# fatchord/WaveRNN

Hardware: AMD Instinct MI355X
Metric: audio samples/sec (real-time factor @22.05 kHz), MoL WaveRNN batched generate (higher is better)
Workload: dtype f32

## Files before the change

### include/wavernn_amd.h

```cpp
#ifndef WAVERNN_AMD_H
#define WAVERNN_AMD_H

#include <stddef.h>
#include <stdint.h>

#ifdef __cplusplus
extern "C" {
#endif

#define WRNN_ABI_VERSION 9

enum {
    WRNN_OK = 0,
    WRNN_ERR_ARG = -1,
    WRNN_ERR_NO_DEVICE = -2,
    WRNN_ERR_HIP = -3,
    WRNN_ERR_WORKSPACE = -4,
    WRNN_ERR_KERNEL = -5,
    WRNN_ERR_RESIDENCY = -6
};

enum { WRNN_MODE_RAW = 0, WRNN_MODE_MOL = 1 };

enum {
    WRNN_ALGO_AUTO = 0,
    WRNN_ALGO_STREAM = 1,
    WRNN_ALGO_LOOP = 2,
    WRNN_ALGO_DUO = 6,
    WRNN_ALGO_CHAIN = 7,
    WRNN_ALGO_OCTO = 8,
    WRNN_ALGO_SPARSE = 5
};

typedef struct wrnn_weights {
    int32_t rnn_dims;
    int32_t fc_dims;
    int32_t feat_dims;
    int32_t aux_dims;
    int32_t n_classes;
    int32_t mode;
    const float *I_w, *I_b;
    const float *w_ih1, *w_hh1, *b_ih1, *b_hh1;
    const float *w_ih2, *w_hh2, *b_ih2, *b_hh2;
    const float *fc1_w, *fc1_b;
    const float *fc2_w, *fc2_b;
    const float *fc3_w, *fc3_b;
} wrnn_weights;

typedef struct wrnn_pack wrnn_pack;

typedef struct wrnn_geometry {
    int32_t B;
    int32_t T;
    int32_t stride;
    int32_t L;
    int32_t hop;
    int32_t n_frames;
} wrnn_geometry;

typedef struct wrnn_timer wrnn_timer;

typedef struct wrnn_run_info {
    const char *kernel;
    int32_t units_per_wg;
    int32_t clusters;
    int32_t depth;
    int32_t rounds;
    int32_t slab_steps;
    int32_t launches;
} wrnn_run_info;

typedef struct wrnn_options {
    int32_t struct_bytes;
    int32_t algo;
    int32_t depth;
    int32_t clusters;
    int32_t cond_valu;
    int32_t slab_steps;
    int32_t t_begin, t_end;
    int32_t tuning;
    const float *force_x;
    float *logits;
    unsigned long long *phase_clocks;
    wrnn_timer *timer;
    wrnn_run_info *info;
    void (*progress)(int32_t steps_done, int32_t T, int32_t n_segments, void *user);
    void *progress_user;
    int32_t mel_stage;
    int32_t mel_rows;
    int32_t mel_scale;
    const float *mel_taps;
    const int32_t *seg_moff;
    int32_t sparse_groups;
    int32_t noise_lib;
    uint64_t noise_seed;
    const uint64_t *noise_seg_id;
} wrnn_options;

const char *wrnn_last_error(void);
int wrnn_abi_version(void);

int wrnn_device_cus(int device);

int wrnn_pack_create(const wrnn_weights *w, int device, wrnn_pack **out);
void wrnn_pack_destroy(wrnn_pack *p);
size_t wrnn_pack_weight_bytes(const wrnn_pack *p);
int wrnn_pack_sparse_blocks(const wrnn_pack *p);
int wrnn_pack_sparse_fc_blocks(const wrnn_pack *p);

size_t wrnn_workspace_bytes(const wrnn_pack *p, const wrnn_geometry *g, const wrnn_options *opt);

int wrnn_generate(const wrnn_pack *p, const wrnn_geometry *g, const float *mels_up, const float *aux,
                  const float *noise, float *out, void *workspace, size_t workspace_bytes, const wrnn_options *opt,
                  void *stream);

int wrnn_generate_segments(const wrnn_pack *p, int32_t n_segments, int32_t T, const int32_t *seg_pos,
                           const int32_t *seg_lim, int32_t L, int32_t hop, int32_t n_frames,
                           const float *mels_up, const float *aux, const float *noise, float *out,
                           void *workspace, size_t workspace_bytes, const wrnn_options *opt, void *stream);
size_t wrnn_workspace_bytes_segments(const wrnn_pack *p, int32_t n_segments, int32_t T, int32_t n_frames,
                                     const wrnn_options *opt);

int wrnn_noise_fill(int mode, int32_t n_segments, int32_t n_classes, int32_t t_begin, int32_t t_end, uint64_t seed, const uint64_t *seg_id,
                    float *out, int device, void *stream);
int wrnn_noise_fill_host(int mode, int32_t n_segments, int32_t n_classes, int32_t t_begin, int32_t t_end, uint64_t seed, const uint64_t *seg_id,
                         float *out);

int wrnn_plan_segments(const wrnn_pack *p, int32_t n_segments, int32_t T, const wrnn_options *opt, wrnn_run_info *out);

int wrnn_status(void *workspace, void *stream);

int wrnn_debug_read_exchange(const wrnn_pack *p, void *workspace, int32_t n_segments, int32_t T, int32_t n_frames,
                             const wrnn_options *opt, int cluster, int slot, int layer, int ring, float *host_out);

typedef struct wrnn_plan_traits {
    int32_t struct_bytes;
    int32_t n_cus;
    int32_t mode, C;
    int32_t generic;
    int32_t gH, gF, gM, gA;
    int32_t sp_nbp;
    int32_t sp_max_blocks;
    int32_t sp_fc;
} wrnn_plan_traits;
int wrnn_debug_plan(const wrnn_plan_traits *traits, int32_t n_segments, int32_t T, int32_t n_frames,
                    const wrnn_options *opt, wrnn_run_info *out, size_t *workspace_bytes);

int wrnn_timer_create(int device, wrnn_timer **out);
void wrnn_timer_destroy(wrnn_timer *t);
float wrnn_timer_ms(wrnn_timer *t);
int wrnn_timer_launches(const wrnn_timer *t);

typedef struct wrnn_pre_weights {
    int32_t feat_dims;
    int32_t compute_dims;
    int32_t res_out_dims;
    int32_t res_blocks;
    int32_t pad;
    int32_t upsample_factors[3];
    const float *conv_in_w;
    const float *bn_in;
    const float *res_w;
    const float *res_bn;
    const float *conv_out_w;
    const float *conv_out_b;
    const float *up_w;
} wrnn_pre_weights;
typedef struct wrnn_pre wrnn_pre;

int wrnn_pre_create(const wrnn_pre_weights *w, int device, wrnn_pre **out);
void wrnn_pre_destroy(wrnn_pre *p);
int wrnn_pre_hop(const wrnn_pre *p);
size_t wrnn_pre_workspace_bytes(const wrnn_pre *p, int32_t n_frames);
int wrnn_pre_upsample(const wrnn_pre *p, const float *mel, int32_t n_frames, float *mels_up, float *aux,
                      void *workspace, size_t workspace_bytes, void *stream);
int wrnn_pre_upsample_rows(const wrnn_pre *p, const float *mel, int32_t n_frames, float *mel_rows, float *aux,
                           void *workspace, size_t workspace_bytes, void *stream);
const char *wrnn_pre_last_error(void);

int wrnn_post_unfold(const float *segments, int32_t T, int32_t n_utt, const int32_t *first, const int32_t *folds,
                     const int64_t *out_off, const double *lut, int32_t n_classes, const double *fade_in,
                     const double *fade_out, int32_t overlap, const double *tail, int32_t tail_len, int32_t batched,
                     double *out, void *stream);
const char *wrnn_post_last_error(void);

typedef struct wrnn_taco_weights {
    uint32_t struct_bytes;
    int32_t n_mels, prenet1, prenet2, decoder_dims, encoder_width, lstm_dims, attn_filters, attn_kernel;
    const float *prenet_fc1_w, *prenet_fc1_b, *prenet_fc2_w, *prenet_fc2_b;
    const float *attn_rnn_w_ih, *attn_rnn_w_hh, *attn_rnn_b_ih, *attn_rnn_b_hh;
    const float *attn_W_w, *attn_W_b, *attn_conv_w, *attn_L_w, *attn_L_b, *attn_v_w;
    const float *rnn_input_w, *rnn_input_b;
    const float *rnn1_w_ih, *rnn1_w_hh, *rnn1_b_ih, *rnn1_b_hh;
    const float *rnn2_w_ih, *rnn2_w_hh, *rnn2_b_ih, *rnn2_b_hh;
    const float *mel_proj_w;
} wrnn_taco_weights;

typedef struct wrnn_taco_call {
    uint32_t struct_bytes;
    int32_t n;
    int32_t r, max_r;
    int32_t max_steps;
    float stop_threshold;
    const float *seq;
    const float *seq_proj;
    float *mel_out;
    float *scores_out;
    int32_t *steps_done;
    void *workspace;
    size_t workspace_bytes;
    void *stream;
    int32_t variant;
} wrnn_taco_call;

size_t wrnn_taco_workspace_bytes(void);
int wrnn_taco_decode(int device, const wrnn_taco_weights *w, const wrnn_taco_call *c);
int wrnn_taco_status(const void *workspace, unsigned *out4, void *stream);
const char *wrnn_taco_last_error(void);

#define WRNN_TACO_BATCH_MAX 8
#define WRNN_TACO_BATCH_NMAX 256
typedef struct wrnn_taco_batch_call {
    uint32_t struct_bytes;
    int32_t n_sent;
    int32_t r, max_r;
    float stop_threshold;
    const int32_t *n;
    const int32_t *max_steps;
    const float *const *seq, *const *seq_proj;
    float *const *mel_out;
    float *const *scores_out;
    int32_t *steps_done;
    void *workspace;
    size_t workspace_bytes;
    void *stream;
} wrnn_taco_batch_call;
size_t wrnn_taco_batch_workspace_bytes(int32_t n_sent);
int wrnn_taco_decode_batch(int device, const wrnn_taco_weights *w, const wrnn_taco_batch_call *c);

typedef struct wrnn_bigru_call {
    uint32_t struct_bytes;
    int32_t T, hidden;
    const float *gi_fwd, *gi_rev;
    const float *w_hh_fwd, *w_hh_rev;
    const float *b_hh_fwd, *b_hh_rev;
    float *out;
    void *stream;
} wrnn_bigru_call;
int wrnn_bigru(int device, const wrnn_bigru_call *c);

typedef struct wrnn_cbhg_weights {
    int32_t K;
    int32_t in_channels;
    int32_t proj1_channels;
    int32_t proj2_channels;
    int32_t channels;
    int32_t num_highways;
    const float *bank_conv_w[16];
    const float *bank_bn_w[16], *bank_bn_b[16], *bank_bn_mean[16], *bank_bn_var[16];
    const float *proj1_conv_w;
    const float *proj1_bn_w, *proj1_bn_b, *proj1_bn_mean, *proj1_bn_var;
    const float *proj2_conv_w;
    const float *proj2_bn_w, *proj2_bn_b, *proj2_bn_mean, *proj2_bn_var;
    const float *pre_highway_w;
    const float *highway_w1[4], *highway_b1[4], *highway_w2[4], *highway_b2[4];
    const float *rnn_w_ih, *rnn_w_hh, *rnn_b_ih, *rnn_b_hh;
    const float *rnn_w_ih_rev, *rnn_w_hh_rev, *rnn_b_ih_rev, *rnn_b_hh_rev;
} wrnn_cbhg_weights;

typedef struct wrnn_taco_front_weights {
    uint32_t struct_bytes;
    int32_t n_symbols, embed_dims;
    int32_t prenet1, prenet2;
    int32_t encoder_proj_dims;
    int32_t n_mels, fft_bins;
    const float *embedding;
    const float *prenet_fc1_w, *prenet_fc1_b, *prenet_fc2_w, *prenet_fc2_b;
    const float *encoder_proj_w, *post_proj_w;
    wrnn_cbhg_weights encoder_cbhg;
    wrnn_cbhg_weights postnet;
} wrnn_taco_front_weights;
typedef struct wrnn_taco_front wrnn_taco_front;

int wrnn_taco_front_create(const wrnn_taco_front_weights *w, int device, wrnn_taco_front **out);
void wrnn_taco_front_destroy(wrnn_taco_front *f);
size_t wrnn_taco_front_workspace_bytes(const wrnn_taco_front *f, int32_t rows);
int wrnn_taco_encode(const wrnn_taco_front *f, const int32_t *ids, int32_t n, float *seq_out, float *seq_proj_out, float *pre_rnn_out,
                     void *workspace, size_t workspace_bytes, void *stream);
int wrnn_taco_postnet(const wrnn_taco_front *f, const float *mel, int32_t N, float *linear_out, float *pre_rnn_out,
                      void *workspace, size_t workspace_bytes, void *stream);

int wrnn_selftest(int device, int which);
float wrnn_selftest_metric(void);

#ifdef __cplusplus
}
#endif
#endif
```

### wavernn_amd/_lib.py

```python
import ctypes
import os
import subprocess

_HERE = os.path.dirname(os.path.abspath(__file__))
CSRC = os.path.join(_HERE, 'csrc')
SO_PATH = os.path.join(CSRC, 'libwavernn_amd.so')

WRNN_OK = 0
ERR_ARG = -1
ERR_NO_DEVICE = -2
ERR_RESIDENCY = -6
MODE_RAW, MODE_MOL = 0, 1
ABI_VERSION = 9
ALGO_AUTO, ALGO_STREAM, ALGO_LOOP, ALGO_SPARSE, ALGO_DUO, ALGO_CHAIN, ALGO_OCTO = 0, 1, 2, 5, 6, 7, 8
ALGOS = {'auto': ALGO_AUTO, 'stream': ALGO_STREAM, 'loop': ALGO_LOOP, 'sparse': ALGO_SPARSE, 'duo': ALGO_DUO, 'chain': ALGO_CHAIN, 'octo': ALGO_OCTO}

EXPORTS = ['wrnn_last_error', 'wrnn_abi_version', 'wrnn_device_cus', 'wrnn_pack_create', 'wrnn_pack_destroy',
           'wrnn_pack_weight_bytes', 'wrnn_pack_sparse_blocks', 'wrnn_pack_sparse_fc_blocks', 'wrnn_workspace_bytes', 'wrnn_workspace_bytes_segments', 'wrnn_generate',
           'wrnn_generate_segments', 'wrnn_noise_fill', 'wrnn_noise_fill_host', 'wrnn_plan_segments', 'wrnn_status', 'wrnn_timer_create', 'wrnn_timer_destroy', 'wrnn_timer_ms',
           'wrnn_timer_launches', 'wrnn_debug_read_exchange', 'wrnn_debug_plan', 'wrnn_selftest', 'wrnn_selftest_metric', 'wrnn_pre_create',
           'wrnn_pre_destroy', 'wrnn_pre_hop', 'wrnn_pre_workspace_bytes', 'wrnn_pre_upsample', 'wrnn_pre_upsample_rows', 'wrnn_pre_last_error',
           'wrnn_post_unfold', 'wrnn_post_last_error', 'wrnn_taco_workspace_bytes', 'wrnn_taco_decode', 'wrnn_taco_status',
           'wrnn_taco_last_error', 'wrnn_bigru', 'wrnn_taco_front_create', 'wrnn_taco_front_destroy', 'wrnn_taco_front_workspace_bytes',
           'wrnn_taco_encode', 'wrnn_taco_postnet', 'wrnn_taco_batch_workspace_bytes', 'wrnn_taco_decode_batch']


class Weights(ctypes.Structure):
    _fields_ = [(n, ctypes.c_int32) for n in ('rnn_dims', 'fc_dims', 'feat_dims', 'aux_dims', 'n_classes', 'mode')] + \
               [(n, ctypes.c_void_p) for n in ('I_w', 'I_b', 'w_ih1', 'w_hh1', 'b_ih1', 'b_hh1', 'w_ih2', 'w_hh2',
                                               'b_ih2', 'b_hh2', 'fc1_w', 'fc1_b', 'fc2_w', 'fc2_b', 'fc3_w', 'fc3_b')]


class PreWeights(ctypes.Structure):
    _fields_ = [(n, ctypes.c_int32) for n in ('feat_dims', 'compute_dims', 'res_out_dims', 'res_blocks', 'pad')] + \
               [('upsample_factors', ctypes.c_int32 * 3)] + \
               [(n, ctypes.c_void_p) for n in ('conv_in_w', 'bn_in', 'res_w', 'res_bn', 'conv_out_w', 'conv_out_b', 'up_w')]


TACO_WEIGHT_FIELDS = ('prenet_fc1_w', 'prenet_fc1_b', 'prenet_fc2_w', 'prenet_fc2_b', 'attn_rnn_w_ih', 'attn_rnn_w_hh', 'attn_rnn_b_ih',
                      'attn_rnn_b_hh', 'attn_W_w', 'attn_W_b', 'attn_conv_w', 'attn_L_w', 'attn_L_b', 'attn_v_w', 'rnn_input_w', 'rnn_input_b',
                      'rnn1_w_ih', 'rnn1_w_hh', 'rnn1_b_ih', 'rnn1_b_hh', 'rnn2_w_ih', 'rnn2_w_hh', 'rnn2_b_ih', 'rnn2_b_hh', 'mel_proj_w')


class TacoWeights(ctypes.Structure):
    _fields_ = [('struct_bytes', ctypes.c_uint32)] + \
               [(n, ctypes.c_int32) for n in ('n_mels', 'prenet1', 'prenet2', 'decoder_dims', 'encoder_width', 'lstm_dims', 'attn_filters',
                                              'attn_kernel')] + \
               [(n, ctypes.c_void_p) for n in TACO_WEIGHT_FIELDS]


class TacoCall(ctypes.Structure):
    _fields_ = [('struct_bytes', ctypes.c_uint32), ('n', ctypes.c_int32), ('r', ctypes.c_int32), ('max_r', ctypes.c_int32),
                ('max_steps', ctypes.c_int32), ('stop_threshold', ctypes.c_float), ('seq', ctypes.c_void_p), ('seq_proj', ctypes.c_void_p),
                ('mel_out', ctypes.c_void_p), ('scores_out', ctypes.c_void_p), ('steps_done', ctypes.c_void_p),
                ('workspace', ctypes.c_void_p), ('workspace_bytes', ctypes.c_size_t), ('stream', ctypes.c_void_p), ('variant', ctypes.c_int32)]


TACO_BATCH_MAX = 8
TACO_BATCH_NMAX = 256


class TacoBatchCall(ctypes.Structure):
    _fields_ = [('struct_bytes', ctypes.c_uint32), ('n_sent', ctypes.c_int32), ('r', ctypes.c_int32), ('max_r', ctypes.c_int32),
                ('stop_threshold', ctypes.c_float), ('n', ctypes.POINTER(ctypes.c_int32)), ('max_steps', ctypes.POINTER(ctypes.c_int32)),
                ('seq', ctypes.POINTER(ctypes.c_void_p)), ('seq_proj', ctypes.POINTER(ctypes.c_void_p)),
                ('mel_out', ctypes.POINTER(ctypes.c_void_p)), ('scores_out', ctypes.POINTER(ctypes.c_void_p)),
                ('steps_done', ctypes.c_void_p), ('workspace', ctypes.c_void_p), ('workspace_bytes', ctypes.c_size_t), ('stream', ctypes.c_void_p)]


class BigruCall(ctypes.Structure):
    _fields_ = [('struct_bytes', ctypes.c_uint32), ('T', ctypes.c_int32), ('hidden', ctypes.c_int32)] + \
               [(n, ctypes.c_void_p) for n in ('gi_fwd', 'gi_rev', 'w_hh_fwd', 'w_hh_rev', 'b_hh_fwd', 'b_hh_rev', 'out', 'stream')]


class CbhgWeights(ctypes.Structure):
    _fields_ = [(n, ctypes.c_int32) for n in ('K', 'in_channels', 'proj1_channels', 'proj2_channels', 'channels', 'num_highways')] + \
               [(n, ctypes.c_void_p * 16) for n in ('bank_conv_w', 'bank_bn_w', 'bank_bn_b', 'bank_bn_mean', 'bank_bn_var')] + \
               [(n, ctypes.c_void_p) for n in ('proj1_conv_w', 'proj1_bn_w', 'proj1_bn_b', 'proj1_bn_mean', 'proj1_bn_var', 'proj2_conv_w',
                                               'proj2_bn_w', 'proj2_bn_b', 'proj2_bn_mean', 'proj2_bn_var', 'pre_highway_w')] + \
               [(n, ctypes.c_void_p * 4) for n in ('highway_w1', 'highway_b1', 'highway_w2', 'highway_b2')] + \
               [(n, ctypes.c_void_p) for n in ('rnn_w_ih', 'rnn_w_hh', 'rnn_b_ih', 'rnn_b_hh', 'rnn_w_ih_rev', 'rnn_w_hh_rev', 'rnn_b_ih_rev',
                                               'rnn_b_hh_rev')]


class TacoFrontWeights(ctypes.Structure):
    _fields_ = [('struct_bytes', ctypes.c_uint32)] + \
               [(n, ctypes.c_int32) for n in ('n_symbols', 'embed_dims', 'prenet1', 'prenet2', 'encoder_proj_dims', 'n_mels', 'fft_bins')] + \
               [(n, ctypes.c_void_p) for n in ('embedding', 'prenet_fc1_w', 'prenet_fc1_b', 'prenet_fc2_w', 'prenet_fc2_b', 'encoder_proj_w',
                                               'post_proj_w')] + \
               [('encoder_cbhg', CbhgWeights), ('postnet', CbhgWeights)]


class Geometry(ctypes.Structure):
    _fields_ = [(n, ctypes.c_int32) for n in ('B', 'T', 'stride', 'L', 'hop', 'n_frames')]


class RunInfo(ctypes.Structure):
    _fields_ = [('kernel', ctypes.c_char_p)] + \
               [(n, ctypes.c_int32) for n in ('units_per_wg', 'clusters', 'depth', 'rounds', 'slab_steps', 'launches')]


class PlanTraits(ctypes.Structure):
    _fields_ = [(n, ctypes.c_int32) for n in ('struct_bytes', 'n_cus', 'mode', 'C', 'generic', 'gH', 'gF', 'gM', 'gA', 'sp_nbp', 'sp_max_blocks',
                                              'sp_fc')]

    def __init__(self, **kw):
        super().__init__(**kw)
        self.struct_bytes = ctypes.sizeof(PlanTraits)


class Options(ctypes.Structure):
    _fields_ = [(n, ctypes.c_int32) for n in ('struct_bytes', 'algo', 'depth', 'clusters', 'cond_valu', 'slab_steps', 't_begin',
                                              't_end', 'tuning')] + \
               [('force_x', ctypes.c_void_p), ('logits', ctypes.c_void_p), ('phase_clocks', ctypes.c_void_p), ('timer', ctypes.c_void_p),
                ('info', ctypes.POINTER(RunInfo)), ('progress', ctypes.c_void_p), ('progress_user', ctypes.c_void_p),
                ('mel_stage', ctypes.c_int32), ('mel_rows', ctypes.c_int32), ('mel_scale', ctypes.c_int32),
                ('mel_taps', ctypes.c_void_p), ('seg_moff', ctypes.c_void_p), ('sparse_groups', ctypes.c_int32),
                ('noise_lib', ctypes.c_int32), ('noise_seed', ctypes.c_uint64), ('noise_seg_id', ctypes.c_void_p)]

    def __init__(self, **kw):
        super().__init__(**kw)
        self.struct_bytes = ctypes.sizeof(Options)


PROGRESS_FN = ctypes.CFUNCTYPE(None, ctypes.c_int32, ctypes.c_int32, ctypes.c_int32, ctypes.c_void_p)


class WrnnError(RuntimeError):
    pass


class ResidencyError(WrnnError):
    """WRNN_ERR_RESIDENCY on the FIRST slice of a step-sliced `auto` run: the persistent grid is not co-resident right now.  The
    callers that slice (WaveRNN.generate, generate_corpus) catch it and redo the call unsliced on the stream kernel."""


def build(verbose=False):
    cmd = [os.path.join(CSRC, 'build.sh')]
    res = subprocess.run(cmd, stdout=subprocess.PIPE, stderr=subprocess.STDOUT, text=True)
    if verbose or res.returncode != 0:
        print(res.stdout)
    if res.returncode != 0:
        raise WrnnError('building libwavernn_amd.so failed')
    global _lib
    _lib = None
    return SO_PATH


_lib = None


def lib():
    global _lib
    if _lib is not None:
        return _lib
    if not os.path.exists(SO_PATH):
        raise WrnnError(f'{SO_PATH} not found: run `python -c "import __graft_entry__ as g; g.build()"` '
                        f'(or wavernn_amd/csrc/build.sh).  There is no CPU fallback.')
    import torch
    L = ctypes.CDLL(SO_PATH)
    L.wrnn_last_error.restype = ctypes.c_char_p
    L.wrnn_abi_version.restype = ctypes.c_int
    L.wrnn_device_cus.argtypes = [ctypes.c_int]
    L.wrnn_pack_create.argtypes = [ctypes.POINTER(Weights), ctypes.c_int, ctypes.POINTER(ctypes.c_void_p)]
    L.wrnn_pack_destroy.argtypes = [ctypes.c_void_p]
    L.wrnn_pack_destroy.restype = None
    L.wrnn_pack_weight_bytes.argtypes = [ctypes.c_void_p]
    L.wrnn_pack_weight_bytes.restype = ctypes.c_size_t
    L.wrnn_pack_sparse_blocks.argtypes = [ctypes.c_void_p]
    L.wrnn_pack_sparse_fc_blocks.argtypes = [ctypes.c_void_p]
    L.wrnn_workspace_bytes.argtypes = [ctypes.c_void_p, ctypes.POINTER(Geometry), ctypes.POINTER(Options)]
    L.wrnn_workspace_bytes.restype = ctypes.c_size_t
    L.wrnn_generate.argtypes = [ctypes.c_void_p, ctypes.POINTER(Geometry), ctypes.c_void_p, ctypes.c_void_p,
                                ctypes.c_void_p, ctypes.c_void_p, ctypes.c_void_p, ctypes.c_size_t, ctypes.POINTER(Options),
                                ctypes.c_void_p]
    L.wrnn_workspace_bytes_segments.argtypes = [ctypes.c_void_p, ctypes.c_int32, ctypes.c_int32, ctypes.c_int32,
                                                ctypes.POINTER(Options)]
    L.wrnn_workspace_bytes_segments.restype = ctypes.c_size_t
    L.wrnn_generate_segments.argtypes = [ctypes.c_void_p, ctypes.c_int32, ctypes.c_int32, ctypes.c_void_p, ctypes.c_void_p,
                                         ctypes.c_int32, ctypes.c_int32, ctypes.c_int32, ctypes.c_void_p, ctypes.c_void_p,
                                         ctypes.c_void_p, ctypes.c_void_p, ctypes.c_void_p, ctypes.c_size_t,
                                         ctypes.POINTER(Options), ctypes.c_void_p]
    L.wrnn_noise_fill.argtypes = [ctypes.c_int, ctypes.c_int32, ctypes.c_int32, ctypes.c_int32, ctypes.c_int32, ctypes.c_uint64, ctypes.c_void_p,
                                  ctypes.c_void_p, ctypes.c_int, ctypes.c_void_p]
    L.wrnn_noise_fill_host.argtypes = L.wrnn_noise_fill.argtypes[:8]
    L.wrnn_plan_segments.argtypes = [ctypes.c_void_p, ctypes.c_int32, ctypes.c_int32, ctypes.POINTER(Options), ctypes.POINTER(RunInfo)]
    L.wrnn_timer_create.argtypes = [ctypes.c_int, ctypes.POINTER(ctypes.c_void_p)]
    L.wrnn_timer_destroy.argtypes = [ctypes.c_void_p]
    L.wrnn_timer_destroy.restype = None
    L.wrnn_timer_ms.argtypes = [ctypes.c_void_p]
    L.wrnn_timer_ms.restype = ctypes.c_float
    L.wrnn_timer_launches.argtypes = [ctypes.c_void_p]
    L.wrnn_debug_read_exchange.argtypes = [ctypes.c_void_p, ctypes.c_void_p, ctypes.c_int32, ctypes.c_int32, ctypes.c_int32,
                                           ctypes.POINTER(Options), ctypes.c_int, ctypes.c_int, ctypes.c_int, ctypes.c_int,
                                           ctypes.c_void_p]
    L.wrnn_debug_plan.argtypes = [ctypes.POINTER(PlanTraits), ctypes.c_int32, ctypes.c_int32, ctypes.c_int32, ctypes.POINTER(Options),
                                  ctypes.POINTER(RunInfo), ctypes.POINTER(ctypes.c_size_t)]
    L.wrnn_pre_create.argtypes = [ctypes.POINTER(PreWeights), ctypes.c_int, ctypes.POINTER(ctypes.c_void_p)]
    L.wrnn_pre_destroy.argtypes = [ctypes.c_void_p]
    L.wrnn_pre_destroy.restype = None
    L.wrnn_pre_hop.argtypes = [ctypes.c_void_p]
    L.wrnn_pre_workspace_bytes.argtypes = [ctypes.c_void_p, ctypes.c_int32]
    L.wrnn_pre_workspace_bytes.restype = ctypes.c_size_t
    L.wrnn_pre_upsample.argtypes = [ctypes.c_void_p, ctypes.c_void_p, ctypes.c_int32, ctypes.c_void_p, ctypes.c_void_p,
                                    ctypes.c_void_p, ctypes.c_size_t, ctypes.c_void_p]
    L.wrnn_pre_upsample_rows.argtypes = L.wrnn_pre_upsample.argtypes
    L.wrnn_pre_last_error.restype = ctypes.c_char_p
    L.wrnn_post_unfold.argtypes = [ctypes.c_void_p, ctypes.c_int32, ctypes.c_int32, ctypes.c_void_p, ctypes.c_void_p, ctypes.c_void_p,
                                   ctypes.c_void_p, ctypes.c_int32, ctypes.c_void_p, ctypes.c_void_p, ctypes.c_int32,
                                   ctypes.c_void_p, ctypes.c_int32, ctypes.c_int32, ctypes.c_void_p, ctypes.c_void_p]
    L.wrnn_post_last_error.restype = ctypes.c_char_p
    L.wrnn_taco_workspace_bytes.restype = ctypes.c_size_t
    L.wrnn_taco_decode.argtypes = [ctypes.c_int, ctypes.POINTER(TacoWeights), ctypes.POINTER(TacoCall)]
    L.wrnn_taco_status.argtypes = [ctypes.c_void_p, ctypes.POINTER(ctypes.c_uint32 * 4), ctypes.c_void_p]
    L.wrnn_taco_last_error.restype = ctypes.c_char_p
    L.wrnn_taco_batch_workspace_bytes.argtypes = [ctypes.c_int32]
    L.wrnn_taco_batch_workspace_bytes.restype = ctypes.c_size_t
    L.wrnn_taco_decode_batch.argtypes = [ctypes.c_int, ctypes.POINTER(TacoWeights), ctypes.POINTER(TacoBatchCall)]
    L.wrnn_bigru.argtypes = [ctypes.c_int, ctypes.POINTER(BigruCall)]
    L.wrnn_taco_front_create.argtypes = [ctypes.POINTER(TacoFrontWeights), ctypes.c_int, ctypes.POINTER(ctypes.c_void_p)]
    L.wrnn_taco_front_destroy.argtypes = [ctypes.c_void_p]
    L.wrnn_taco_front_destroy.restype = None
    L.wrnn_taco_front_workspace_bytes.argtypes = [ctypes.c_void_p, ctypes.c_int32]
    L.wrnn_taco_front_workspace_bytes.restype = ctypes.c_size_t
    L.wrnn_taco_encode.argtypes = [ctypes.c_void_p, ctypes.c_void_p, ctypes.c_int32, ctypes.c_void_p, ctypes.c_void_p, ctypes.c_void_p,
                                   ctypes.c_void_p, ctypes.c_size_t, ctypes.c_void_p]
    L.wrnn_taco_postnet.argtypes = [ctypes.c_void_p, ctypes.c_void_p, ctypes.c_int32, ctypes.c_void_p, ctypes.c_void_p, ctypes.c_void_p,
                                    ctypes.c_size_t, ctypes.c_void_p]
    L.wrnn_status.argtypes = [ctypes.c_void_p, ctypes.c_void_p]
    L.wrnn_selftest.argtypes = [ctypes.c_int, ctypes.c_int]
    L.wrnn_selftest_metric.restype = ctypes.c_float
    _lib = L
    return L


def check(rc, what):
    if rc != WRNN_OK:
        raise WrnnError(f'{what} failed (rc={rc}): {lib().wrnn_last_error().decode()}')


def noise_fill_host(mode, n_segments, n_classes, t_begin, t_end, seed, seg_id=None):
    import numpy as np
    mol = mode == 'MOL'
    out = np.empty((t_end - t_begin, 11 * n_segments) if mol else (t_end - t_begin, n_segments, n_classes), np.float32)
    ids = None if seg_id is None else np.ascontiguousarray(seg_id, dtype=np.uint64)
    if ids is not None and ids.shape != (n_segments,):
        raise ValueError('seg_id: one 64-bit id per segment')
    check(lib().wrnn_noise_fill_host(MODE_MOL if mol else MODE_RAW, n_segments, n_classes, t_begin, t_end, int(seed) & (2 ** 64 - 1),
                                     None if ids is None else ids.ctypes.data, out.ctypes.data), 'wrnn_noise_fill_host')
    return out
```

### wavernn_amd/batch.py

```python
import time
from dataclasses import dataclass
from typing import List, Optional, Sequence

import numpy as np
import torch

from . import fold as _fold


@dataclass
class Plan:
    target: int
    overlap: int
    T: int
    stride: int
    lengths: List[int]
    offsets: np.ndarray
    folds: np.ndarray
    first: np.ndarray
    seg_pos: np.ndarray
    seg_lim: np.ndarray
    seg_utt: np.ndarray

    @property
    def n_segments(self):
        return int(self.seg_pos.shape[0])

    @property
    def total_len(self):
        return int(sum(self.lengths))


def plan_utterances(lengths: Sequence[int], target: int, overlap: int) -> Plan:
    lengths = [int(x) for x in lengths]
    if not lengths or min(lengths) < 1:
        raise ValueError('need at least one non-empty utterance')
    stride, T = target + overlap, target + 2 * overlap
    folds = np.array([_fold.fold_geometry(L, target, overlap)[0] for L in lengths], dtype=np.int64)
    offsets = np.concatenate([[0], np.cumsum(lengths)[:-1]]).astype(np.int64)
    first = np.concatenate([[0], np.cumsum(folds)[:-1]]).astype(np.int64)
    if offsets[-1] + lengths[-1] + T >= 2 ** 31:
        raise ValueError('concatenated conditioning exceeds int32 positions; split the corpus')
    seg_pos, seg_lim, seg_utt = [], [], []
    for u, (L, nf) in enumerate(zip(lengths, folds)):
        seg_pos.append(offsets[u] + np.arange(nf, dtype=np.int64) * stride)
        seg_lim.append(np.full(nf, offsets[u] + L, dtype=np.int64))
        seg_utt.append(np.full(nf, u, dtype=np.int64))
    return Plan(target, overlap, T, stride, lengths, offsets, folds, first,
                np.concatenate(seg_pos).astype(np.int32), np.concatenate(seg_lim).astype(np.int32),
                np.concatenate(seg_utt).astype(np.int32))


def shard_bounds(n_segments: int, world: int, active: Optional[int] = None):
    active = world if active is None else max(1, min(int(active), world))
    return [((r * n_segments) // active, ((r + 1) * n_segments) // active) if r < active else (n_segments, n_segments) for r in range(world)]


DEFAULT_STEP_US_BY_DEPTH = {1: 10.4, 2: 13.8, 3: 19.4, 4: 22.9, 5: 27.4, 6: 31.3, 7: 35.5, 8: 38.9}
_STEP_TABLE = None


def kernel_source_sha16() -> str:
    import hashlib
    import os
    from . import _lib
    h = hashlib.sha256()
    for name in ('wrnn_abi.hip', 'wrnn_cond.hip', 'wrnn_device.h', 'wrnn_duo.hip', 'wrnn_loop.hip', 'wrnn_ring.h', 'wrnn_tiles.h'):
        h.update(open(os.path.join(_lib.CSRC, name), 'rb').read())
    return h.hexdigest()[:16]


def step_table(path: Optional[str] = None):
    global _STEP_TABLE
    if _STEP_TABLE is None or path is not None:
        import json
        import os
        from . import _lib
        f = path or os.path.join(os.path.dirname(os.path.dirname(_lib.CSRC)), 'profiles', 'step_us.json')
        table, origin = dict(DEFAULT_STEP_US_BY_DEPTH), 'built-in defaults (no profiles/step_us.json)'
        try:
            j = json.load(open(f))
            if j.get('source_sha16') == kernel_source_sha16():
                table, origin = {int(k): float(v) for k, v in j['step_us_by_depth'].items()}, f'{f} (measured on these kernel sources)'
            else:
                origin = f'built-in defaults ({f} was measured on other kernel sources)'
        except (OSError, ValueError, KeyError):
            pass
        if path is not None:
            return table, origin
        _STEP_TABLE = (table, origin)
    return _STEP_TABLE


def estimate_step_us(n_segments: int, table: Optional[dict] = None) -> float:
    if n_segments <= 0:
        return 0.0
    table = table or step_table()[0]
    groups = -(-n_segments // 16)
    rounds = -(-groups // 32)
    depth = min(8, max(1, -(-(-(-groups // rounds)) // 4)))
    return rounds * table[depth]


def choose_ranks(n_segments: int, world: int, table: Optional[dict] = None) -> int:
    est = [estimate_step_us(-(-n_segments // r), table) for r in range(1, world + 1)]
    best = min(est)
    return 1 + next(i for i, e in enumerate(est) if e <= best * 1.01)


def pack_noise(mode: str, plan: Plan, per_utt, lo: int = 0, hi: Optional[int] = None, steps: Optional[int] = None):
    hi = plan.n_segments if hi is None else hi
    T = plan.T if steps is None else int(steps)
    n = hi - lo
    utts = [u for u in range(len(plan.lengths)) if plan.first[u] < hi and plan.first[u] + plan.folds[u] > lo]
    sample = per_utt[utts[0]]
    is_torch = isinstance(sample, torch.Tensor)
    cat = (lambda xs, d: torch.cat(xs, dim=d)) if is_torch else (lambda xs, d: np.concatenate(xs, axis=d))
    mix, logi, raw = [], [], []
    for u in utts:
        Bu, f0 = int(plan.folds[u]), int(plan.first[u])
        a, b = max(lo, f0) - f0, min(hi, f0 + Bu) - f0
        z = per_utt[u]
        if mode == 'MOL':
            z = z.reshape(T, 11 * Bu)
            mix.append(z[:, 10 * a:10 * b])
            logi.append(z[:, 10 * Bu + a:10 * Bu + b])
        else:
            raw.append(z.reshape(T, Bu, -1)[:, a:b])
    out = cat(mix + logi, 1) if mode == 'MOL' else cat(raw, 1)
    assert out.shape[0] == T and (out.shape[1] == 11 * n if mode == 'MOL' else out.shape[1] == n)
    return out.contiguous() if is_torch else np.ascontiguousarray(out)


def library_seg_ids(seed, folds, first_fold: int = 0) -> np.ndarray:
    hi = np.uint64((int(seed) & 0xffffffff) << 32)
    return hi | np.arange(first_fold, first_fold + int(folds), dtype=np.uint64)


def chunk_utterances(plan: Plan, lo: int, hi: int, max_segments: int):
    chunks, cur, cur_lo, cur_hi = [], [], None, None
    for u in range(len(plan.lengths)):
        a, b = max(lo, int(plan.first[u])), min(hi, int(plan.first[u] + plan.folds[u]))
        if a >= b:
            continue
        if cur and (b - cur_lo) > max_segments:
            chunks.append((cur, cur_lo, cur_hi))
            cur, cur_lo = [], None
        if cur_lo is None:
            cur_lo = a
        cur.append(u)
        cur_hi = b
    if cur:
        chunks.append((cur, cur_lo, cur_hi))
    return chunks


def generate_corpus(model, mels: Sequence, target: int, overlap: int, mu_law: bool, seeds: Optional[Sequence[int]] = None,
                    group=None, loop_fn=None, return_segments=False, noise_source='cpu', finish='all', check=True,
                    max_segments_per_launch: int = 4096, shard=None, ranks: Optional[int] = None, timings: Optional[dict] = None):
    import torch.distributed as dist
    from .rng import draw_steps
    if noise_source in ('cpu', 'library') and seeds is None:
        raise ValueError(f"noise_source={noise_source!r} needs `seeds` (one per utterance); "
                         "pass noise_source='device' to draw from the device generator instead")
    if noise_source not in ('cpu', 'device', 'library'):
        raise ValueError(f'unknown noise source {noise_source!r}')
    world = dist.get_world_size(group) if group is not None else 1
    rank = dist.get_rank(group) if group is not None else 0
    if shard is not None:
        if group is not None:
            raise ValueError('shard=(rank, world) emulates a rank without a process group')
        rank, world = int(shard[0]), int(shard[1])
        finish = 'own'
    device = next(model.parameters()).device
    mode = model.mode
    mu_law = mu_law if mode == 'RAW' else False
    hop = model.hop_length
    was_training = model.training
    model.eval()
    mels = [torch.as_tensor(m) for m in mels]
    mels = [m.unsqueeze(0) if m.dim() == 2 else m for m in mels]
    frames = [int(m.size(-1)) for m in mels]
    plan = plan_utterances([n * hop for n in frames], target, overlap)
    bounds = shard_bounds(plan.n_segments, world, ranks)
    lo, hi = bounds[rank]
    n_max = max(h - l for l, h in bounds)

    out_local = torch.zeros(n_max, plan.T, dtype=torch.float32, device=device)
    native_pre = loop_fn is None and getattr(model, 'pre_algo', 'torch') == 'native' and device.type == 'cuda'
    with torch.no_grad():
        for utts, clo, chi in (chunk_utterances(plan, lo, hi, max_segments_per_launch) if hi > lo else []):
            noise = [None] * len(mels)
            local_off, off = {}, 0
            for u in utts:
                local_off[u] = off
                off += frames[u] * hop
            n_seg, T = chi - clo, plan.T
            eng = model._loop_engine() if loop_fn is None else None

            def conditioning(rows):
                if native_pre:
                    pre = model._pre_engine()
                    n_rows = [pre.rows_of(frames[u]) for u in utts] if rows else None
                    mels_up = torch.empty(sum(n_rows) if rows else off, mels[utts[0]].size(1), dtype=torch.float32, device=device)
                    aux = torch.empty(off // hop, 4 * model.aux_dims, dtype=torch.float32, device=device)
                    r0, jobs = 0, []
                    for k, u in enumerate(utts):
                        a0 = local_off[u]
                        if rows:
                            jobs.append((mels[u], mels_up[r0:r0 + n_rows[k]], aux[a0 // hop:a0 // hop + frames[u]]))
                            r0 += n_rows[k]
                        else:
                            jobs.append((mels[u], mels_up[a0:a0 + frames[u] * hop], aux[a0 // hop:a0 // hop + frames[u]]))
                    pre.upsample_many(jobs, rows=rows, streams=int(getattr(model, 'pre_streams', 8)))
                    if rows:
                        from .engine import MelRows
                        indent, order = pre.pad * hop, {u: k for k, u in enumerate(utts)}
                        seg_off = np.array([indent * (2 * order[int(u)] + 1) for u in plan.seg_utt[clo:chi]], dtype=np.int32)
                        mels_up = MelRows(mels_up, off, pre.scales[2], pre.last_taps, seg_off)
                    return mels_up, aux
                ups, auxs = zip(*[model.conditioning(mels[u])[:2] for u in utts])
                return torch.cat(ups).contiguous(), torch.cat(auxs).contiguous()
            rows = eng is not None and native_pre and model.mel_rows_ok(eng, n_seg, T)
            mels_up, aux = conditioning(rows)
            rebase = np.array([local_off[int(u)] - int(plan.offsets[int(u)]) for u in plan.seg_utt[clo:chi]], dtype=np.int64)
            seg_pos = (plan.seg_pos[clo:chi].astype(np.int64) + rebase).astype(np.int32)
            seg_lim = (plan.seg_lim[clo:chi].astype(np.int64) + rebase).astype(np.int32)
            out_view = out_local[clo - lo:chi - lo]
            gens, pool = {}, None
            if noise_source == 'cpu':
                if len(utts) > 1 and mode == 'RAW':
                    import os
                    from concurrent.futures import ThreadPoolExecutor
                    pool = ThreadPoolExecutor(max(1, min(len(utts), (os.cpu_count() or 2) // (2 * max(1, int(os.environ.get('LOCAL_WORLD_SIZE', '1')))))))
                from .rng import burn_ctor_draws
                for u in utts:
                    gens[u] = torch.Generator(device='cpu').manual_seed(int(seeds[u]))
                    burn_ctor_draws(model.rnn_dims, model.aux_dims, 'cpu', gens[u])

            lib_ids = None
            if noise_source == 'library':
                lib_ids = np.concatenate([library_seg_ids(seeds[u], min(chi, int(plan.first[u] + plan.folds[u])) - max(clo, int(plan.first[u])),
                                                          max(clo, int(plan.first[u])) - int(plan.first[u])) for u in utts])
                assert lib_ids.shape == (n_seg,)
            lib_kw = dict(noise_seed=int(getattr(model, 'noise_key', 0)), noise_seg_id=lib_ids) if lib_ids is not None else {}

            def draw(steps_):
                if noise_source == 'library':
                    if loop_fn is None:
                        return None
                    from ._lib import noise_fill_host
                    return torch.from_numpy(noise_fill_host(mode, n_seg, model.n_classes, 0, steps_, lib_kw['noise_seed'], lib_ids)).to(device)
                if noise_source != 'cpu':
                    return draw_steps(mode, n_seg, steps_, model.n_classes, device, 'device')
                def one(u):
                    noise[u] = draw_steps(mode, int(plan.folds[u]), steps_, model.n_classes, 'cpu', 'cpu', generator=gens[u])
                if pool is None:
                    for u in utts:
                        one(u)
                else:
                    list(pool.map(one, utts))
                return pack_noise(mode, plan, noise, clo, chi, steps=steps_).to(device)

            if loop_fn is not None:
                out_view[:] = loop_fn(mels_up, aux, seg_pos, seg_lim, T, draw(T), hop)
                if pool is not None:
                    pool.shutdown()
                continue
            from ._lib import ResidencyError
            from .engine import RESUMABLE_KERNELS
            steps = T
            groups = model.loop_sparse_groups(eng, n_seg, T) if hasattr(model, 'loop_sparse_groups') else 0
            if noise_source != 'library' and eng.plan(n_seg, T, algo=model.loop_algo)['kernel'] in RESUMABLE_KERNELS:
                per_step = n_seg * (11 if mode == 'MOL' else model.n_classes) * 4
                steps = max(1, min(T, getattr(model, 'noise_chunk_bytes', 2 << 30) // per_step))
                steps = -(-T // (-(-T // steps)))
            try:
                for t0 in range(0, T, steps):
                    t1 = min(T, t0 + steps)
                    eng.run_segments(mels_up, aux, seg_pos, seg_lim, T, draw(t1 - t0), hop, algo=model.loop_algo, check=check, out=out_view,
                                     t_range=None if (t0 == 0 and t1 == T) else (t0, t1), sparse_groups=groups, **lib_kw)
            except ResidencyError as e:
                import warnings
                warnings.warn(f'wavernn_amd: {e}; redoing the chunk unsliced on the next kernel')
                if rows:
                    mels_up, aux = conditioning(False)
                for u in gens:
                    gens[u].manual_seed(int(seeds[u]))
                    burn_ctor_draws(model.rnn_dims, model.aux_dims, 'cpu', gens[u])
                eng.run_segments(mels_up, aux, seg_pos, seg_lim, T, draw(T), hop, algo=model.loop_algo, check=check, out=out_view, sparse_groups=groups, **lib_kw)
            finally:
                if pool is not None:
                    pool.shutdown()
    n_utt = len(frames)
    work, gathered = None, None
    if group is not None:
        gathered = [torch.empty_like(out_local) for _ in range(world)]
        work = dist.all_gather(gathered, out_local, group=group, async_op=True)
        if timings is not None:
            timings['gather_bytes'] = timings.get('gather_bytes', 0) + (world - 1) * out_local.numel() * out_local.element_size()
            timings['world_seen'] = dist.get_world_size(group)

    def gathered_segments():
        nonlocal work
        if group is None:
            if shard is not None:
                raise ValueError('an emulated shard has only its own block of segments')
            return out_local[:plan.n_segments]
        if work is not None:
            t_w = time.perf_counter()
            work.wait()
            work = None
            if timings is not None:
                timings['gather_wait_ms'] = timings.get('gather_wait_ms', 0.0) + (time.perf_counter() - t_w) * 1e3
        return torch.cat([gathered[r][:h - l] for r, (l, h) in enumerate(bounds)])

    if was_training:
        model.train()
    if return_segments:
        return gathered_segments().cpu().numpy().astype(np.float64), plan
    mine_u = [u for u in range(n_utt) if finish != 'own' or (lo <= plan.first[u] < hi)]
    local_u = [u for u in mine_u if lo <= plan.first[u] and plan.first[u] + plan.folds[u] <= hi]
    local_set = set(local_u)
    rest_u = [u for u in mine_u if u not in local_set]
    outs = [None] * n_utt
    native_post = loop_fn is None and getattr(model, 'post_algo', 'numpy') == 'native' and out_local.is_cuda

    def unfold(segs, first_of, us):
        if not us:
            return
        if native_post:
            from .post import unfold_on_device
            wav, sl = unfold_on_device(segs, [first_of(u) for u in us], [int(plan.folds[u]) for u in us],
                                       [(frames[u] - 1) * hop for u in us], overlap, hop, model.n_classes, mu_law, True)
            if getattr(model, 'pinned_output', True):
                host = torch.empty(wav.shape, dtype=wav.dtype, pin_memory=True)
                host.copy_(wav, non_blocking=True)
                torch.cuda.current_stream(wav.device).synchronize()
                wav = host.numpy()
            else:
                wav = wav.cpu().numpy()
            for (a, b), u in zip(sl, us):
                outs[u] = wav[a:b]
            return
        host = segs.cpu().numpy().astype(np.float64)
        for u in us:
            y = host[first_of(u):first_of(u) + int(plan.folds[u])].copy()
            if mu_law:
                y = _fold.decode_mu_law(y, model.n_classes, False)
            y = _fold.xfade_and_unfold(y, target, overlap)
            outs[u] = _fold.finish_waveform(y, (frames[u] - 1) * hop, hop)

    t_u = time.perf_counter()
    unfold(out_local, lambda u: int(plan.first[u]) - lo, local_u)
    if timings is not None:
        timings['unfold_under_gather_ms'] = timings.get('unfold_under_gather_ms', 0.0) + (time.perf_counter() - t_u) * 1e3
    if shard is not None:
        return outs
    if rest_u:
        unfold(gathered_segments(), lambda u: int(plan.first[u]), rest_u)
    elif work is not None:
        t_w = time.perf_counter()
        work.wait()
        if timings is not None:
            timings['gather_wait_ms'] = timings.get('gather_wait_ms', 0.0) + (time.perf_counter() - t_w) * 1e3
    return outs
```

### wavernn_amd/csrc/wrnn_abi.hip

```cpp
#include <hip/hip_runtime.h>
#include <stdarg.h>
#include <stdio.h>
#include <stdlib.h>
#include <string.h>
#include <math.h>
#include <string>
#include <vector>

#include "../../include/wavernn_amd.h"
#include "wrnn_device.h"

namespace wrnn {
hipError_t launch_cond(const CondArgs &a, int n_cus, bool valu, hipStream_t stream);
hipError_t launch_cond_frames(const CondArgs &a, hipStream_t stream);
hipError_t launch_cond_frames_slab(const CondArgs &a, hipStream_t stream);
hipError_t launch_cond_frag(const CondArgs &a, int n_cus, hipStream_t stream);
hipError_t launch_noise_mol(const float *in, float *out, long n, int B, int n_cus, hipStream_t stream);
hipError_t launch_noise_fill(bool mol, int B, int C, int t0, int t1, uint64_t seed, const uint64_t *seg_id, float *out, int n_cus, hipStream_t stream);
void noise_fill_host(bool mol, int B, int C, int t0, int t1, uint64_t seed, const uint64_t *seg_id, float *out);
hipError_t launch_stream(const LoopArgs &args, int mode, hipStream_t stream);
hipError_t launch_loop(const LoopArgs &args, int ncl, int mode, hipStream_t stream);
int loop_max_depth(int mode);
size_t loop_state_floats(int G);
hipError_t launch_generic(const GenArgs &args, int mode, hipStream_t stream);
bool generic_dims_ok(int H, int F, int M, int A, int C, int mode);
hipError_t launch_duo(const LoopArgs &args, int ncl, int mode, hipStream_t stream);
int duo_max_depth();
size_t duo_xbuf_bytes(int G);
size_t duo_xbuf_bytes_max();
hipError_t launch_sparse(const LoopArgs &args, int nbp, int mode, hipStream_t stream);
int sparse_clusters(int n_cus);
int sparse_max_slots();
size_t sparse_state_floats(int slots);
size_t sparse_xbuf_bytes(int slots);
hipError_t launch_put_floats(float *dst, const float *src, int n, hipStream_t stream);
hipError_t launch_chain(const LoopArgs &args, int mode, hipStream_t stream);
hipError_t launch_octo(const LoopArgs &args, int ncl, int mode, hipStream_t stream);
int octo_max_depth();
int chain_clusters(int n_cus);
int chain_max_depth();
size_t chain_state_floats(int G);
size_t chain_xbuf_bytes(int G);
int selftest_mfma(char *msg, size_t n);
int selftest_allgather(int n_cus, char *msg, size_t n, float *us_per_round);
int selftest_tanh(char *msg, size_t n);
int selftest_xor(char *msg, size_t n);
}

using namespace wrnn;

static thread_local char g_err[512] = "";
static void set_err(const char *fmt, ...)
{
    va_list ap;
    va_start(ap, fmt);
    vsnprintf(g_err, sizeof g_err, fmt, ap);
    va_end(ap);
}
#define HIPCHK(expr)                                                                          \
    do {                                                                                      \
        hipError_t e_ = (expr);                                                               \
        if (e_ != hipSuccess) {                                                               \
            set_err("%s failed: %s (%s:%d)", #expr, hipGetErrorString(e_), __FILE__, __LINE__); \
            return WRNN_ERR_HIP;                                                              \
        }                                                                                     \
    } while (0)

struct wrnn_pack {
    int device;
    wrnn_plan_traits tr;
    size_t weight_bytes;
    char *dev;
    size_t dev_bytes;
    const float *I_w0, *I_b, *I_cT;
    const float *w_ih1, *w_hh1, *b_ih1, *b_hh1, *w_ih2, *w_hh2, *b_ih2, *b_hh2;
    const float *fc1_w, *fc1_b, *fc2_w, *fc2_b, *fc3_w, *fc3_b;
    const float *w_ih1T, *w_hh1T, *w_ih2T, *w_hh2T, *fc1T, *fc2T, *fc3T, *c2_wT, *c3_wT, *c4_wT;
    const float *fc3f;
    const float *u1;
    const float *g_I_T, *g_fc1T, *g_fc2T, *g_w_ih2T;
    const float *sp_vals;
    const int *sp_cols;
    int sp_fc_max_blocks;
    const float *sp_fc_vals;
    const int *sp_fc_cols;
};

extern "C" const char *wrnn_last_error(void) { return g_err; }
extern "C" int wrnn_abi_version(void) { return WRNN_ABI_VERSION; }

extern "C" int wrnn_device_cus(int device)
{
    int n = 0;
    if (hipGetDeviceCount(&n) != hipSuccess || n <= 0 || device >= n) {
        set_err("no HIP device %d (count %d)", device, n);
        return WRNN_ERR_NO_DEVICE;
    }
    hipDeviceProp_t prop;
    if (hipGetDeviceProperties(&prop, device) != hipSuccess) return WRNN_ERR_NO_DEVICE;
    return prop.multiProcessorCount;
}

namespace {
struct Builder {
    std::vector<float> host;
    size_t add(const float *src, size_t n)
    {
        size_t off = (host.size() + 63) / 64 * 64;
        host.resize(off + n);
        if (src) memcpy(host.data() + off, src, n * sizeof(float));
        return off;
    }
    size_t add_T(const float *src, int rows, int ld, int col0, int ncols)
    {
        size_t off = add(nullptr, (size_t)ncols * rows);
        float *d = host.data() + off;
        for (int r = 0; r < rows; ++r)
            for (int k = 0; k < ncols; ++k) d[(size_t)k * rows + r] = src[(size_t)r * ld + col0 + k];
        return off;
    }
};
}

extern "C" int wrnn_pack_create(const wrnn_weights *w, int device, wrnn_pack **out)
{
    if (!w || !out) { set_err("NULL argument"); return WRNN_ERR_ARG; }
    const int C = w->n_classes;
    const bool shipped = w->rnn_dims == H && w->fc_dims == H && w->feat_dims == MEL && w->aux_dims == AUX && !(w->mode == WRNN_MODE_RAW && C > H);
    if (w->mode == WRNN_MODE_MOL) {
        if (C != 30) { set_err("MOL needs n_classes == 30"); return WRNN_ERR_ARG; }
    } else if (w->mode == WRNN_MODE_RAW) {
        if (shipped && C < 2) { set_err("RAW needs 2 <= n_classes <= 2048 (the shipped dims: up to 512 on the MFMA / stream kernels, more on the generic kernel)"); return WRNN_ERR_ARG; }
    } else { set_err("unknown mode %d", w->mode); return WRNN_ERR_ARG; }
    if (!shipped && !generic_dims_ok(w->rnn_dims, w->fc_dims, w->feat_dims, w->aux_dims, C, w->mode)) {
        set_err("unsupported dims rnn=%d fc=%d feat=%d aux=%d classes=%d: the generic kernel takes rnn, fc, classes <= 2048, feat + aux <= 1024 "
                "(MOL: 30 classes)", w->rnn_dims, w->fc_dims, w->feat_dims, w->aux_dims, C);
        return WRNN_ERR_ARG;
    }
    const float *const *ptrs = &w->I_w;
    for (int i = 0; i < 16; ++i)
        if (!ptrs[i]) { set_err("NULL weight pointer #%d", i); return WRNN_ERR_ARG; }
    const int cus = wrnn_device_cus(device);
    if (cus < 0) return cus;
    DeviceGuard dg(device);
    HIPCHK(dg.err);

    if (!shipped) {
        const int gH = w->rnn_dims, gF = w->fc_dims, gM = w->feat_dims, gA = w->aux_dims;
        Builder b;
        const size_t oI = b.add_T(w->I_w, gH, 1 + gM + gA, 0, 1 + gM + gA), oIb = b.add(w->I_b, gH);
        const size_t o1i = b.add_T(w->w_ih1, 3 * gH, gH, 0, gH), o1h = b.add_T(w->w_hh1, 3 * gH, gH, 0, gH);
        const size_t o1bi = b.add(w->b_ih1, 3 * gH), o1bh = b.add(w->b_hh1, 3 * gH);
        const size_t o2i = b.add_T(w->w_ih2, 3 * gH, gH + gA, 0, gH + gA), o2h = b.add_T(w->w_hh2, 3 * gH, gH, 0, gH);
        const size_t o2bi = b.add(w->b_ih2, 3 * gH), o2bh = b.add(w->b_hh2, 3 * gH);
        const size_t of1 = b.add_T(w->fc1_w, gF, gH + gA, 0, gH + gA), of1b = b.add(w->fc1_b, gF);
        const size_t of2 = b.add_T(w->fc2_w, gF, gF + gA, 0, gF + gA), of2b = b.add(w->fc2_b, gF);
        const size_t of3 = b.add_T(w->fc3_w, C, gF, 0, gF), of3b = b.add(w->fc3_b, C);
        b.add(nullptr, 64);
        wrnn_pack *p = new wrnn_pack();
        memset(p, 0, sizeof *p);
        p->device = device; p->tr.n_cus = cus; p->tr.C = C; p->tr.mode = w->mode; p->tr.generic = 1;
        p->tr.gH = gH; p->tr.gF = gF; p->tr.gM = gM; p->tr.gA = gA;
        p->dev_bytes = b.host.size() * sizeof(float);
        p->weight_bytes = sizeof(float) * ((size_t)gH * (1 + gM + gA) + gH + 2 * ((size_t)3 * gH * gH) + (size_t)3 * gH * (gH + gA) + (size_t)3 * gH * gH +
                                           4 * 3 * gH + (size_t)gF * (gH + gA) + (size_t)gF * (gF + gA) + 2 * gF + (size_t)C * gF + C);
        hipError_t e = hipMalloc((void **)&p->dev, p->dev_bytes);
        if (e != hipSuccess) { set_err("hipMalloc(%zu) failed: %s", p->dev_bytes, hipGetErrorString(e)); delete p; return WRNN_ERR_HIP; }
        e = hipMemcpy(p->dev, b.host.data(), p->dev_bytes, hipMemcpyHostToDevice);
        if (e != hipSuccess) { set_err("hipMemcpy failed: %s", hipGetErrorString(e)); (void)hipFree(p->dev); delete p; return WRNN_ERR_HIP; }
        const float *base = (const float *)p->dev;
        p->g_I_T = base + oI; p->I_b = base + oIb;
        p->w_ih1T = base + o1i; p->w_hh1T = base + o1h; p->b_ih1 = base + o1bi; p->b_hh1 = base + o1bh;
        p->g_w_ih2T = base + o2i; p->w_hh2T = base + o2h; p->b_ih2 = base + o2bi; p->b_hh2 = base + o2bh;
        p->g_fc1T = base + of1; p->fc1_b = base + of1b; p->g_fc2T = base + of2; p->fc2_b = base + of2b;
        p->fc3T = base + of3; p->fc3_b = base + of3b;
        p->tr.sp_max_blocks = gH;
        p->tr.struct_bytes = (int32_t)sizeof p->tr;
        *out = p;
        return WRNN_OK;
    }

    const int KI = 1 + MEL + AUX, K2 = H + AUX;
    Builder b;
    std::vector<float> col0(H);
    for (int r = 0; r < H; ++r) col0[r] = w->I_w[(size_t)r * KI];
    const size_t o_I_w0 = b.add(col0.data(), H), o_I_b = b.add(w->I_b, H);
    const size_t o_I_cT = b.add_T(w->I_w, H, KI, 1, KCOND);
    const size_t o_w_ih1 = b.add(w->w_ih1, (size_t)3 * H * H), o_w_hh1 = b.add(w->w_hh1, (size_t)3 * H * H);
    const size_t o_b_ih1 = b.add(w->b_ih1, 3 * H), o_b_hh1 = b.add(w->b_hh1, 3 * H);
    const size_t o_w_ih2 = b.add(w->w_ih2, (size_t)3 * H * K2), o_w_hh2 = b.add(w->w_hh2, (size_t)3 * H * H);
    const size_t o_b_ih2 = b.add(w->b_ih2, 3 * H), o_b_hh2 = b.add(w->b_hh2, 3 * H);
    const size_t o_fc1_w = b.add(w->fc1_w, (size_t)H * K2), o_fc1_b = b.add(w->fc1_b, H);
    const size_t o_fc2_w = b.add(w->fc2_w, (size_t)H * K2), o_fc2_b = b.add(w->fc2_b, H);
    const size_t o_fc3_w = b.add(w->fc3_w, (size_t)C * H), o_fc3_b = b.add(w->fc3_b, C);
    const size_t o_w_ih1T = b.add_T(w->w_ih1, 3 * H, H, 0, H), o_w_hh1T = b.add_T(w->w_hh1, 3 * H, H, 0, H);
    const size_t o_w_ih2T = b.add_T(w->w_ih2, 3 * H, K2, 0, H), o_w_hh2T = b.add_T(w->w_hh2, 3 * H, H, 0, H);
    const size_t o_fc1T = b.add_T(w->fc1_w, H, K2, 0, H), o_fc2T = b.add_T(w->fc2_w, H, K2, 0, H);
    const size_t o_fc3T = b.add_T(w->fc3_w, C, H, 0, H);
    const size_t o_c2_wT = b.add_T(w->w_ih2, 3 * H, K2, H, AUX);
    const size_t o_c3_wT = b.add_T(w->fc1_w, H, K2, H, AUX), o_c4_wT = b.add_T(w->fc2_w, H, K2, H, AUX);
    size_t o_fc3f = 0;
    if (w->mode == WRNN_MODE_MOL) {
        o_fc3f = b.add(nullptr, (size_t)2 * SEG * H);
        for (int q = 0; q < 2 * SEG * H / 4; ++q) {
            const int l6 = q & 63, r = (q >> 6) & 7, wv = (q >> 9) & 3, tile = q >> 11;
            const int row = 16 * tile + (l6 & 15), kq = l6 >> 4;
            for (int e = 0; e < 4; ++e)
                b.host[o_fc3f + (size_t)q * 4 + e] = row < C ? w->fc3_w[(size_t)row * H + 128 * wv + 16 * r + 4 * kq + e] : 0.f;
        }
    }
    size_t o_u1 = 0;
    {
        o_u1 = b.add(nullptr, (size_t)3 * H);
        for (int r = 0; r < 3 * H; ++r) {
            double acc = 0.0;
            for (int k = 0; k < H; ++k) acc += (double)w->w_ih1[(size_t)r * H + k] * (double)col0[k];
            b.host[o_u1 + r] = (float)acc;
        }
    }
    int sp_nbp = 0, sp_max = 0, sp_fc_max = 0;
    bool sp_fc_ok = false;
    size_t o_spv = 0, o_spc = 0, o_sfv = 0, o_sfc = 0;
    {
        const float *mats[4] = {w->w_ih1, w->w_hh1, w->w_ih2, w->w_hh2};
        const int lds_[4] = {H, H, K2, H};
        std::vector<std::vector<int>> cols((size_t)4 * 32 * 3);
        for (int m = 0; m < 4; ++m)
            for (int wg = 0; wg < 32; ++wg)
                for (int g = 0; g < 3; ++g) {
                    std::vector<int> &cv = cols[((size_t)m * 32 + wg) * 3 + g];
                    const float *base = mats[m] + ((size_t)g * H + 16 * wg) * lds_[m];
                    for (int c = 0; c < H; ++c) {
                        bool nz = false;
                        for (int r = 0; r < 16 && !nz; ++r) nz = base[(size_t)r * lds_[m] + c] != 0.0f;
                        if (nz) cv.push_back(c);
                    }
                    if ((int)cv.size() > sp_max) sp_max = (int)cv.size();
                }
        const float *fmats[2] = {w->fc1_w, w->fc2_w};
        std::vector<std::vector<int>> fcols((size_t)2 * 32);
        for (int m = 0; m < 2; ++m)
            for (int wg = 0; wg < 32; ++wg) {
                std::vector<int> &cv = fcols[(size_t)m * 32 + wg];
                const float *base = fmats[m] + (size_t)(16 * wg) * K2;
                for (int c = 0; c < H; ++c) {
                    bool nz = false;
                    for (int r = 0; r < 16 && !nz; ++r) nz = base[(size_t)r * K2 + c] != 0.0f;
                    if (nz) cv.push_back(c);
                }
                if ((int)cv.size() > sp_fc_max) sp_fc_max = (int)cv.size();
            }
        if (sp_max <= 64 && (w->mode == WRNN_MODE_MOL || C == H)) {
            sp_nbp = sp_max <= 48 ? 48 : 64;
            if (sp_fc_max <= 64) {
                if (sp_fc_max > 48) sp_nbp = 64;
                o_sfv = b.add(nullptr, (size_t)2 * 32 * sp_nbp * 16);
                o_sfc = b.add(nullptr, (size_t)2 * 32 * sp_nbp);
                for (size_t q = 0; q < (size_t)2 * 32 * sp_nbp * 16; ++q) b.host[o_sfv + q] = 0.f;
                int *fi_ = reinterpret_cast<int *>(b.host.data() + o_sfc);
                for (size_t q = 0; q < (size_t)2 * 32 * sp_nbp; ++q) fi_[q] = 0;
                for (int m = 0; m < 2; ++m)
                    for (int wg = 0; wg < 32; ++wg) {
                        const size_t br = (size_t)m * 32 + wg;
                        const std::vector<int> &cv = fcols[br];
                        const float *base = fmats[m] + (size_t)(16 * wg) * K2;
                        for (size_t k = 0; k < cv.size(); ++k) {
                            reinterpret_cast<int *>(b.host.data() + o_sfc)[br * sp_nbp + k] = cv[k];
                            for (int r = 0; r < 16; ++r) b.host[o_sfv + (br * sp_nbp + k) * 16 + r] = base[(size_t)r * K2 + cv[k]];
                        }
                    }
                sp_fc_ok = true;
            }
            o_spv = b.add(nullptr, (size_t)4 * 32 * 3 * sp_nbp * 16);
            o_spc = b.add(nullptr, (size_t)4 * 32 * 3 * sp_nbp);
            for (size_t q = 0; q < (size_t)4 * 32 * 3 * sp_nbp * 16; ++q) b.host[o_spv + q] = 0.f;
            int *ci = reinterpret_cast<int *>(b.host.data() + o_spc);
            for (size_t q = 0; q < (size_t)4 * 32 * 3 * sp_nbp; ++q) ci[q] = 0;
            for (int m = 0; m < 4; ++m)
                for (int wg = 0; wg < 32; ++wg)
                    for (int g = 0; g < 3; ++g) {
                        const size_t br = ((size_t)m * 32 + wg) * 3 + g;
                        const std::vector<int> &cv = cols[br];
                        const float *base = mats[m] + ((size_t)g * H + 16 * wg) * lds_[m];
                        for (size_t k = 0; k < cv.size(); ++k) {
                            ci[br * sp_nbp + k] = cv[k];
                            for (int r = 0; r < 16; ++r) b.host[o_spv + (br * sp_nbp + k) * 16 + r] = base[(size_t)r * lds_[m] + cv[k]];
                        }
                    }
        }
    }
    b.add(nullptr, 64);

    wrnn_pack *p = new wrnn_pack();
    p->device = device; p->tr.n_cus = cus; p->tr.C = C; p->tr.mode = w->mode;
    p->dev_bytes = b.host.size() * sizeof(float);
    p->weight_bytes = sizeof(float) * ((size_t)H * KI + H + 2 * ((size_t)3 * H * H) + (size_t)3 * H * K2 + (size_t)3 * H * H +
                                       4 * 3 * H + 2 * ((size_t)H * K2 + H) + (size_t)C * H + C);
    hipError_t e = hipMalloc((void **)&p->dev, p->dev_bytes);
    if (e != hipSuccess) { set_err("hipMalloc(%zu) failed: %s", p->dev_bytes, hipGetErrorString(e)); delete p; return WRNN_ERR_HIP; }
    e = hipMemcpy(p->dev, b.host.data(), p->dev_bytes, hipMemcpyHostToDevice);
    if (e != hipSuccess) { set_err("hipMemcpy failed: %s", hipGetErrorString(e)); (void)hipFree(p->dev); delete p; return WRNN_ERR_HIP; }
    const float *base = (const float *)p->dev;
    p->I_w0 = base + o_I_w0; p->I_b = base + o_I_b; p->I_cT = base + o_I_cT;
    p->w_ih1 = base + o_w_ih1; p->w_hh1 = base + o_w_hh1; p->b_ih1 = base + o_b_ih1; p->b_hh1 = base + o_b_hh1;
    p->w_ih2 = base + o_w_ih2; p->w_hh2 = base + o_w_hh2; p->b_ih2 = base + o_b_ih2; p->b_hh2 = base + o_b_hh2;
    p->fc1_w = base + o_fc1_w; p->fc1_b = base + o_fc1_b; p->fc2_w = base + o_fc2_w; p->fc2_b = base + o_fc2_b;
    p->fc3_w = base + o_fc3_w; p->fc3_b = base + o_fc3_b;
    p->w_ih1T = base + o_w_ih1T; p->w_hh1T = base + o_w_hh1T; p->w_ih2T = base + o_w_ih2T; p->w_hh2T = base + o_w_hh2T;
    p->fc1T = base + o_fc1T; p->fc2T = base + o_fc2T; p->fc3T = base + o_fc3T;
    p->c2_wT = base + o_c2_wT; p->c3_wT = base + o_c3_wT; p->c4_wT = base + o_c4_wT;
    p->fc3f = w->mode == WRNN_MODE_MOL ? base + o_fc3f : nullptr;
    p->u1 = base + o_u1;
    p->tr.sp_nbp = sp_nbp; p->tr.sp_max_blocks = sp_max;
    p->sp_vals = sp_nbp ? base + o_spv : nullptr;
    p->sp_cols = sp_nbp ? reinterpret_cast<const int *>(base + o_spc) : nullptr;
    p->sp_fc_max_blocks = sp_fc_max;
    p->sp_fc_vals = sp_fc_ok ? base + o_sfv : nullptr;
    p->sp_fc_cols = sp_fc_ok ? reinterpret_cast<const int *>(base + o_sfc) : nullptr;
// ... 244 lines not shown
        return p->mode != WRNN_MODE_MOL ? WRNN_ERR_ARG : WRNN_ERR_RESIDENCY;
    }
    if (algo == WRNN_ALGO_DUO && (!shape_ok || KINDS[K_DUO].clusters(p->n_cus) < 1)) {
        set_err("the two-workgroups-per-CU loop kernel needs MOL or RAW with 512 classes, and >= 64 CUs (C = %d, device has %d CUs)", p->C, p->n_cus);
        return !shape_ok ? WRNN_ERR_ARG : WRNN_ERR_RESIDENCY;
    }
    if (algo == WRNN_ALGO_LOOP && !(shape_ok && lcl >= 1)) {
        set_err("the loop kernel needs >= 64 CUs and (MOL or RAW with 512 classes); device has %d CUs, C=%d", p->n_cus, p->C);
        return WRNN_ERR_RESIDENCY;
    }
    const bool sparse_auto = p->sp_nbp && p->mode == WRNN_MODE_MOL;
    Kind kind = K_STREAM;
    int ncl = 0;
    if (algo == WRNN_ALGO_CHAIN || (algo == WRNN_ALGO_AUTO && chain_hw && groups <= CHAIN_AUTO_GROUPS && !sparse_auto)) {
        kind = K_CHAIN; ncl = ccl;
    } else if (algo == WRNN_ALGO_SPARSE || (algo == WRNN_ALGO_AUTO && sparse_auto && scl >= 1)) {
        kind = K_SPARSE; ncl = scl;
    } else if (algo != WRNN_ALGO_STREAM && shape_ok && lcl >= 1) {
        ncl = lcl;
        if (o->clusters == 1 || o->clusters == 2 || o->clusters == 4) ncl = o->clusters < ncl ? o->clusters : ncl;
        else if (groups < ncl && !(DUO_AUTO && algo != WRNN_ALGO_LOOP && ncl == MAXCL)) {
            int c2 = 1; while (c2 < groups) c2 *= 2; if (c2 < ncl) ncl = c2;
        }
        kind = K_LOOP;
        if (algo == WRNN_ALGO_DUO || (algo == WRNN_ALGO_AUTO && DUO_AUTO && ncl == MAXCL)) kind = K_DUO;
        if (algo == WRNN_ALGO_OCTO || (kind == K_DUO && algo == WRNN_ALGO_AUTO && OCTO_AUTO && p->mode == WRNN_MODE_MOL && !o->clusters)) kind = K_OCTO;
    }
    const KindDesc &k = KINDS[kind];
    pl->kind = kind;
    if (two_groups) {
        if (kind != K_SPARSE) {
            set_err("wrnn_options.sparse_groups = 2: only wrnn_sparse_kernel runs two groups per cluster (this call runs on %s)", k.name);
            return WRNN_ERR_ARG;
        }
        if (p->mode != WRNN_MODE_MOL) { set_err("wrnn_options.sparse_groups = 2: wrnn_sparse_kernel's 9-bit RAW form is built with one group per cluster only"); return WRNN_ERR_ARG; }
        if (!p->sp_fc || (o->tuning & 2048)) {
            set_err("wrnn_options.sparse_groups = 2: needs a pack whose Linear layers are block-sparse too (wrnn_pack_sparse_fc_blocks() > 0) and their gathered fc "
                    "stages: the dense fc tiles leave no registers for a second group");
            return WRNN_ERR_ARG;
        }
        if (o->phase_clocks && !(o->tuning & 64)) { set_err("wrnn_options.sparse_groups = 2: the phase-clock build of wrnn_sparse_kernel has one group per cluster only"); return WRNN_ERR_ARG; }
    }
    if (k.persistent) {
        if (two_groups) plan_split(pl, B, ncl, sparse_max_slots(), sparse_max_slots());
        else plan_split(pl, B, ncl, k.max_depth(p->mode), o->depth);
        pl->slab = o->slab_steps >= 1 ? o->slab_steps : default_slab(*pl, p->mode, p->C, o->noise_lib != 0);
        if (pl->slab > T) pl->slab = T;
        pl->tab_fps = DUO_TAB_FPS;
    } else if (partial) {
        set_err("a partial step range [%d, %d) needs a persistent loop kernel", pl->t0, pl->t1);
        return WRNN_ERR_ARG;
    }
    if (k.slabbed && ((size_t)B * pl->tab_fps + 1) * 3 * H * sizeof(float) >= 0x7FFFF000ull) {
        set_err("%d segments in one call: the per-slab aux tables exceed a 2 GB buffer resource; split the call (generate_corpus caps a launch at 4096 segments)", B);
        return WRNN_ERR_ARG;
    }
    return WRNN_OK;
}

WsLayout ws_layout(const wrnn_plan_traits *p, const Plan &pl, int B, int T, int n_frames, bool noise_lib)
{
    const size_t noise_row = (size_t)B * (p->mode == WRNN_MODE_MOL ? 11 : p->C) * sizeof(float);
    const KindDesc &k = KINDS[pl.kind];
    WsLayout l;
    memset(&l, 0, sizeof l);
    size_t o = 0;
    l.status = o; o = al(o + STATUS_WORDS * sizeof(unsigned));
    l.xcc = o;    o = al(o + XCC_WORDS * sizeof(unsigned));
    l.segs = o;   o = al(o + (size_t)3 * B * sizeof(int));
    l.melc = o;   o = al(o + (size_t)3 * LAST_SCALE * sizeof(float));
    if (pl.kind == K_GENERIC) {
        l.nlib = o; if (noise_lib) o = al(o + (size_t)T * noise_row);
        l.total = o;
        return l;
    }
    const size_t tab_rows = k.slabbed ? (size_t)B * pl.tab_fps + 1 : (size_t)n_frames + 1;
    l.c2f = o;    o = al(o + tab_rows * 3 * H * sizeof(float));
    l.c3f = o;    o = al(o + tab_rows * H * sizeof(float));
    l.c4f = o;    o = al(o + tab_rows * H * sizeof(float));
    if (k.persistent) {
        l.xbuf = o;  o = al(o + k.xbuf_bytes(pl.G));
        l.state = o; o = al(o + (size_t)pl.rounds * k.state_floats(pl.G) * sizeof(float));
        l.cIf = o;   if (!k.slabbed) o = al(o + (size_t)pl.slab * pl.ngr_max * SEG * H * sizeof(float));
        l.npre = o;  if (p->mode == WRNN_MODE_MOL) o = al(o + (size_t)pl.slab * 11 * B * sizeof(float));
    } else {
        l.cI = o;    o = al(o + (size_t)T * B * H * sizeof(float));
        l.npre = o;
    }
    l.nlib = o;   if (noise_lib) o = al(o + (size_t)(k.persistent ? pl.slab : T) * noise_row);
    l.total = o;
    return l;
}
void hop_magic(int hop, unsigned *magic, int *shift)
{
    *magic = 0u; *shift = 0;
    if (hop < 2) return;
    int s = 0;
    while ((1ll << s) < hop) ++s;
    const unsigned long long m = ((1ull << (31 + s)) + (unsigned long long)hop - 1ull) / (unsigned long long)hop;
    if (m >> 32) return;
    const int sh = s - 1;
    for (long long q = 0; q * hop < (1ll << 31); q += 997) {
        for (long long p = q * hop - 1; p <= q * hop + 1; ++p) {
            if (p < 0 || p >= (1ll << 31)) continue;
            if ((long long)(((unsigned long long)p * m) >> (32 + sh)) != p / hop) return;
        }
    }
    *magic = (unsigned)m; *shift = sh;
}

int check_geometry(const wrnn_geometry *g)
{
    if (!g) { set_err("NULL geometry"); return WRNN_ERR_ARG; }
    if (g->B < 1 || g->T < 1 || g->L < 1 || g->hop < 1 || g->n_frames < 1 || g->stride < 0) {
        set_err("bad geometry B=%d T=%d stride=%d L=%d hop=%d n_frames=%d", g->B, g->T, g->stride, g->L, g->hop, g->n_frames);
        return WRNN_ERR_ARG;
    }
    if ((long)g->n_frames * g->hop < g->L) { set_err("n_frames*hop < L"); return WRNN_ERR_ARG; }
    if ((double)g->B * g->stride + g->T > 2.0e9) { set_err("geometry overflows int32"); return WRNN_ERR_ARG; }
    return WRNN_OK;
}
int check_segments(int B, int T, const int32_t *seg_pos, const int32_t *seg_lim, int L, int hop, int n_frames)
{
    if (B < 1 || T < 1 || L < 1 || hop < 1 || n_frames < 1 || !seg_pos || !seg_lim) {
        set_err("bad segment table B=%d T=%d L=%d hop=%d n_frames=%d", B, T, L, hop, n_frames);
        return WRNN_ERR_ARG;
    }
    if ((long)n_frames * hop < L) { set_err("n_frames*hop < L"); return WRNN_ERR_ARG; }
    for (int b = 0; b < B; ++b) {
        if (seg_pos[b] < 0 || seg_lim[b] < 0 || seg_lim[b] > L || (double)seg_pos[b] + T > 2.0e9) {
            set_err("segment %d: pos=%d lim=%d outside [0,%d]", b, seg_pos[b], seg_lim[b], L);
            return WRNN_ERR_ARG;
        }
    }
    return WRNN_OK;
}
int plan_report(const wrnn_plan_traits *tr, int B, int T, int n_frames, const wrnn_options &o, wrnn_run_info *out, size_t *ws_bytes)
{
    Plan pl;
    const int rc = make_plan(tr, B, T, &o, &pl);
    if (rc != WRNN_OK) return rc;
    if (out) {
        memset(out, 0, sizeof *out);
        out->kernel = KINDS[pl.kind].name; out->units_per_wg = KINDS[pl.kind].units_per_wg;
        out->clusters = pl.ncl; out->depth = pl.G; out->rounds = pl.rounds; out->slab_steps = pl.slab;
    }
    if (ws_bytes) *ws_bytes = ws_layout(tr, pl, B, T, n_frames, o.noise_lib != 0).total;
    return WRNN_OK;
}
}

extern "C" size_t wrnn_workspace_bytes_segments(const wrnn_pack *p, int32_t n_segments, int32_t T, int32_t n_frames,
                                                const wrnn_options *opt)
{
    if (!p || n_segments < 1 || T < 1 || n_frames < 1) return 0;
    size_t bytes = 0;
    (void)plan_report(&p->tr, n_segments, T, n_frames, whole_call(opt), nullptr, &bytes);
    return bytes;
}

extern "C" int wrnn_plan_segments(const wrnn_pack *p, int32_t n_segments, int32_t T, const wrnn_options *opt, wrnn_run_info *out)
{
    if (!p || !out || n_segments < 1 || T < 1) { set_err("bad argument"); return WRNN_ERR_ARG; }
    return plan_report(&p->tr, n_segments, T, 1, whole_call(opt), out, nullptr);
}

extern "C" size_t wrnn_workspace_bytes(const wrnn_pack *p, const wrnn_geometry *g, const wrnn_options *opt)
{
    if (!p || check_geometry(g) != WRNN_OK) return 0;
    return wrnn_workspace_bytes_segments(p, g->B, g->T, g->n_frames, opt);
}

extern "C" int wrnn_generate_segments(const wrnn_pack *p, int32_t B, int32_t T, const int32_t *seg_pos,
                                      const int32_t *seg_lim, int32_t L, int32_t hop, int32_t n_frames,
                                      const float *mels_up, const float *aux, const float *noise, float *out,
                                      void *workspace, size_t workspace_bytes, const wrnn_options *opt, void *stream_)
{
    const wrnn_options opts = norm_struct(opt), *o = &opts;
    const bool lib_noise = o->noise_lib == 1;
    if (lib_noise && noise) {
        set_err("wrnn_options.noise_lib = 1: the library draws the noise itself -- `noise` must be NULL (the tensor passed would not be read)");
        return WRNN_ERR_ARG;
    }
    if (!p || !mels_up || !aux || (!noise && !lib_noise) || !out || !workspace) { set_err("NULL argument"); return WRNN_ERR_ARG; }
    int rc = check_segments(B, T, seg_pos, seg_lim, L, hop, n_frames);
    if (rc != WRNN_OK) return rc;
    Plan pl;
    if ((rc = make_plan(&p->tr, B, T, o, &pl)) != WRNN_OK) return rc;
    const KindDesc &k = KINDS[pl.kind];
    const WsLayout l = ws_layout(&p->tr, pl, B, T, n_frames, lib_noise);
    if (workspace_bytes < l.total) { set_err("workspace %zu < required %zu", workspace_bytes, l.total); return WRNN_ERR_WORKSPACE; }
    if (((uintptr_t)workspace & 255) != 0) { set_err("workspace must be 256-byte aligned"); return WRNN_ERR_ARG; }
    hipStream_t stream = (hipStream_t)stream_;
    DeviceGuard dg(p->device);
    HIPCHK(dg.err);
    char *ws = (char *)workspace;
    const bool mol_mode = p->tr.mode == WRNN_MODE_MOL;
    wrnn_timer *timer = o->timer;
    if (timer && pl.t0 == 0) timer->used = 0;

    if (pl.t0 == 0) HIPCHK(hipMemsetAsync(ws + l.status, 0, STATUS_WORDS * sizeof(unsigned), stream));
    HIPCHK(hipMemcpyAsync(ws + l.segs, seg_pos, (size_t)B * sizeof(int), hipMemcpyHostToDevice, stream));
    HIPCHK(hipMemcpyAsync(ws + l.segs + (size_t)B * sizeof(int), seg_lim, (size_t)B * sizeof(int), hipMemcpyHostToDevice, stream));
    const int *d_pos = (const int *)(ws + l.segs), *d_lim = d_pos + B;
    if (o->mel_stage) {
        if (!k.mel_stage) { set_err("wrnn_options.mel_stage: only wrnn_duo_kernel / wrnn_sparse_kernel / wrnn_chain_kernel form the last up-sampling stage (this call runs on another kernel)"); return WRNN_ERR_ARG; }
        if (o->mel_stage != 1 || o->mel_scale != LAST_SCALE || !o->mel_taps || !o->seg_moff || o->mel_rows < 3) {
            set_err("wrnn_options.mel_stage=%d: needs mel_scale == %d (got %d), mel_taps, seg_moff, mel_rows >= 3", o->mel_stage, LAST_SCALE, o->mel_scale);
            return WRNN_ERR_ARG;
        }
        for (int b = 0; b < B; ++b) {
            const long last = (seg_lim[b] < (long)seg_pos[b] + T ? seg_lim[b] : (long)seg_pos[b] + T) - 1;
            if (last < seg_pos[b]) continue;
            const long j0 = (long)seg_pos[b] + o->seg_moff[b], j1 = last + o->seg_moff[b];
            if (o->seg_moff[b] < 0 || j0 / LAST_SCALE < 1 || j1 / LAST_SCALE + 1 >= o->mel_rows) {
                set_err("segment %d: positions %ld..%ld of the last up-sampling stage reach outside its %d input rows", b, j0, j1, o->mel_rows);
                return WRNN_ERR_ARG;
            }
        }
        float coef[3 * LAST_SCALE];
        for (int ph = 0; ph < LAST_SCALE; ++ph) {
            double c0 = 0, c1 = 0, c2 = 0;
            for (int j = 0; j <= 2 * LAST_SCALE; ++j) {
                const double w = o->mel_taps[j];
                if (j < LAST_SCALE - ph) c0 += w; else if (j < 2 * LAST_SCALE - ph) c1 += w; else c2 += w;
            }
            coef[3 * ph] = (float)c0; coef[3 * ph + 1] = (float)c1; coef[3 * ph + 2] = (float)c2;
        }
        HIPCHK(hipMemcpyAsync(ws + l.segs + (size_t)2 * B * sizeof(int), o->seg_moff, (size_t)B * sizeof(int), hipMemcpyHostToDevice, stream));
        HIPCHK(launch_put_floats((float *)(ws + l.melc), coef, 3 * LAST_SCALE, stream));
    }
    if (pl.kind == K_GENERIC) {
        GenArgs g;
        memset(&g, 0, sizeof g);
        g.I_T = p->g_I_T; g.I_b = p->I_b; g.w_ih1T = p->w_ih1T; g.w_hh1T = p->w_hh1T; g.b_ih1 = p->b_ih1; g.b_hh1 = p->b_hh1;
        g.w_ih2T = p->g_w_ih2T; g.w_hh2T = p->w_hh2T; g.b_ih2 = p->b_ih2; g.b_hh2 = p->b_hh2;
        g.fc1T = p->g_fc1T; g.fc1_b = p->fc1_b; g.fc2T = p->g_fc2T; g.fc2_b = p->fc2_b; g.fc3T = p->fc3T; g.fc3_b = p->fc3_b;
        g.mels_up = mels_up; g.aux = aux; g.noise = noise; g.force_x = o->force_x; g.out = out; g.dbg_logits = o->logits;
        g.seg_pos = d_pos; g.seg_lim = d_lim;
        if (lib_noise) {
            HIPCHK(launch_noise_fill(mol_mode, B, p->tr.C, 0, T, o->noise_seed, o->noise_seg_id, (float *)(ws + l.nlib), p->tr.n_cus, stream));
            g.noise = (const float *)(ws + l.nlib);
        }
        g.H = p->tr.gH; g.F = p->tr.gF; g.M = p->tr.gM; g.A = p->tr.gA; g.C = p->tr.C; g.B = B; g.T = T; g.hop = hop;
        if ((rc = timer_mark(timer, stream)) != WRNN_OK) return rc;
        HIPCHK(launch_generic(g, p->tr.mode, stream));
        if ((rc = timer_mark(timer, stream)) != WRNN_OK) return rc;
        wrnn_run_info gi;
        memset(&gi, 0, sizeof gi);
        gi.kernel = k.name; gi.rounds = 1; gi.slab_steps = T; gi.launches = 1;
        if (o->info) *o->info = gi;
        return enqueue_progress(o, T, T, B, stream);
    }

    CondArgs c;
    memset(&c, 0, sizeof c);
    c.mels_up = mels_up; c.aux = aux; c.I_cT = p->I_cT; c.I_b = p->I_b; c.c2_wT = p->c2_wT; c.b_ih2 = p->b_ih2;
    c.c3_wT = p->c3_wT; c.fc1_b = p->fc1_b; c.c4_wT = p->c4_wT; c.fc2_b = p->fc2_b;
    c.c2f = (float *)(ws + l.c2f); c.c3f = (float *)(ws + l.c3f); c.c4f = (float *)(ws + l.c4f);
    c.seg_pos = d_pos; c.seg_lim = d_lim;
    c.B = B; c.T = T; c.hop = hop; c.NF = n_frames;
    if (k.slabbed) {
        const long eff = (long)(pl.tab_fps - 2) * hop + 1;
        if (pl.slab > eff) pl.slab = (int)eff;
    } else HIPCHK(launch_cond_frames(c, stream));

    LoopArgs a;
    memset(&a, 0, sizeof a);
    a.I_w0 = p->I_w0; a.w_ih1 = p->w_ih1; a.w_hh1 = p->w_hh1; a.b_ih1 = p->b_ih1; a.b_hh1 = p->b_hh1;
    a.w_ih2 = p->w_ih2; a.w_hh2 = p->w_hh2; a.b_hh2 = p->b_hh2; a.fc1_w = p->fc1_w; a.fc2_w = p->fc2_w;
    a.fc3_w = p->fc3_w; a.fc3_b = p->fc3_b; a.fc3f = p->fc3f; a.u1 = p->u1;
    a.w_ih1T = p->w_ih1T; a.w_hh1T = p->w_hh1T; a.w_ih2T = p->w_ih2T; a.w_hh2T = p->w_hh2T;
    a.fc1T = p->fc1T; a.fc2T = p->fc2T; a.fc3T = p->fc3T;
    a.c2f = c.c2f; a.c3f = c.c3f; a.c4f = c.c4f;
    a.noise = noise; a.force_x = o->force_x; a.out = out; a.dbg_logits = o->logits;
    a.status = (unsigned *)(ws + l.status);
    a.prof = (u64 *)o->phase_clocks;
    a.tuning = o->tuning;
    a.seg_pos = d_pos; a.seg_lim = d_lim;
    a.Btot = B; a.T = T; a.hop = hop; a.NF = n_frames; a.C = p->tr.C;
    a.NG = (B + SEG - 1) / SEG;
    a.Nall = B;
    a.xcc_tab = (unsigned *)(ws + l.xcc);
    a.mels_up = mels_up; a.aux_fr = aux; a.I_cT = p->I_cT; a.I_b = p->I_b;
    a.mel_stage = o->mel_stage; a.seg_moff = d_pos + 2 * B; a.mel_coef = (const float *)(ws + l.melc);
    hop_magic(hop, &a.hop_magic, &a.hop_shift);

    wrnn_run_info info;
    memset(&info, 0, sizeof info);
    info.kernel = k.name; info.units_per_wg = k.units_per_wg;
    info.clusters = pl.ncl; info.depth = pl.G; info.rounds = pl.rounds; info.slab_steps = pl.slab;

    if (k.persistent) {
        a.sp_vals = p->sp_vals; a.sp_cols = p->sp_cols;
        a.sp_fc_vals = (o->tuning & 2048) ? nullptr : p->sp_fc_vals; a.sp_fc_cols = p->sp_fc_cols;
        const bool mol = p->tr.mode == WRNN_MODE_MOL;
        a.xbuf = (float *)(ws + l.xbuf);
        a.cIf = (const float *)(ws + l.cIf);
        a.G = pl.G;
        c.cI = (float *)(ws + l.cIf);
        for (int s0 = pl.t0; s0 < pl.t1; s0 += pl.slab) {
            const int s1 = s0 + pl.slab < pl.t1 ? s0 + pl.slab : pl.t1;
            if (lib_noise) HIPCHK(launch_noise_fill(mol, B, p->tr.C, s0, s1, o->noise_seed, o->noise_seg_id, (float *)(ws + l.nlib), p->tr.n_cus, stream));
            if (mol) {
                const float *const rows = lib_noise ? (const float *)(ws + l.nlib) : noise + (size_t)(s0 - pl.t0) * 11 * B;
                HIPCHK(launch_noise_mol(rows, (float *)(ws + l.npre), (long)(s1 - s0) * 11 * B, B, p->tr.n_cus, stream));
                a.noise_pre = (const float *)(ws + l.npre);
                a.noise_t0 = s0;
            } else if (lib_noise) {
                a.noise = (const float *)(ws + l.nlib);
                a.noise_t0 = s0;
            } else {
                a.noise_t0 = pl.t0;
            }
            if (k.slabbed) {
                c.t0 = s0; c.B = B; c.FPS = pl.tab_fps;
                HIPCHK(launch_cond_frames_slab(c, stream));
                a.tab_fps = pl.tab_fps; a.tab_t0 = s0;
            }
            for (int r = 0; r < pl.rounds; ++r) {
                const int rb0 = (int)(((long)r * B) / pl.rounds), rb1 = (int)(((long)(r + 1) * B) / pl.rounds);
                const int nr = rb1 - rb0;
                if (nr < 1) continue;
                const int ngr = (nr + SEG - 1) / SEG;
                c.t0 = s0; c.t1 = s1; c.rb0 = rb0; c.B = nr; c.NG = ngr;
                if (!k.slabbed) HIPCHK(launch_cond_frag(c, p->tr.n_cus, stream));
                if (!k.slabbed || s0 == 0 || pl.rounds > 1 || (o->tuning & 4)) HIPCHK(hipMemsetAsync(ws + l.xbuf, 0xFF, k.xbuf_fill(pl.G), stream));
                if (k.slabbed) HIPCHK(hipMemsetAsync(ws + l.xcc, 0, XCC_WORDS * sizeof(unsigned), stream));
                a.state = (float *)(ws + l.state) + (size_t)r * k.state_floats(pl.G);
                a.t0 = s0; a.t1 = s1; a.cI_t0 = s0; a.rb0 = rb0; a.Btot = nr; a.NG = ngr; a.resume = s0 > 0 ? 1 : 0;
                a.kind_tag = k.kind_tag;
                if ((rc = timer_mark(timer, stream)) != WRNN_OK) return rc;
                hipError_t e = k.launch(a, pl.ncl, p->tr.sp_nbp, p->tr.mode, stream);
                if (e != hipSuccess) {
                    (void)hipGetLastError();
                    set_err("%s cooperative launch failed: %s", info.kernel, hipGetErrorString(e));
                    return e == hipErrorCooperativeLaunchTooLarge ? WRNN_ERR_RESIDENCY : WRNN_ERR_HIP;
                }
                if ((rc = timer_mark(timer, stream)) != WRNN_OK) return rc;
                info.launches += 1;
            }
            if ((rc = enqueue_progress(o, s1, T, B, stream)) != WRNN_OK) return rc;
        }
    } else {
        c.cI = (float *)(ws + l.cI);
        a.cI = c.cI;
        HIPCHK(launch_cond(c, p->tr.n_cus, o->cond_valu != 0, stream));
        if (lib_noise) {
            HIPCHK(launch_noise_fill(mol_mode, B, p->tr.C, 0, T, o->noise_seed, o->noise_seg_id, (float *)(ws + l.nlib), p->tr.n_cus, stream));
            a.noise = (const float *)(ws + l.nlib);
        }
        a.b0 = 0;
        a.nb = B;
        if ((rc = timer_mark(timer, stream)) != WRNN_OK) return rc;
        HIPCHK(launch_stream(a, p->tr.mode, stream));
        if ((rc = timer_mark(timer, stream)) != WRNN_OK) return rc;
        info.launches = 1;
        if ((rc = enqueue_progress(o, T, T, B, stream)) != WRNN_OK) return rc;
    }
    if (o->info) *o->info = info;
    return WRNN_OK;
}

extern "C" int wrnn_generate(const wrnn_pack *p, const wrnn_geometry *g, const float *mels_up, const float *aux,
                             const float *noise, float *out, void *workspace, size_t workspace_bytes, const wrnn_options *opt,
                             void *stream_)
{
    int rc = check_geometry(g);
    if (rc != WRNN_OK) return rc;
    std::vector<int32_t> pos(g->B), lim(g->B, g->L);
    for (int b = 0; b < g->B; ++b) pos[b] = b * g->stride;
    return wrnn_generate_segments(p, g->B, g->T, pos.data(), lim.data(), g->L, g->hop, g->n_frames, mels_up, aux,
                                  noise, out, workspace, workspace_bytes, opt, stream_);
}

extern "C" int wrnn_status(void *workspace, void *stream)
{
    if (!workspace) { set_err("NULL workspace"); return WRNN_ERR_ARG; }
    HIPCHK(hipStreamSynchronize((hipStream_t)stream));
    unsigned st[STATUS_WORDS];
    HIPCHK(hipMemcpy(st, workspace, sizeof st, hipMemcpyDeviceToHost));
    if (st[0] != 0 || st[1] != 0) {
        set_err("loop kernel gave up: code 0x%x (phase %u) workgroup %u step %u thread %u", st[1], st[1] & 0xff, st[2], st[3], st[4]);
        return WRNN_ERR_KERNEL;
    }
    return WRNN_OK;
}

extern "C" int wrnn_debug_read_exchange(const wrnn_pack *p, void *workspace, int32_t n_segments, int32_t T, int32_t n_frames,
                                        const wrnn_options *opt, int cluster, int slot, int layer, int ring, float *host_out)
{
    if (!p || !workspace || !host_out) { set_err("NULL argument"); return WRNN_ERR_ARG; }
    const wrnn_options whole = whole_call(opt);
    Plan pl;
    int rc = make_plan(&p->tr, n_segments, T, &whole, &pl);
    if (rc != WRNN_OK) return rc;
    if (pl.kind != K_LOOP || cluster < 0 || cluster >= MAXCL || slot < 0 || slot >= LMAXG || layer < 0 || layer >= NXLAYER || ring < 0 || ring >= XRING) {
        set_err("no such exchange layer");
        return WRNN_ERR_ARG;
    }
    const WsLayout l = ws_layout(&p->tr, pl, n_segments, T, n_frames, whole.noise_lib != 0);
    HIPCHK(hipDeviceSynchronize());
    std::vector<float> frag((size_t)SEG * H);
    const size_t off = ((((size_t)cluster * LMAXG + slot) * NXLAYER + layer) * XRING + ring) * SEG * H;
    HIPCHK(hipMemcpy(frag.data(), (char *)workspace + l.xbuf + off * sizeof(float), frag.size() * sizeof(float), hipMemcpyDeviceToHost));
    for (int j = 0; j < SEG; ++j)
        for (int k = 0; k < H; ++k) {
            const int w = k >> 7, r = (k >> 4) & 7, kq = (k >> 2) & 3, e = k & 3;
            host_out[(size_t)j * H + k] = frag[(size_t)(((w * 8 + r) * 64 + kq * 16 + j) * 4 + e)];
        }
    return WRNN_OK;
}

namespace {
int check_noise_fill(int mode, int32_t B, int32_t C, int32_t t0, int32_t t1, const float *out)
{
    if (mode != WRNN_MODE_MOL && mode != WRNN_MODE_RAW) { set_err("unknown mode %d", mode); return WRNN_ERR_ARG; }
    if (!out) { set_err("NULL argument"); return WRNN_ERR_ARG; }
    if (B < 1 || t0 < 0 || t1 <= t0 || (mode == WRNN_MODE_RAW && C < 1)) { set_err("bad noise shape: %d segments, %d classes, steps [%d, %d)", B, C, t0, t1); return WRNN_ERR_ARG; }
    if ((double)(t1 - t0) * B >= 2147483648.0) { set_err("%d steps x %d segments: more than 2^31 - 1 rows in one fill; split the step range", t1 - t0, B); return WRNN_ERR_ARG; }
    return WRNN_OK;
}
}

extern "C" int wrnn_noise_fill(int mode, int32_t n_segments, int32_t n_classes, int32_t t_begin, int32_t t_end, uint64_t seed, const uint64_t *seg_id,
                               float *out, int device, void *stream)
{
    int rc = check_noise_fill(mode, n_segments, n_classes, t_begin, t_end, out);
    if (rc != WRNN_OK) return rc;
    if (((uintptr_t)out & 15) != 0) { set_err("`out` must be 16-byte aligned"); return WRNN_ERR_ARG; }
    const int cus = wrnn_device_cus(device);
    if (cus < 0) return cus;
    DeviceGuard dg(device);
    HIPCHK(dg.err);
    HIPCHK(launch_noise_fill(mode == WRNN_MODE_MOL, n_segments, n_classes, t_begin, t_end, seed, seg_id, out, cus, (hipStream_t)stream));
    return WRNN_OK;
}

extern "C" int wrnn_noise_fill_host(int mode, int32_t n_segments, int32_t n_classes, int32_t t_begin, int32_t t_end, uint64_t seed, const uint64_t *seg_id,
                                    float *out)
{
    const int rc = check_noise_fill(mode, n_segments, n_classes, t_begin, t_end, out);
    if (rc != WRNN_OK) return rc;
    noise_fill_host(mode == WRNN_MODE_MOL, n_segments, n_classes, t_begin, t_end, seed, seg_id, out);
    return WRNN_OK;
}

extern "C" int wrnn_debug_plan(const wrnn_plan_traits *traits, int32_t n_segments, int32_t T, int32_t n_frames,
                               const wrnn_options *opt, wrnn_run_info *out, size_t *workspace_bytes)
{
    if (!traits || !out || !workspace_bytes || n_segments < 1 || T < 1 || n_frames < 1) { set_err("bad argument"); return WRNN_ERR_ARG; }
    *workspace_bytes = 0;
    const wrnn_plan_traits tr = norm_struct(traits);
    return plan_report(&tr, n_segments, T, n_frames, norm_struct(opt), out, workspace_bytes);
}

static float g_selftest_metric = -1.f;
extern "C" float wrnn_selftest_metric(void) { return g_selftest_metric; }

extern "C" int wrnn_selftest(int device, int which)
{
    const int cus = wrnn_device_cus(device);
    if (cus < 0) return cus;
    DeviceGuard dg(device);
    HIPCHK(dg.err);
    char msg[400] = "";
    int rc;
    if (which == 1) rc = selftest_mfma(msg, sizeof msg);
    else if (which == 2) rc = selftest_allgather(cus, msg, sizeof msg, &g_selftest_metric);
    else if (which == 3) rc = selftest_tanh(msg, sizeof msg);
    else if (which == 4) rc = selftest_xor(msg, sizeof msg);
    else { set_err("unknown selftest %d", which); return WRNN_ERR_ARG; }
    if (rc != 0) { set_err("selftest %d failed: %s", which, msg); return WRNN_ERR_KERNEL; }
    set_err("selftest %d ok: %s", which, msg);
    return WRNN_OK;
}
```

### wavernn_amd/csrc/wrnn_cond.hip

```cpp
#include <stdlib.h>
#include <string.h>

#include "wrnn_device.h"

namespace wrnn {


constexpr int CR = 8;

__global__ __launch_bounds__(H) void wrnn_cond_sample_kernel(const CondArgs a)
{
    __shared__ __attribute__((aligned(16))) float in[CR][KCOND];
    const int r = threadIdx.x;
    float wreg[KCOND];
#pragma unroll
    for (int k = 0; k < KCOND; ++k) wreg[k] = a.I_cT[k * H + r];
    const float bias = a.I_b[r];
    const long rows = (long)a.T * a.B;
    for (long base = (long)blockIdx.x * CR; base < rows; base += (long)gridDim.x * CR) {
        __syncthreads();
        for (int q = r; q < CR * KCOND; q += H) {
            const int rr = q / KCOND, k = q % KCOND;
            const long row = base + rr;
            float val = 0.f;
            if (row < rows) {
                const int t = (int)(row / a.B), b = (int)(row % a.B);
                const int p = a.seg_pos[b] + t;
                if (p < a.seg_lim[b]) val = (k < MEL) ? a.mels_up[(size_t)p * MEL + k] : a.aux[(size_t)(p / a.hop) * 4 * AUX + (k - MEL)];
            }
            in[rr][k] = val;
        }
        __syncthreads();
#pragma unroll
        for (int rr = 0; rr < CR; ++rr) {
            float acc = 0.f;
#pragma unroll
            for (int k = 0; k < KCOND; k += 4) {
                const float4 x = *reinterpret_cast<const float4 *>(&in[rr][k]);
                acc = fmaf(wreg[k + 0], x.x, acc);
                acc = fmaf(wreg[k + 1], x.y, acc);
                acc = fmaf(wreg[k + 2], x.z, acc);
                acc = fmaf(wreg[k + 3], x.w, acc);
            }
            if (base + rr < rows) a.cI[(size_t)(base + rr) * H + r] = acc + bias;
        }
    }
}


constexpr int CKB = KCOND / 16;
constexpr int CLD = KCOND + 4;
__global__ __launch_bounds__(256, 1) void wrnn_cond_mfma_kernel(const CondArgs a)
{
    __shared__ __attribute__((aligned(16))) float in[16 * CLD];
    const int tid = threadIdx.x, lane = tid & 63, w = tid >> 6;
    const int fi = lane & 15, kq = lane >> 4;
    float A[8][4 * CKB];
    float4 bias[8];
#pragma unroll
    for (int tt = 0; tt < 8; ++tt) {
        const int row = 128 * w + 16 * tt + fi;
#pragma unroll
        for (int r = 0; r < CKB; ++r)
#pragma unroll
            for (int e = 0; e < 4; ++e) A[tt][4 * r + e] = a.I_cT[(size_t)(16 * r + 4 * kq + e) * H + row];
        bias[tt] = *reinterpret_cast<const float4 *>(a.I_b + 128 * w + 16 * tt + 4 * kq);
    }
    const long rows = (long)a.T * a.B;
    for (long base = (long)blockIdx.x * 16; base < rows; base += (long)gridDim.x * 16) {
        __syncthreads();
        for (int q = tid; q < 16 * KCOND; q += 256) {
            const int rr = q / KCOND, k = q % KCOND;
            const long row = base + rr;
            float val = 0.f;
            if (row < rows) {
                const int t = (int)(row / a.B), b = (int)(row % a.B);
                const int p = a.seg_pos[b] + t;
                if (p < a.seg_lim[b]) val = (k < MEL) ? a.mels_up[(size_t)p * MEL + k] : a.aux[(size_t)(p / a.hop) * 4 * AUX + (k - MEL)];
            }
            in[rr * CLD + k] = val;
        }
        __syncthreads();
        float4 bf[CKB];
#pragma unroll
        for (int r = 0; r < CKB; ++r) bf[r] = *reinterpret_cast<const float4 *>(in + fi * CLD + 16 * r + 4 * kq);
        f32x4 acc[8];
#pragma unroll
        for (int tt = 0; tt < 8; ++tt) acc[tt] = f32x4{0.f, 0.f, 0.f, 0.f};
#pragma unroll
        for (int r = 0; r < CKB; ++r) {
#pragma unroll
            for (int tt = 0; tt < 8; ++tt) acc[tt] = __builtin_amdgcn_mfma_f32_16x16x4f32(A[tt][4 * r + 0], bf[r].x, acc[tt], 0, 0, 0);
#pragma unroll
            for (int tt = 0; tt < 8; ++tt) acc[tt] = __builtin_amdgcn_mfma_f32_16x16x4f32(A[tt][4 * r + 1], bf[r].y, acc[tt], 0, 0, 0);
#pragma unroll
            for (int tt = 0; tt < 8; ++tt) acc[tt] = __builtin_amdgcn_mfma_f32_16x16x4f32(A[tt][4 * r + 2], bf[r].z, acc[tt], 0, 0, 0);
#pragma unroll
            for (int tt = 0; tt < 8; ++tt) acc[tt] = __builtin_amdgcn_mfma_f32_16x16x4f32(A[tt][4 * r + 3], bf[r].w, acc[tt], 0, 0, 0);
        }
        if (base + fi < rows) {
#pragma unroll
            for (int tt = 0; tt < 8; ++tt) {
                const float4 o = make_float4(acc[tt][0] + bias[tt].x, acc[tt][1] + bias[tt].y, acc[tt][2] + bias[tt].z, acc[tt][3] + bias[tt].w);
                *reinterpret_cast<float4 *>(a.cI + (size_t)(base + fi) * H + 128 * w + 16 * tt + 4 * kq) = o;
            }
        }
    }
}

__global__ __launch_bounds__(256, 1) void wrnn_cond_frag_kernel(const CondArgs a)
{
    __shared__ __attribute__((aligned(16))) float in[16 * CLD];
    const int tid = threadIdx.x, lane = tid & 63, w = tid >> 6;
    const int fi = lane & 15, kq = lane >> 4;
    float A[8][4 * CKB];
    float4 bias[8];
#pragma unroll
    for (int tt = 0; tt < 8; ++tt) {
        const int row = 128 * w + 16 * tt + fi;
#pragma unroll
        for (int r = 0; r < CKB; ++r)
#pragma unroll
            for (int e = 0; e < 4; ++e) A[tt][4 * r + e] = a.I_cT[(size_t)(16 * r + 4 * kq + e) * H + row];
        bias[tt] = *reinterpret_cast<const float4 *>(a.I_b + 128 * w + 16 * tt + 4 * kq);
    }
    const long tiles = (long)(a.t1 - a.t0) * a.NG;
    constexpr int NQ = (16 * KCOND + 255) / 256;
    auto gather = [&](long tile, float (&v)[NQ]) {
        const int t = a.t0 + (int)(tile / a.NG), g = (int)(tile % a.NG);
        const int b0 = a.rb0 + (int)(((long)g * a.B) / a.NG), nb = a.rb0 + (int)(((long)(g + 1) * a.B) / a.NG) - b0;
#pragma unroll
        for (int i = 0; i < NQ; ++i) {
            const int q = tid + 256 * i;
            const int rr = q / KCOND, k = q % KCOND;
            float val = 0.f;
            if (q < 16 * KCOND && rr < nb) {
                const int p = a.seg_pos[b0 + rr] + t;
                if (p < a.seg_lim[b0 + rr]) val = (k < MEL) ? a.mels_up[(size_t)p * MEL + k] : a.aux[(size_t)(p / a.hop) * 4 * AUX + (k - MEL)];
            }
            v[i] = val;
        }
    };
    float cur[NQ] = {}, nxt[NQ] = {};
    if (blockIdx.x < tiles) gather(blockIdx.x, cur);
    for (long tile = blockIdx.x; tile < tiles; tile += gridDim.x) {
        __syncthreads();
#pragma unroll
        for (int i = 0; i < NQ; ++i) {
            const int q = tid + 256 * i;
            if (q < 16 * KCOND) in[(q / KCOND) * CLD + q % KCOND] = cur[i];
        }
        __syncthreads();
        if (tile + gridDim.x < tiles) gather(tile + gridDim.x, nxt);
        float4 bf[CKB];
#pragma unroll
        for (int r = 0; r < CKB; ++r) bf[r] = *reinterpret_cast<const float4 *>(in + fi * CLD + 16 * r + 4 * kq);
        f32x4 acc[8];
#pragma unroll
        for (int tt = 0; tt < 8; ++tt) acc[tt] = f32x4{0.f, 0.f, 0.f, 0.f};
#pragma unroll
        for (int r = 0; r < CKB; ++r) {
#pragma unroll
            for (int tt = 0; tt < 8; ++tt) acc[tt] = __builtin_amdgcn_mfma_f32_16x16x4f32(A[tt][4 * r + 0], bf[r].x, acc[tt], 0, 0, 0);
#pragma unroll
            for (int tt = 0; tt < 8; ++tt) acc[tt] = __builtin_amdgcn_mfma_f32_16x16x4f32(A[tt][4 * r + 1], bf[r].y, acc[tt], 0, 0, 0);
#pragma unroll
            for (int tt = 0; tt < 8; ++tt) acc[tt] = __builtin_amdgcn_mfma_f32_16x16x4f32(A[tt][4 * r + 2], bf[r].z, acc[tt], 0, 0, 0);
#pragma unroll
            for (int tt = 0; tt < 8; ++tt) acc[tt] = __builtin_amdgcn_mfma_f32_16x16x4f32(A[tt][4 * r + 3], bf[r].w, acc[tt], 0, 0, 0);
        }
        float4 *dst = reinterpret_cast<float4 *>(a.cI + (size_t)tile * (SEG * H)) + (w * 8) * 64 + lane;
#pragma unroll
        for (int tt = 0; tt < 8; ++tt)
            dst[tt * 64] = make_float4(acc[tt][0] + bias[tt].x, acc[tt][1] + bias[tt].y, acc[tt][2] + bias[tt].z, acc[tt][3] + bias[tt].w);
#pragma unroll
        for (int i = 0; i < NQ; ++i) cur[i] = nxt[i];
    }
}

__global__ __launch_bounds__(H) void wrnn_cond_frame_kernel(const CondArgs a)
{
    __shared__ float ax[4 * AUX];
    const int f = blockIdx.x, r = threadIdx.x;
    if (r < 4 * AUX) ax[r] = (f < a.NF) ? a.aux[(size_t)f * 4 * AUX + r] : 0.f;
    __syncthreads();
    float g0 = 0.f, g1 = 0.f, g2 = 0.f, y3 = 0.f, y4 = 0.f;
#pragma unroll 8
    for (int k = 0; k < AUX; ++k) {
        g0 = fmaf(a.c2_wT[k * 3 * H + r], ax[AUX + k], g0);
        g1 = fmaf(a.c2_wT[k * 3 * H + H + r], ax[AUX + k], g1);
        g2 = fmaf(a.c2_wT[k * 3 * H + 2 * H + r], ax[AUX + k], g2);
        y3 = fmaf(a.c3_wT[k * H + r], ax[2 * AUX + k], y3);
        y4 = fmaf(a.c4_wT[k * H + r], ax[3 * AUX + k], y4);
    }
    a.c2f[(size_t)f * 3 * H + r] = g0 + a.b_ih2[r];
    a.c2f[(size_t)f * 3 * H + H + r] = g1 + a.b_ih2[H + r];
    a.c2f[(size_t)f * 3 * H + 2 * H + r] = g2 + a.b_ih2[2 * H + r];
    a.c3f[(size_t)f * H + r] = y3 + a.fc1_b[r];
    a.c4f[(size_t)f * H + r] = y4 + a.fc2_b[r];
}

__global__ __launch_bounds__(H) void wrnn_cond_frame_slab_kernel(const CondArgs a)
{
    __shared__ float ax[4 * AUX];
    const int row = blockIdx.x, r = threadIdx.x;
    int f = a.NF;
    if (row < a.B * a.FPS) {
        const int b = row / a.FPS, j = row % a.FPS;
        f = (a.seg_pos[b] + a.t0) / a.hop + j;
    }
    if (r < 4 * AUX) ax[r] = (f < a.NF) ? a.aux[(size_t)f * 4 * AUX + r] : 0.f;
    __syncthreads();
    float g0 = 0.f, g1 = 0.f, g2 = 0.f, y3 = 0.f, y4 = 0.f;
#pragma unroll 8
    for (int k = 0; k < AUX; ++k) {
        g0 = fmaf(a.c2_wT[k * 3 * H + r], ax[AUX + k], g0);
        g1 = fmaf(a.c2_wT[k * 3 * H + H + r], ax[AUX + k], g1);
        g2 = fmaf(a.c2_wT[k * 3 * H + 2 * H + r], ax[AUX + k], g2);
        y3 = fmaf(a.c3_wT[k * H + r], ax[2 * AUX + k], y3);
        y4 = fmaf(a.c4_wT[k * H + r], ax[3 * AUX + k], y4);
    }
    a.c2f[(size_t)row * 3 * H + r] = g0 + a.b_ih2[r];
    a.c2f[(size_t)row * 3 * H + H + r] = g1 + a.b_ih2[H + r];
    a.c2f[(size_t)row * 3 * H + 2 * H + r] = g2 + a.b_ih2[2 * H + r];
    a.c3f[(size_t)row * H + r] = y3 + a.fc1_b[r];
    a.c4f[(size_t)row * H + r] = y4 + a.fc2_b[r];
}

__global__ __launch_bounds__(256) void wrnn_noise_mol_kernel(const float *__restrict__ in, float *__restrict__ out, long n, int B)
{
    const long stride = (long)gridDim.x * blockDim.x;
    for (long i = (long)blockIdx.x * blockDim.x + threadIdx.x; i < n; i += stride) {
        const float u = in[i];
        const int col = (int)(i % (11L * B));
        out[i] = (col < 10 * B) ? logf(-logf(u)) : (logf(u) - logf(1.0f - u));
    }
}

hipError_t launch_noise_mol(const float *in, float *out, long n, int B, int n_cus, hipStream_t stream)
{
    long blocks = (n + 255) / 256;
    if (blocks > (long)n_cus * 8) blocks = (long)n_cus * 8;
    if (blocks < 1) blocks = 1;
    hipLaunchKernelGGL(wrnn_noise_mol_kernel, dim3((unsigned)blocks), dim3(256), 0, stream, in, out, n, B);
    return hipGetLastError();
}

hipError_t launch_cond_frames(const CondArgs &a, hipStream_t stream)
{
    hipLaunchKernelGGL(wrnn_cond_frame_kernel, dim3(a.NF + 1), dim3(H), 0, stream, a);
    return hipGetLastError();
}

hipError_t launch_cond_frames_slab(const CondArgs &a, hipStream_t stream)
{
    hipLaunchKernelGGL(wrnn_cond_frame_slab_kernel, dim3(a.B * a.FPS + 1), dim3(H), 0, stream, a);
    return hipGetLastError();
}

struct PutFloats { float v[64]; };
__global__ void wrnn_put_floats_kernel(float *dst, PutFloats src, int n)
{
    if ((int)threadIdx.x < n) dst[threadIdx.x] = src.v[threadIdx.x];
}
hipError_t launch_put_floats(float *dst, const float *src, int n, hipStream_t stream)
{
    if (n < 1 || n > 64) return hipErrorInvalidValue;
    PutFloats p;
    for (int i = 0; i < 64; ++i) p.v[i] = i < n ? src[i] : 0.f;
    hipLaunchKernelGGL(wrnn_put_floats_kernel, dim3(1), dim3(64), 0, stream, dst, p, n);
    return hipGetLastError();
}

hipError_t launch_cond_frag(const CondArgs &a, int n_cus, hipStream_t stream)
{
    long blocks = (long)(a.t1 - a.t0) * a.NG;
    if (blocks > n_cus) blocks = n_cus;
    if (blocks < 1) blocks = 1;
    hipLaunchKernelGGL(wrnn_cond_frag_kernel, dim3((unsigned)blocks), dim3(256), 0, stream, a);
    return hipGetLastError();
}

hipError_t launch_cond(const CondArgs &a, int n_cus, bool valu, hipStream_t stream)
{
    const long rows = (long)a.T * a.B;
    if (valu) {
        long blocks = (rows + CR - 1) / CR;
        const long cap = (long)n_cus * 4;
        if (blocks > cap) blocks = cap;
        if (blocks < 1) blocks = 1;
        hipLaunchKernelGGL(wrnn_cond_sample_kernel, dim3((unsigned)blocks), dim3(H), 0, stream, a);
    } else {
        long blocks = (rows + 15) / 16;
        if (blocks > n_cus) blocks = n_cus;
        if (blocks < 1) blocks = 1;
        hipLaunchKernelGGL(wrnn_cond_mfma_kernel, dim3((unsigned)blocks), dim3(256), 0, stream, a);
    }
    return hipGetLastError();
}

}
```

### wavernn_amd/csrc/wrnn_pre.hip

```cpp
#include <math.h>
#include <stdio.h>
#include <string.h>
#include <vector>

#include "wrnn_device.h"
#include "../../include/wavernn_amd.h"

namespace wrnn {

constexpr int PC = 128;
constexpr int PFEAT = MEL;
constexpr int PK = 5;
constexpr int PPAD = 2;
constexpr int PKIN = PFEAT * PK;
constexpr int PLDI = 516;
constexpr int PLDX = 132;
constexpr int PNF = 16;

struct PreArgs {
    const float *mel;
    const float *conv_in_w;
    const float *bn_in;
    const float *res_w;
    const float *res_bn;
    const float *conv_out_w;
    const float *conv_out_b;
    float *aux;
    int N, blocks;
};

__device__ __forceinline__ f32x4 pre_tile(const float *W, int ld, int kvalid, int row0, int nchunks, const float *act, int lda,
                                          int lane)
{
    const int fi = lane & 15, kq = lane >> 4;
    f32x4 total = {0.f, 0.f, 0.f, 0.f};
    for (int kc = 0; kc < nchunks; ++kc) {
        float a[AF];
#pragma unroll
        for (int r = 0; r < AF / 4; ++r) {
            const int col = kc * 128 + 16 * r + 4 * kq;
            float4 v = make_float4(0.f, 0.f, 0.f, 0.f);
            if (col < kvalid) v = *reinterpret_cast<const float4 *>(W + (size_t)(row0 + fi) * ld + col);
            a[4 * r + 0] = v.x; a[4 * r + 1] = v.y; a[4 * r + 2] = v.z; a[4 * r + 3] = v.w;
        }
        const f32x4 part = mfma_tile(a, act + fi * lda + kc * 128 + 4 * kq);
        total = (kc == 0) ? part : total + part;
    }
    return total;
}

__global__ __launch_bounds__(256) void wrnn_resnet_kernel(const PreArgs a)
{
    __shared__ __attribute__((aligned(16))) float XIN[PNF * PLDI];
    __shared__ __attribute__((aligned(16))) float XA[PNF * PLDX];
    __shared__ __attribute__((aligned(16))) float XB[PNF * PLDX];
    const int tid = threadIdx.x, lane = tid & 63, w = tid >> 6;
    const int j0 = blockIdx.x * PNF;
    const int N = a.N;
    for (int q = tid; q < PNF * PLDI; q += 256) {
        const int j = q / PLDI, k = q % PLDI;
        float v = 0.f;
        if (k < PKIN) {
            const int c = k / PK, t = k % PK;
            const int f = j0 + j + t - PPAD;
            if (f >= 0 && f < N && j0 + j < N) v = a.mel[(size_t)c * N + f];
        }
        XIN[q] = v;
    }
    __syncthreads();
    const int fi = lane & 15, rq = (lane >> 4) * 4;
#pragma unroll
    for (int tt = 0; tt < 2; ++tt) {
        const int row0 = 32 * w + 16 * tt;
        const f32x4 d = pre_tile(a.conv_in_w, PKIN, PKIN, row0, 4, XIN, PLDI, lane);
        const float4 s = *reinterpret_cast<const float4 *>(a.bn_in + row0 + rq);
        const float4 t = *reinterpret_cast<const float4 *>(a.bn_in + PC + row0 + rq);
        float4 y;
        y.x = fmaxf(fmaf(d[0], s.x, t.x), 0.f); y.y = fmaxf(fmaf(d[1], s.y, t.y), 0.f);
        y.z = fmaxf(fmaf(d[2], s.z, t.z), 0.f); y.w = fmaxf(fmaf(d[3], s.w, t.w), 0.f);
        *reinterpret_cast<float4 *>(XA + fi * PLDX + row0 + rq) = y;
    }
    __syncthreads();
    for (int b = 0; b < a.blocks; ++b) {
        const float *W1 = a.res_w + (size_t)(2 * b) * PC * PC, *W2 = W1 + PC * PC;
        const float *bn1 = a.res_bn + (size_t)(2 * b) * 2 * PC, *bn2 = bn1 + 2 * PC;
#pragma unroll
        for (int tt = 0; tt < 2; ++tt) {
            const int row0 = 32 * w + 16 * tt;
            const f32x4 d = pre_tile(W1, PC, PC, row0, 1, XA, PLDX, lane);
            const float4 s = *reinterpret_cast<const float4 *>(bn1 + row0 + rq);
            const float4 t = *reinterpret_cast<const float4 *>(bn1 + PC + row0 + rq);
            float4 y;
            y.x = fmaxf(fmaf(d[0], s.x, t.x), 0.f); y.y = fmaxf(fmaf(d[1], s.y, t.y), 0.f);
            y.z = fmaxf(fmaf(d[2], s.z, t.z), 0.f); y.w = fmaxf(fmaf(d[3], s.w, t.w), 0.f);
            *reinterpret_cast<float4 *>(XB + fi * PLDX + row0 + rq) = y;
        }
        __syncthreads();
        f32x4 d2[2];
#pragma unroll
        for (int tt = 0; tt < 2; ++tt) d2[tt] = pre_tile(W2, PC, PC, 32 * w + 16 * tt, 1, XB, PLDX, lane);
#pragma unroll
        for (int tt = 0; tt < 2; ++tt) {
            const int row0 = 32 * w + 16 * tt;
            const float4 s = *reinterpret_cast<const float4 *>(bn2 + row0 + rq);
            const float4 t = *reinterpret_cast<const float4 *>(bn2 + PC + row0 + rq);
            float4 r = *reinterpret_cast<float4 *>(XA + fi * PLDX + row0 + rq);
            r.x += fmaf(d2[tt][0], s.x, t.x); r.y += fmaf(d2[tt][1], s.y, t.y);
            r.z += fmaf(d2[tt][2], s.z, t.z); r.w += fmaf(d2[tt][3], s.w, t.w);
            *reinterpret_cast<float4 *>(XA + fi * PLDX + row0 + rq) = r;
        }
        __syncthreads();
    }
#pragma unroll
    for (int tt = 0; tt < 2; ++tt) {
        const int row0 = 32 * w + 16 * tt;
        const f32x4 d = pre_tile(a.conv_out_w, PC, PC, row0, 1, XA, PLDX, lane);
        const float4 bo = *reinterpret_cast<const float4 *>(a.conv_out_b + row0 + rq);
        if (j0 + fi < N)
            *reinterpret_cast<float4 *>(a.aux + (size_t)(j0 + fi) * PC + row0 + rq) = make_float4(d[0] + bo.x, d[1] + bo.y, d[2] + bo.z, d[3] + bo.w);
    }
}

struct GenPreArgs {
    PreArgs p;
    int feat, C, R, pad, gf;
};
__global__ __launch_bounds__(256) void wrnn_resnet_generic_kernel(const GenPreArgs g)
{
    extern __shared__ __attribute__((aligned(16))) float gsm[];
    const PreArgs &a = g.p;
    const int feat = g.feat, C = g.C, R = g.R, pad = g.pad, GF = g.gf, K = 2 * pad + 1, WW = GF + 2 * pad;
    float *MW = gsm, *XA = MW + feat * WW, *XB = XA + GF * C;
    const int tid = threadIdx.x, N = a.N;
    const int j0 = blockIdx.x * GF;
    for (int q = tid; q < feat * WW; q += 256) {
        const int c = q / WW, f = j0 + q % WW - pad;
        MW[q] = (f >= 0 && f < N) ? a.mel[(size_t)c * N + f] : 0.f;
    }
    __syncthreads();
    for (int o = tid; o < C * GF; o += 256) {
        const int c = o / GF, j = o % GF;
        const float *wr = a.conv_in_w + (size_t)c * feat * K;
        float acc = 0.f;
        for (int ci = 0; ci < feat; ++ci)
            for (int t = 0; t < K; ++t) acc = fmaf(wr[ci * K + t], MW[ci * WW + j + t], acc);
        XA[j * C + c] = fmaxf(fmaf(acc, a.bn_in[c], a.bn_in[C + c]), 0.f);
    }
    __syncthreads();
    for (int b = 0; b < a.blocks; ++b) {
        const float *W1 = a.res_w + (size_t)(2 * b) * C * C, *W2 = W1 + (size_t)C * C;
        const float *bn1 = a.res_bn + (size_t)(2 * b) * 2 * C, *bn2 = bn1 + 2 * C;
        for (int o = tid; o < C * GF; o += 256) {
            const int c = o / GF, j = o % GF;
            float acc = 0.f;
            for (int k = 0; k < C; ++k) acc = fmaf(W1[(size_t)c * C + k], XA[j * C + k], acc);
            XB[j * C + c] = fmaxf(fmaf(acc, bn1[c], bn1[C + c]), 0.f);
        }
        __syncthreads();
        for (int o = tid; o < C * GF; o += 256) {
            const int c = o / GF, j = o % GF;
            float acc = 0.f;
            for (int k = 0; k < C; ++k) acc = fmaf(W2[(size_t)c * C + k], XB[j * C + k], acc);
            XA[j * C + c] += fmaf(acc, bn2[c], bn2[C + c]);
        }
        __syncthreads();
    }
    for (int o = tid; o < R * GF; o += 256) {
        const int r = o / GF, j = o % GF;
        float acc = 0.f;
        for (int k = 0; k < C; ++k) acc = fmaf(a.conv_out_w[(size_t)r * C + k], XA[j * C + k], acc);
        if (j0 + j < N) a.aux[(size_t)(j0 + j) * R + r] = acc + a.conv_out_b[r];
    }
}

template <bool FIRST, bool LAST, int S, int F = PFEAT>
__global__ __launch_bounds__(256) void wrnn_upstage_kernel(const float *__restrict__ in, float *__restrict__ out,
                                                           const float *__restrict__ taps, int n_in, int s_rt, int pad, int indent, int feat_rt = PFEAT)
{
    const int s = S > 0 ? S : s_rt;
    const int feat = F > 0 ? F : feat_rt;
    const long n_out = (long)n_in * s;
    const long total = LAST ? (n_out - 2L * indent) * feat : n_out * feat;
    const int ld_in = FIRST ? n_in - 2 * pad : n_in;
    for (long idx = (long)blockIdx.x * blockDim.x + threadIdx.x; idx < total; idx += (long)gridDim.x * blockDim.x) {
        int c;
        long q;
        if (LAST) { c = (int)(idx % feat); q = idx / feat + indent; }
        else { c = (int)(idx / n_out); q = idx % n_out; }
        float acc = 0.f;
#pragma unroll
        for (int j = 0; j <= 2 * s; ++j) {
            const long u = q + j - s;
            float v = 0.f;
            if (u >= 0 && u < n_out) {
                int f = (int)(u / s);
                if (FIRST) { f -= pad; v = (f >= 0 && f < ld_in) ? in[(size_t)c * ld_in + f] : 0.f; }
                else v = in[(size_t)c * ld_in + f];
            }
            acc = fmaf(taps[j], v, acc);
        }
        if (LAST) out[(size_t)(q - indent) * feat + c] = acc;
        else out[(size_t)c * n_out + q] = acc;
    }
}

template <int S>
__global__ __launch_bounds__(256) void wrnn_upstage_last_kernel(const float *__restrict__ in, float *__restrict__ out,
                                                                const float *__restrict__ taps, int n_in, int s_rt, int indent)
{
    constexpr int TQ = 64;
    __shared__ float tile[TQ][PFEAT + 1];
    const int s = S > 0 ? S : s_rt;
    const long n_out = (long)n_in * s, nq = n_out - 2L * indent;
    for (long q0 = (long)blockIdx.x * TQ; q0 < nq; q0 += (long)gridDim.x * TQ) {
        for (int e = threadIdx.x; e < TQ * PFEAT; e += 256) {
            const int c = e / TQ, ql = e % TQ;
            const long q = q0 + ql + indent;
            float acc = 0.f;
            if (q0 + ql < nq) {
#pragma unroll
                for (int j = 0; j <= 2 * s; ++j) {
                    const long u = q + j - s;
                    float v = 0.f;
                    if (u >= 0 && u < n_out) v = in[(size_t)c * n_in + (int)(u / s)];
                    acc = fmaf(taps[j], v, acc);
                }
            }
            tile[ql][c] = acc;
        }
        __syncthreads();
        for (int e = threadIdx.x; e < TQ * PFEAT; e += 256) {
            const int ql = e / PFEAT, c = e % PFEAT;
            if (q0 + ql < nq) out[(size_t)(q0 + ql) * PFEAT + c] = tile[ql][c];
        }
        __syncthreads();
    }
}

}

using namespace wrnn;

static thread_local char g_pre_err[384] = "";
extern "C" const char *wrnn_pre_last_error(void) { return g_pre_err; }
#define PRE_FAIL(code, ...)                                  \
    do {                                                     \
        snprintf(g_pre_err, sizeof g_pre_err, __VA_ARGS__);  \
        return code;                                         \
    } while (0)
#define PRE_HIP(expr)                                                                                   \
    do {                                                                                                \
        hipError_t e_ = (expr);                                                                         \
        if (e_ != hipSuccess) PRE_FAIL(WRNN_ERR_HIP, "%s failed: %s", #expr, hipGetErrorString(e_));    \
    } while (0)

struct wrnn_pre {
    int device, blocks, scales[3], total_scale;
    int feat, C, R, pad;
    int gf;
    float *dev;
    const float *conv_in_w, *bn_in, *res_w, *res_bn, *conv_out_w, *conv_out_b, *taps[3];
};

static size_t generic_lds_bytes(int feat, int C, int pad, int gf) { return ((size_t)feat * (gf + 2 * pad) + 2 * (size_t)gf * C) * sizeof(float); }

extern "C" int wrnn_pre_create(const wrnn_pre_weights *w, int device, wrnn_pre **out)
{
    if (!w || !out) PRE_FAIL(WRNN_ERR_ARG, "NULL argument");
    if (w->feat_dims < 1 || w->feat_dims > 4096 || w->compute_dims < 1 || w->compute_dims > 4096 || w->res_out_dims < 1 || w->res_out_dims > 4096 ||
        w->pad < 0 || w->pad > 64 || w->res_blocks < 0 || w->res_blocks > 64)
        PRE_FAIL(WRNN_ERR_ARG, "bad UpsampleNetwork dims: feat_dims %d, compute_dims %d, res_out_dims %d, pad %d, res_blocks %d", w->feat_dims,
                 w->compute_dims, w->res_out_dims, w->pad, w->res_blocks);
    for (int i = 0; i < 3; ++i)
        if (w->upsample_factors[i] < 1 || w->upsample_factors[i] > 64) PRE_FAIL(WRNN_ERR_ARG, "bad upsample factor %d", w->upsample_factors[i]);
    if (!w->conv_in_w || !w->bn_in || (w->res_blocks && (!w->res_w || !w->res_bn)) || !w->conv_out_w || !w->conv_out_b || !w->up_w)
        PRE_FAIL(WRNN_ERR_ARG, "NULL weight pointer");
    const int FE = w->feat_dims, C = w->compute_dims, R = w->res_out_dims, PD = w->pad, KT = 2 * PD + 1;
    const bool shipped_dims = FE == PFEAT && C == PC && R == PC && PD == PPAD;
    int gf = 0;
    if (!shipped_dims) {
        for (gf = 16; gf >= 1 && generic_lds_bytes(FE, C, PD, gf) > 65536; gf >>= 1) {}
        if (gf < 1) PRE_FAIL(WRNN_ERR_ARG, "UpsampleNetwork too wide for the pre-loop kernel (feat_dims %d, compute_dims %d, pad %d)", FE, C, PD);
    }
    int n = 0;
    if (hipGetDeviceCount(&n) != hipSuccess || n <= 0 || device >= n) PRE_FAIL(WRNN_ERR_NO_DEVICE, "no HIP device %d (count %d)", device, n);
    DeviceGuard dg(device);
    PRE_HIP(dg.err);
    const int B = w->res_blocks;
    const double eps = 1e-5;
    std::vector<float> h;
    auto put = [&](const float *src, size_t cnt) { size_t o = (h.size() + 63) / 64 * 64; h.resize(o + cnt); if (src) memcpy(h.data() + o, src, cnt * 4); return o; };
    auto fold = [&](const float *bn, size_t o) {
        for (int c = 0; c < C; ++c) {
            const float s = bn[c] / sqrtf(bn[3 * C + c] + (float)eps);
            h[o + c] = s;
            h[o + C + c] = bn[C + c] - bn[2 * C + c] * s;
        }
    };
    const size_t o_cin = put(w->conv_in_w, (size_t)C * FE * KT);
    const size_t o_bnin = put(nullptr, 2 * (size_t)C);
    fold(w->bn_in, o_bnin);
    const size_t o_resw = put(w->res_w, (size_t)B * 2 * C * C);
    const size_t o_resbn = put(nullptr, (size_t)B * 2 * 2 * C);
    for (int i = 0; i < 2 * B; ++i) fold(w->res_bn + (size_t)i * 4 * C, o_resbn + (size_t)i * 2 * C);
    const size_t o_cow = put(w->conv_out_w, (size_t)R * C), o_cob = put(w->conv_out_b, R);
    size_t o_t[3], toff = 0;
    for (int i = 0; i < 3; ++i) { o_t[i] = put(w->up_w + toff, 2 * w->upsample_factors[i] + 1); toff += 2 * w->upsample_factors[i] + 1; }
    put(nullptr, 64);
    wrnn_pre *p = new wrnn_pre();
    p->device = device; p->blocks = B; p->total_scale = 1;
    p->feat = FE; p->C = C; p->R = R; p->pad = PD; p->gf = gf;
    for (int i = 0; i < 3; ++i) { p->scales[i] = w->upsample_factors[i]; p->total_scale *= w->upsample_factors[i]; }
    hipError_t e = hipMalloc((void **)&p->dev, h.size() * 4);
    if (e != hipSuccess) { delete p; PRE_FAIL(WRNN_ERR_HIP, "hipMalloc failed: %s", hipGetErrorString(e)); }
    e = hipMemcpy(p->dev, h.data(), h.size() * 4, hipMemcpyHostToDevice);
    if (e != hipSuccess) { (void)hipFree(p->dev); delete p; PRE_FAIL(WRNN_ERR_HIP, "hipMemcpy failed: %s", hipGetErrorString(e)); }
    p->conv_in_w = p->dev + o_cin; p->bn_in = p->dev + o_bnin; p->res_w = p->dev + o_resw; p->res_bn = p->dev + o_resbn;
    p->conv_out_w = p->dev + o_cow; p->conv_out_b = p->dev + o_cob;
    for (int i = 0; i < 3; ++i) p->taps[i] = p->dev + o_t[i];
    *out = p;
    return WRNN_OK;
}

extern "C" void wrnn_pre_destroy(wrnn_pre *p)
{
    if (!p) return;
    (void)hipFree(p->dev);
    delete p;
}

extern "C" int wrnn_pre_hop(const wrnn_pre *p) { return p ? p->total_scale : 0; }

extern "C" size_t wrnn_pre_workspace_bytes(const wrnn_pre *p, int32_t n_frames)
{
    if (!p || n_frames < 1) return 0;
    const size_t nf = (size_t)n_frames + 2 * p->pad;
    return (nf * p->scales[0] + nf * p->scales[0] * p->scales[1]) * p->feat * sizeof(float) + 512;
}

static int pre_run(const wrnn_pre *p, const float *mel, int32_t n_frames, float *mels_up, float *aux,
                   void *workspace, size_t workspace_bytes, void *stream_, bool rows_only)
{
    if (!p || !mel || !mels_up || !aux || !workspace) PRE_FAIL(WRNN_ERR_ARG, "NULL argument");
    if (n_frames < 1 || (double)n_frames * p->total_scale > 2.0e9) PRE_FAIL(WRNN_ERR_ARG, "bad n_frames %d", n_frames);
    if (workspace_bytes < wrnn_pre_workspace_bytes(p, n_frames)) PRE_FAIL(WRNN_ERR_WORKSPACE, "workspace too small");
    if (((uintptr_t)workspace & 255) != 0) PRE_FAIL(WRNN_ERR_ARG, "workspace must be 256-byte aligned");
    hipStream_t stream = (hipStream_t)stream_;
    DeviceGuard dg(p->device);
    PRE_HIP(dg.err);
    PreArgs a;
    a.mel = mel; a.conv_in_w = p->conv_in_w; a.bn_in = p->bn_in; a.res_w = p->res_w; a.res_bn = p->res_bn;
    a.conv_out_w = p->conv_out_w; a.conv_out_b = p->conv_out_b; a.aux = aux; a.N = n_frames; a.blocks = p->blocks;
    const int FE = p->feat, PD = p->pad;
    if (p->gf == 0) hipLaunchKernelGGL(wrnn_resnet_kernel, dim3((n_frames + PNF - 1) / PNF), dim3(256), 0, stream, a);
    else {
        GenPreArgs g;
        g.p = a; g.feat = FE; g.C = p->C; g.R = p->R; g.pad = PD; g.gf = p->gf;
        hipLaunchKernelGGL(wrnn_resnet_generic_kernel, dim3((n_frames + p->gf - 1) / p->gf), dim3(256), generic_lds_bytes(FE, p->C, PD, p->gf), stream, g);
    }
    const int nf = n_frames + 2 * PD;
    float *s1 = (float *)workspace;
    float *s2 = s1 + (size_t)nf * p->scales[0] * FE;
    auto grid = [](long total) { long b = (total + 255) / 256; return (unsigned)(b > 65535 ? 65535 : (b < 1 ? 1 : b)); };
    const bool feat80 = FE == PFEAT;
    const bool shipped = feat80 && PD == PPAD && p->scales[0] == 5 && p->scales[1] == 5 && p->scales[2] == 11;
    const unsigned g1 = grid((long)nf * p->scales[0] * FE), g2 = grid((long)nf * p->scales[0] * p->scales[1] * FE);
    const unsigned g3 = grid((long)n_frames * p->total_scale * 4);
    const int n2 = nf * p->scales[0], n3 = n2 * p->scales[1], indent = PD * p->total_scale;
    if (rows_only) {
        if (shipped) {
            hipLaunchKernelGGL((wrnn_upstage_kernel<true, false, 5>), dim3(g1), dim3(256), 0, stream, mel, s1, p->taps[0], nf, 5, PD, 0, PFEAT);
            hipLaunchKernelGGL((wrnn_upstage_kernel<false, true, 5>), dim3(g2), dim3(256), 0, stream, s1, mels_up, p->taps[1], n2, 5, 0, 0, PFEAT);
        } else {
            hipLaunchKernelGGL((wrnn_upstage_kernel<true, false, 0, 0>), dim3(g1), dim3(256), 0, stream, mel, s1, p->taps[0], nf, p->scales[0], PD, 0, FE);
            hipLaunchKernelGGL((wrnn_upstage_kernel<false, true, 0, 0>), dim3(g2), dim3(256), 0, stream, s1, mels_up, p->taps[1], n2, p->scales[1], 0, 0, FE);
        }
    } else if (shipped) {
        hipLaunchKernelGGL((wrnn_upstage_kernel<true, false, 5>), dim3(g1), dim3(256), 0, stream, mel, s1, p->taps[0], nf, 5, PD, 0, PFEAT);
        hipLaunchKernelGGL((wrnn_upstage_kernel<false, false, 5>), dim3(g2), dim3(256), 0, stream, s1, s2, p->taps[1], n2, 5, 0, 0, PFEAT);
        hipLaunchKernelGGL((wrnn_upstage_last_kernel<11>), dim3(g3), dim3(256), 0, stream, s2, mels_up, p->taps[2], n3, 11, indent);
    } else {
        hipLaunchKernelGGL((wrnn_upstage_kernel<true, false, 0, 0>), dim3(g1), dim3(256), 0, stream, mel, s1, p->taps[0], nf, p->scales[0], PD, 0, FE);
        hipLaunchKernelGGL((wrnn_upstage_kernel<false, false, 0, 0>), dim3(g2), dim3(256), 0, stream, s1, s2, p->taps[1], n2, p->scales[1], 0, 0, FE);
        if (feat80) hipLaunchKernelGGL((wrnn_upstage_last_kernel<0>), dim3(g3), dim3(256), 0, stream, s2, mels_up, p->taps[2], n3, p->scales[2], indent);
        else hipLaunchKernelGGL((wrnn_upstage_kernel<false, true, 0, 0>), dim3(grid((long)n_frames * p->total_scale * FE)), dim3(256), 0, stream, s2, mels_up, p->taps[2], n3, p->scales[2], 0, indent, FE);
    }
    PRE_HIP(hipGetLastError());
    return WRNN_OK;
}

extern "C" int wrnn_pre_upsample(const wrnn_pre *p, const float *mel, int32_t n_frames, float *mels_up, float *aux,
                                 void *workspace, size_t workspace_bytes, void *stream)
{
    return pre_run(p, mel, n_frames, mels_up, aux, workspace, workspace_bytes, stream, false);
}

extern "C" int wrnn_pre_upsample_rows(const wrnn_pre *p, const float *mel, int32_t n_frames, float *mel_rows, float *aux,
                                      void *workspace, size_t workspace_bytes, void *stream)
{
    return pre_run(p, mel, n_frames, mel_rows, aux, workspace, workspace_bytes, stream, true);
}
```

### wavernn_amd/model.py

```python
import sys
import time
from pathlib import Path
from typing import Union

import numpy as np
import torch
import torch.nn as nn
import torch.nn.functional as F

from . import _lib
from . import fold as _fold
from .dsp import save_wav
from .engine import LoopEngine, LOOP_KEYS, RESUMABLE_KERNELS, MEL_STAGE_KERNELS
from .rng import burn_ctor_draws, draw_steps


class ResBlock(nn.Module):

    def __init__(self, dims):
        super().__init__()
        self.conv1 = nn.Conv1d(dims, dims, kernel_size=1, bias=False)
        self.conv2 = nn.Conv1d(dims, dims, kernel_size=1, bias=False)
        self.batch_norm1 = nn.BatchNorm1d(dims)
        self.batch_norm2 = nn.BatchNorm1d(dims)

    def forward(self, x):
        y = F.relu(self.batch_norm1(self.conv1(x)))
        return x + self.batch_norm2(self.conv2(y))


class MelResNet(nn.Module):

    def __init__(self, res_blocks, in_dims, compute_dims, res_out_dims, pad):
        super().__init__()
        self.conv_in = nn.Conv1d(in_dims, compute_dims, kernel_size=2 * pad + 1, bias=False)
        self.batch_norm = nn.BatchNorm1d(compute_dims)
        self.layers = nn.ModuleList([ResBlock(compute_dims) for _ in range(res_blocks)])
        self.conv_out = nn.Conv1d(compute_dims, res_out_dims, kernel_size=1)

    def forward(self, x):
        x = F.relu(self.batch_norm(self.conv_in(x)))
        for layer in self.layers:
            x = layer(x)
        return self.conv_out(x)


class Stretch2d(nn.Module):

    def __init__(self, x_scale, y_scale):
        super().__init__()
        self.x_scale, self.y_scale = x_scale, y_scale

    def forward(self, x):
        return x.repeat_interleave(self.y_scale, dim=2).repeat_interleave(self.x_scale, dim=3)


class UpsampleNetwork(nn.Module):

    def __init__(self, feat_dims, upsample_scales, compute_dims, res_blocks, res_out_dims, pad):
        super().__init__()
        self.total_scale = int(np.prod(upsample_scales))
        self.indent = pad * self.total_scale
        self.resnet = MelResNet(res_blocks, feat_dims, compute_dims, res_out_dims, pad)
        self.resnet_stretch = Stretch2d(self.total_scale, 1)
        self.up_layers = nn.ModuleList()
        for scale in upsample_scales:
            conv = nn.Conv2d(1, 1, kernel_size=(1, 2 * scale + 1), padding=(0, scale), bias=False)
            conv.weight.data.fill_(1. / (2 * scale + 1))
            self.up_layers.append(Stretch2d(scale, 1))
            self.up_layers.append(conv)

    def aux_frames(self, m):
        return self.resnet(m)

    def upsample_mel(self, m):
        m = m.unsqueeze(1)
        for f in self.up_layers:
            m = f(m)
        return m.squeeze(1)[:, :, self.indent:-self.indent].transpose(1, 2)

    def forward(self, m):
        aux = self.resnet_stretch(self.aux_frames(m).unsqueeze(1)).squeeze(1)
        return self.upsample_mel(m), aux.transpose(1, 2)


class WaveRNN(nn.Module):
    def __init__(self, rnn_dims, fc_dims, bits, pad, upsample_factors, feat_dims, compute_dims, res_out_dims,
                 res_blocks, hop_length, sample_rate, mode='RAW'):
        super().__init__()
        self.mode = mode
        self.pad = pad
        if self.mode == 'RAW':
            self.n_classes = 2 ** bits
        elif self.mode == 'MOL':
            self.n_classes = 30
        else:
            RuntimeError("Unknown model mode value - ", self.mode)
        self.rnn_dims = rnn_dims
        self.aux_dims = res_out_dims // 4
        self.hop_length = hop_length
        self.sample_rate = sample_rate

        self.upsample = UpsampleNetwork(feat_dims, upsample_factors, compute_dims, res_blocks, res_out_dims, pad)
        self.I = nn.Linear(feat_dims + self.aux_dims + 1, rnn_dims)
        self.rnn1 = nn.GRU(rnn_dims, rnn_dims, batch_first=True)
        self.rnn2 = nn.GRU(rnn_dims + self.aux_dims, rnn_dims, batch_first=True)
        self.fc1 = nn.Linear(rnn_dims + self.aux_dims, fc_dims)
        self.fc2 = nn.Linear(fc_dims + self.aux_dims, fc_dims)
        self.fc3 = nn.Linear(fc_dims, self.n_classes)
        self.register_buffer('step', torch.zeros(1, dtype=torch.long))
        self.num_params()

        self.noise_source = 'cpu'
        self.noise_seed = 0
        self.noise_key = 0
        self.loop_algo = 'auto'
        self.sparse_groups = None
        self.pre_algo = 'native'
        self.pre_streams = 8
        self.pinned_output = True
        self.mel_in_loop = None
        self.post_algo = 'native'
        self.noise_chunk_bytes = 2 << 30
        self.progress_callback = None
        self._engine = None
        self._engine_key = None
        self._pre = None
        self._pre_key = None
        self.last_loop_ms = None
        self.last_loop_kernel = None

    def forward(self, x, mels):
        self.step += 1
        bsize = x.size(0)
        device = x.device
        h1 = torch.zeros(1, bsize, self.rnn_dims, device=device)
        h2 = torch.zeros(1, bsize, self.rnn_dims, device=device)
        mels, aux = self.upsample(mels)
        d = self.aux_dims
        a1, a2, a3, a4 = (aux[:, :, d * i:d * (i + 1)] for i in range(4))
        x = self.I(torch.cat([x.unsqueeze(-1), mels, a1], dim=2))
        res = x
        x, _ = self.rnn1(x, h1)
        x = x + res
        res = x
        x, _ = self.rnn2(torch.cat([x, a2], dim=2), h2)
        x = x + res
        x = F.relu(self.fc1(torch.cat([x, a3], dim=2)))
        x = F.relu(self.fc2(torch.cat([x, a4], dim=2)))
        return self.fc3(x)

    def invalidate_engines(self):
        self._engine = self._pre = self._engine_key = self._pre_key = None

    @staticmethod
    def _weights_key(sd):
        return tuple((k, v.data_ptr(), str(v.device), tuple(v.shape), str(v.dtype), int(v._version)) for k, v in sorted(sd.items()))

    def _loop_engine(self):
        sd = {k: v for k, v in self.state_dict().items() if k in LOOP_KEYS.values()}
        key = self._weights_key(sd)
        if self._engine is None or key != self._engine_key:
            dev = next(self.parameters()).device
            self._engine = LoopEngine(sd, self.mode, device=dev)
            self._engine_key = key
        return self._engine

    def _pre_engine(self):
        from .pre import PreEngine
        sd = {k: v for k, v in self.state_dict().items() if k.startswith('upsample.')}
        key = self._weights_key(sd)
        if self._pre is None or key != self._pre_key:
            self._pre = PreEngine(sd, device=next(self.parameters()).device)
            self._pre_key = key
        return self._pre

    @staticmethod
    def _require_hip_device(device):
        if device.type != 'cuda':
            raise RuntimeError('wavernn_amd.WaveRNN.generate needs the model on a HIP device (model.to("cuda")); '
                               'there is no CPU path in this package')

    def mel_rows_ok(self, eng, n_segments, T):
        device = next(self.parameters()).device
        in_loop = bool(self.mel_in_loop)
        if not (in_loop and self.pre_algo == 'native' and device.type == 'cuda'):
            return False
        if eng.plan(n_segments, T, algo=self.loop_algo)['kernel'] not in MEL_STAGE_KERNELS:
            return False
        try:
            pre = self._pre_engine()
            return pre.scales[2] == 11 and pre.pad >= 1
        except _lib.WrnnError:
            return False

    def loop_sparse_groups(self, eng, n_segments, T):
        groups = int(self.sparse_groups or 0)
        if groups <= 1 or eng.plan(n_segments, T, algo=self.loop_algo)['kernel'] != 'wrnn_sparse_kernel':
            return 0
        return groups

    def conditioning(self, mels, rows=False):
        device = next(self.parameters()).device
        mels = torch.as_tensor(mels, device=device)
        wave_len = (mels.size(-1) - 1) * self.hop_length
        if rows:
            from .engine import MelRows
            pre = self._pre_engine()
            mel_rows, aux = pre.upsample_rows(mels.float())
            return MelRows(mel_rows, mels.size(-1) * self.hop_length, pre.scales[2], pre.last_taps, self.pad * self.hop_length), aux, wave_len
        if self.pre_algo == 'native' and device.type == 'cuda':
            try:
                mels_up, aux = self._pre_engine().upsample(mels.float())
                return mels_up, aux, wave_len
            except _lib.WrnnError as e:
                if 'too wide for the pre-loop kernel' not in str(e):
                    raise
                import warnings
                warnings.warn(f'wavernn_amd: {e}; up-sampling with the PyTorch-ROCm modules instead')
                self.pre_algo = 'torch'
        m = _fold.pad_tensor(mels.transpose(1, 2), pad=self.pad, side='both').transpose(1, 2)
        mels_up = self.upsample.upsample_mel(m)[0].contiguous()
        aux = self.upsample.aux_frames(m)[0].transpose(0, 1).contiguous()
        return mels_up, aux, wave_len

    def generate(self, mels, save_path: Union[str, Path], batched, target, overlap, mu_law):
        self.eval()
        device = next(self.parameters()).device
        self._require_hip_device(device)
        if self.mode not in ('RAW', 'MOL'):
            raise RuntimeError("Unknown model mode value - ", self.mode)
        mu_law = mu_law if self.mode == 'RAW' else False

        with torch.no_grad():
            L = int(torch.as_tensor(mels).size(-1)) * self.hop_length
            if batched:
                B, _ = _fold.fold_geometry(L, target, overlap)
                T, stride = target + 2 * overlap, target + overlap
            else:
                B, T, stride = 1, L, 0
            eng = self._loop_engine()
            rows = self.mel_rows_ok(eng, B, T)
            try:
                mels_up, aux, wave_len = self.conditioning(mels, rows=rows)
            except _lib.WrnnError:
                if not rows:
                    raise
                rows = False
                mels_up, aux, wave_len = self.conditioning(mels)
            assert (mels_up.L if rows else mels_up.size(0)) == L
            burn_ctor_draws(self.rnn_dims, self.aux_dims, self.noise_source)
            per_step = B * (11 if self.mode == 'MOL' else self.n_classes) * 4
            resumable = eng.plan(B, T, algo=self.loop_algo)['kernel'] in RESUMABLE_KERNELS
            chunk = max(1, min(T, self.noise_chunk_bytes // per_step)) if (resumable and self.noise_source != 'library') else T
            chunk = -(-T // (-(-T // chunk)))
            rng_state = torch.get_rng_state() if (self.noise_source == 'cpu' and (chunk < T or rows)) else None
            algo = self.loop_algo
            groups = self.loop_sparse_groups(eng, B, T)
            import warnings
            try:
                out = self._run_sliced(eng, mels_up, aux, B, T, stride, chunk, algo, device, groups)
            except _lib.ResidencyError as e:
                if rng_state is not None:
                    torch.set_rng_state(rng_state)
                if rows:
                    warnings.warn(f'wavernn_amd: {e}; up-sampling the mel in full for the other loop kernels')
                    mels_up, aux, _ = self.conditioning(mels)
                    try:
                        out = self._run_sliced(eng, mels_up, aux, B, T, stride, chunk, algo, device, groups)
                        e = None
                    except _lib.ResidencyError as e2:
                        e = e2
                        if rng_state is not None:
                            torch.set_rng_state(rng_state)
                if e is not None:
                    warnings.warn(f'wavernn_amd: {e}; using the stream kernel')
                    out = self._run_sliced(eng, mels_up, aux, B, T, stride, T, 'stream', device)
            self.last_loop_ms = eng.last_loop_ms()
            self.last_loop_kernel = eng.last_loop_kernel()

        if self.post_algo == 'native':
            from .post import unfold_on_device
            wav, _ = unfold_on_device(out, [0], [B], [wave_len], overlap, self.hop_length, self.n_classes, mu_law, batched)
            output = wav.cpu().numpy()
        else:
            output = out.cpu().numpy().astype(np.float64)
            if mu_law:
                output = _fold.decode_mu_law(output, self.n_classes, False)
            if batched:
                output = _fold.xfade_and_unfold(output, target, overlap)
            else:
                output = output[0]
            output = _fold.finish_waveform(output, wave_len, self.hop_length)
        save_wav(output, save_path, self.sample_rate)
        self.train()
        return output

    def _run_sliced(self, eng, mels_up, aux, B, T, stride, chunk, algo, device, sparse_groups=0):
        out = None
        prog = None
        if self.progress_callback is not None:
            t_start, cb = time.perf_counter(), self.progress_callback
            prog = lambda done, T_, n_: cb(done, T_, n_, time.perf_counter() - t_start)
        if self.noise_source == 'library':
            from .batch import library_seg_ids
            return eng.run(mels_up, aux, B, T, stride, None, self.hop_length, algo=algo, progress=prog, sparse_groups=sparse_groups,
                           noise_seed=self.noise_key, noise_seg_id=library_seg_ids(self.noise_seed, B))
        for t0 in range(0, T, chunk):
            t1 = min(T, t0 + chunk)
            noise = draw_steps(self.mode, B, t1 - t0, self.n_classes, device, self.noise_source)
            out = eng.run(mels_up, aux, B, T, stride, noise, self.hop_length, algo=algo, out=out,
                          t_range=None if (t0 == 0 and t1 == T) else (t0, t1), progress=prog, sparse_groups=sparse_groups)
        return out

    def gen_display(self, i, seq_len, b_size, gen_rate):
        bar_len = 16
        done = (i * bar_len) // max(1, seq_len)
        pbar = ''.join(chr(0x2588) if k < done else chr(0x2591) for k in range(bar_len))
        msg = f'| {pbar} {i * b_size}/{seq_len * b_size} | Batch Size: {b_size} | Gen Rate: {gen_rate:.1f}kHz | '
        sys.stdout.write(f'\r{msg}')

    def pad_tensor(self, x, pad, side='both'):
        return _fold.pad_tensor(x, pad, side)

    def fold_with_overlap(self, x, target, overlap):
        return _fold.fold_with_overlap(x, target, overlap)

    def xfade_and_unfold(self, y, target, overlap):
        return _fold.xfade_and_unfold(y, target, overlap)

    def get_step(self):
        return self.step.data.item()

    def log(self, path, msg):
        with open(path, 'a') as f:
            print(msg, file=f)

    def load(self, path: Union[str, Path]):
        device = next(self.parameters()).device
        self.load_state_dict(torch.load(path, map_location=device), strict=False)

    def save(self, path: Union[str, Path]):
        torch.save(self.state_dict(), path)

    def num_params(self, print_out=True):
        n = sum(int(np.prod(p.size())) for p in self.parameters() if p.requires_grad) / 1_000_000
        if print_out:
            print('Trainable Parameters: %.3fM' % n)
        return n
```

### wavernn_amd/post.py

```python
import numpy as np
import torch

from . import _lib
from . import fold as _fold

_tables = {}


def _fade_tables(overlap, hop, device):
    key = ('fade', overlap, hop, str(device))
    if key not in _tables:
        silence_len = overlap // 2
        fade_len = overlap - silence_len
        t = np.linspace(-1, 1, fade_len, dtype=np.float64)
        fade_in = np.concatenate([np.zeros(silence_len, np.float64), np.sqrt(0.5 * (1 + t))])
        fade_out = np.concatenate([np.ones(silence_len, np.float64), np.sqrt(0.5 * (1 - t))])
        tail = np.linspace(1, 0, 20 * hop)
        _tables[key] = tuple(torch.from_numpy(np.ascontiguousarray(x)).to(device) for x in (fade_in, fade_out, tail))
    return _tables[key]


def _mu_law_lut(n_classes, device):
    key = ('lut', n_classes, str(device))
    if key not in _tables:
        idx = np.arange(n_classes, dtype=np.float32)
        y32 = np.float32(2.0) * idx / np.float32(n_classes - 1) - np.float32(1.0)
        lut = _fold.decode_mu_law(y32.astype(np.float64), n_classes, False)
        _tables[key] = torch.from_numpy(np.ascontiguousarray(lut, dtype=np.float64)).to(device)
    return _tables[key]


def unfold_on_device(segments, first, folds, wave_lens, overlap, hop, n_classes, mu_law, batched=True):
    dev = segments.device
    tail_len = 20 * hop
    if min(wave_lens) < tail_len:
        raise ValueError(f'operands could not be broadcast together with shapes ({min(wave_lens)},) ({tail_len},)')
    L = _lib.lib()
    n_utt, T = len(wave_lens), int(segments.shape[1])
    off = np.concatenate([[0], np.cumsum(wave_lens)]).astype(np.int64)
    tabs = torch.from_numpy(np.concatenate([np.asarray(first, np.int32), np.asarray(folds, np.int32)])).to(dev)
    d_off = torch.from_numpy(off).to(dev)
    fade_in, fade_out, tail = _fade_tables(overlap if batched else 0, hop, dev)
    lut = _mu_law_lut(n_classes, dev) if mu_law else None
    out = torch.empty(int(off[-1]), dtype=torch.float64, device=dev)
    segments = segments.contiguous()
    stream = torch.cuda.current_stream(dev).cuda_stream
    rc = L.wrnn_post_unfold(segments.data_ptr(), T, n_utt, tabs.data_ptr(), tabs.data_ptr() + 4 * n_utt, d_off.data_ptr(),
                            lut.data_ptr() if lut is not None else None, n_classes, fade_in.data_ptr(), fade_out.data_ptr(),
                            overlap if batched else 0, tail.data_ptr(), tail_len, 1 if batched else 0, out.data_ptr(), stream)
    if rc != 0:
        raise _lib.WrnnError(f'wrnn_post_unfold failed (rc={rc}): {L.wrnn_post_last_error().decode()}')
    return out, [(int(off[u]), int(off[u + 1])) for u in range(n_utt)]
```

### wavernn_amd/pre.py

```python
import ctypes

import numpy as np
import torch

from . import _lib


def _f32(v):
    if isinstance(v, torch.Tensor):
        v = v.detach().to('cpu', torch.float32).numpy()
    return np.ascontiguousarray(v, dtype=np.float32)


class PreEngine:

    def __init__(self, state_dict, device=None):
        if not torch.cuda.is_available():
            raise _lib.WrnnError('wavernn_amd needs a HIP device; there is no CPU fallback')
        self.lib = _lib.lib()
        self.device = torch.device('cuda', torch.cuda.current_device()) if device is None else torch.device(device)
        sd = state_dict
        conv_in = _f32(sd['upsample.resnet.conv_in.weight'])
        C, feat, k = conv_in.shape
        blocks = 0
        while f'upsample.resnet.layers.{blocks}.conv1.weight' in sd:
            blocks += 1
        bn = lambda p: np.stack([_f32(sd[p + s]) for s in ('.weight', '.bias', '.running_mean', '.running_var')])
        res_w = np.stack([np.stack([_f32(sd[f'upsample.resnet.layers.{i}.conv{j}.weight'])[:, :, 0] for j in (1, 2)])
                          for i in range(blocks)]) if blocks else np.zeros((0, 2, C, C), np.float32)
        res_bn = np.stack([np.stack([bn(f'upsample.resnet.layers.{i}.batch_norm{j}') for j in (1, 2)])
                           for i in range(blocks)]) if blocks else np.zeros((0, 2, 4, C), np.float32)
        conv_out_w = _f32(sd['upsample.resnet.conv_out.weight'])[:, :, 0]
        ups = [_f32(sd[f'upsample.up_layers.{2 * i + 1}.weight']).reshape(-1) for i in range(3)]
        scales = [(u.shape[0] - 1) // 2 for u in ups]
        host = dict(conv_in_w=np.ascontiguousarray(conv_in.reshape(C, feat * k)), bn_in=np.ascontiguousarray(bn('upsample.resnet.batch_norm')),
                    res_w=np.ascontiguousarray(res_w), res_bn=np.ascontiguousarray(res_bn), conv_out_w=np.ascontiguousarray(conv_out_w),
                    conv_out_b=_f32(sd['upsample.resnet.conv_out.bias']), up_w=np.ascontiguousarray(np.concatenate(ups)))
        w = _lib.PreWeights()
        w.feat_dims, w.compute_dims, w.res_out_dims, w.res_blocks, w.pad = feat, C, conv_out_w.shape[0], blocks, (k - 1) // 2
        for i in range(3):
            w.upsample_factors[i] = scales[i]
        for name, arr in host.items():
            setattr(w, name, arr.ctypes.data)
        self.feat_dims, self.res_out_dims = int(feat), int(conv_out_w.shape[0])
        self.pad, self.scales, self.last_taps = int(w.pad), [int(s_) for s_ in scales], ups[2].copy()
        pre = ctypes.c_void_p()
        rc = self.lib.wrnn_pre_create(ctypes.byref(w), (self.device.index if self.device.index is not None else torch.cuda.current_device()), ctypes.byref(pre))
        if rc != 0:
            raise _lib.WrnnError(f'wrnn_pre_create failed (rc={rc}): {self.lib.wrnn_pre_last_error().decode()}')
        self._pre = pre
        self.hop = int(self.lib.wrnn_pre_hop(pre))
        self._ws = None

    def __del__(self):
        try:
            if getattr(self, '_pre', None):
                self.lib.wrnn_pre_destroy(self._pre)
                self._pre = None
        except Exception:
            pass

    def upsample_rows(self, mel, rows=None, aux=None):
        return self.upsample(mel, mels_up=rows, aux=aux, _rows=True)

    def rows_of(self, n_frames):
        return (int(n_frames) + 2 * self.pad) * self.scales[0] * self.scales[1]

    def upsample(self, mel, mels_up=None, aux=None, _rows=False):
        if mel.dim() == 3:
            mel = mel[0]
        mel = mel.to(self.device, torch.float32).contiguous()
        n = int(mel.shape[1])
        if mel.shape[0] != self.feat_dims:
            raise ValueError(f'Expected a mel shaped ({self.feat_dims}, n_hops), but got {tuple(mel.shape)}!')
        n_out = self.rows_of(n) if _rows else n * self.hop
        if mels_up is None:
            mels_up = torch.empty(n_out, self.feat_dims, dtype=torch.float32, device=self.device)
        if aux is None:
            aux = torch.empty(n, self.res_out_dims, dtype=torch.float32, device=self.device)
        assert mels_up.is_contiguous() and aux.is_contiguous() and mels_up.shape == (n_out, self.feat_dims)
        nbytes = int(self.lib.wrnn_pre_workspace_bytes(self._pre, n))
        stream = torch.cuda.current_stream(self.device).cuda_stream
        if self._ws is None:
            self._ws = {}
        ws = self._ws.get(stream)
        if ws is None or ws.numel() < nbytes:
            ws = self._ws[stream] = torch.empty(nbytes, dtype=torch.uint8, device=self.device)
        fn = self.lib.wrnn_pre_upsample_rows if _rows else self.lib.wrnn_pre_upsample
        rc = fn(self._pre, mel.data_ptr(), n, mels_up.data_ptr(), aux.data_ptr(), ws.data_ptr(), ws.numel(), stream)
        if rc != 0:
            raise _lib.WrnnError(f'wrnn_pre_upsample failed (rc={rc}): {self.lib.wrnn_pre_last_error().decode()}')
        return mels_up, aux

    def upsample_many(self, jobs, rows=False, streams=8):
        if streams <= 1 or len(jobs) <= 1:
            for mel, up, aux in jobs:
                self.upsample(mel, mels_up=up, aux=aux, _rows=rows)
            return
        cur = torch.cuda.current_stream(self.device)
        if getattr(self, '_side', None) is None or len(self._side) < streams:
            self._side = [torch.cuda.Stream(device=self.device) for _ in range(streams)]
        mels = [mel[0] if mel.dim() == 3 else mel for mel, _, _ in jobs]
        mels = [m.to(self.device, torch.float32).contiguous() for m in mels]
        fork = cur.record_event()
        used = self._side[:min(streams, len(jobs))]
        for s in used:
            s.wait_event(fork)
        for k, (m, (_, up, aux)) in enumerate(zip(mels, jobs)):
            with torch.cuda.stream(used[k % len(used)]):
                self.upsample(m, mels_up=up, aux=aux, _rows=rows)
        for s in used:
            cur.wait_stream(s)
```

Baseline: 11.14 million.

## Batch mel upsampling into one launch set, fuse slab prep, prebuild unfold tables

Adds a multi-utterance upsample path that runs the resnet and upsample stages for all utterances in a single sequence of kernel launches, driven by a device-side table, in place of many per-utterance launches spread over several streams. It also fuses the MoL noise transform, the slab conditioning projection and the xcc-counter clear into one slab-prep kernel, which removes a separate launch and a memset per slab. Post-processing unfold tables are now built and uploaded before generation so that transfer can overlap the work, rather than being built afterwards. The risks are extra host table construction and a less flexible code path.

```diff
diff --git a/include/wavernn_amd.h b/include/wavernn_amd.h
--- a/include/wavernn_amd.h
+++ b/include/wavernn_amd.h
@@ -176,6 +176,17 @@
                       void *workspace, size_t workspace_bytes, void *stream);
 int wrnn_pre_upsample_rows(const wrnn_pre *p, const float *mel, int32_t n_frames, float *mel_rows, float *aux,
                            void *workspace, size_t workspace_bytes, void *stream);
+typedef struct wrnn_pre_utt {
+    const float *mel;
+    int32_t n_frames;
+    int32_t reserved;
+    int64_t up_row;
+    int64_t aux_row;
+} wrnn_pre_utt;
+size_t wrnn_pre_workspace_bytes_many(const wrnn_pre *p, const wrnn_pre_utt *utts, int32_t n_utt, int32_t rows_only);
+int wrnn_pre_upsample_many(const wrnn_pre *p, const wrnn_pre_utt *utts, int32_t n_utt, int32_t rows_only, float *mels_up, float *aux,
+                           void *workspace, size_t workspace_bytes, void *stream);
+int wrnn_pre_debug_host_handle(const wrnn_pre_weights *w, wrnn_pre **out);
 const char *wrnn_pre_last_error(void);
 
 int wrnn_post_unfold(const float *segments, int32_t T, int32_t n_utt, const int32_t *first, const int32_t *folds,
diff --git a/wavernn_amd/_lib.py b/wavernn_amd/_lib.py
--- a/wavernn_amd/_lib.py
+++ b/wavernn_amd/_lib.py
@@ -19,7 +19,8 @@
            'wrnn_pack_weight_bytes', 'wrnn_pack_sparse_blocks', 'wrnn_pack_sparse_fc_blocks', 'wrnn_workspace_bytes', 'wrnn_workspace_bytes_segments', 'wrnn_generate',
            'wrnn_generate_segments', 'wrnn_noise_fill', 'wrnn_noise_fill_host', 'wrnn_plan_segments', 'wrnn_status', 'wrnn_timer_create', 'wrnn_timer_destroy', 'wrnn_timer_ms',
            'wrnn_timer_launches', 'wrnn_debug_read_exchange', 'wrnn_debug_plan', 'wrnn_selftest', 'wrnn_selftest_metric', 'wrnn_pre_create',
-           'wrnn_pre_destroy', 'wrnn_pre_hop', 'wrnn_pre_workspace_bytes', 'wrnn_pre_upsample', 'wrnn_pre_upsample_rows', 'wrnn_pre_last_error',
+           'wrnn_pre_destroy', 'wrnn_pre_hop', 'wrnn_pre_workspace_bytes', 'wrnn_pre_upsample', 'wrnn_pre_upsample_rows', 'wrnn_pre_workspace_bytes_many',
+           'wrnn_pre_upsample_many', 'wrnn_pre_debug_host_handle', 'wrnn_pre_last_error',
            'wrnn_post_unfold', 'wrnn_post_last_error', 'wrnn_taco_workspace_bytes', 'wrnn_taco_decode', 'wrnn_taco_status',
            'wrnn_taco_last_error', 'wrnn_bigru', 'wrnn_taco_front_create', 'wrnn_taco_front_destroy', 'wrnn_taco_front_workspace_bytes',
            'wrnn_taco_encode', 'wrnn_taco_postnet', 'wrnn_taco_batch_workspace_bytes', 'wrnn_taco_decode_batch']
@@ -35,6 +36,11 @@
     _fields_ = [(n, ctypes.c_int32) for n in ('feat_dims', 'compute_dims', 'res_out_dims', 'res_blocks', 'pad')] + \
                [('upsample_factors', ctypes.c_int32 * 3)] + \
                [(n, ctypes.c_void_p) for n in ('conv_in_w', 'bn_in', 'res_w', 'res_bn', 'conv_out_w', 'conv_out_b', 'up_w')]
+
+
+class PreUtt(ctypes.Structure):
+    _fields_ = [('mel', ctypes.c_void_p), ('n_frames', ctypes.c_int32), ('reserved', ctypes.c_int32), ('up_row', ctypes.c_int64),
+                ('aux_row', ctypes.c_int64)]
 
 
 TACO_WEIGHT_FIELDS = ('prenet_fc1_w', 'prenet_fc1_b', 'prenet_fc2_w', 'prenet_fc2_b', 'attn_rnn_w_ih', 'attn_rnn_w_hh', 'attn_rnn_b_ih',
@@ -205,6 +211,11 @@
     L.wrnn_pre_upsample.argtypes = [ctypes.c_void_p, ctypes.c_void_p, ctypes.c_int32, ctypes.c_void_p, ctypes.c_void_p,
                                     ctypes.c_void_p, ctypes.c_size_t, ctypes.c_void_p]
     L.wrnn_pre_upsample_rows.argtypes = L.wrnn_pre_upsample.argtypes
+    L.wrnn_pre_workspace_bytes_many.argtypes = [ctypes.c_void_p, ctypes.POINTER(PreUtt), ctypes.c_int32, ctypes.c_int32]
+    L.wrnn_pre_workspace_bytes_many.restype = ctypes.c_size_t
+    L.wrnn_pre_upsample_many.argtypes = [ctypes.c_void_p, ctypes.POINTER(PreUtt), ctypes.c_int32, ctypes.c_int32, ctypes.c_void_p, ctypes.c_void_p,
+                                         ctypes.c_void_p, ctypes.c_size_t, ctypes.c_void_p]
+    L.wrnn_pre_debug_host_handle.argtypes = [ctypes.POINTER(PreWeights), ctypes.POINTER(ctypes.c_void_p)]
     L.wrnn_pre_last_error.restype = ctypes.c_char_p
     L.wrnn_post_unfold.argtypes = [ctypes.c_void_p, ctypes.c_int32, ctypes.c_int32, ctypes.c_void_p, ctypes.c_void_p, ctypes.c_void_p,
                                    ctypes.c_void_p, ctypes.c_int32, ctypes.c_void_p, ctypes.c_void_p, ctypes.c_int32,
diff --git a/wavernn_amd/batch.py b/wavernn_amd/batch.py
--- a/wavernn_amd/batch.py
+++ b/wavernn_amd/batch.py
@@ -188,6 +188,23 @@
 
     out_local = torch.zeros(n_max, plan.T, dtype=torch.float32, device=device)
     native_pre = loop_fn is None and getattr(model, 'pre_algo', 'torch') == 'native' and device.type == 'cuda'
+    n_utt = len(frames)
+    mine_u = [u for u in range(n_utt) if finish != 'own' or (lo <= plan.first[u] < hi)]
+    local_u = [u for u in mine_u if lo <= plan.first[u] and plan.first[u] + plan.folds[u] <= hi]
+    local_set = set(local_u)
+    rest_u = [u for u in mine_u if u not in local_set]
+    native_post = loop_fn is None and getattr(model, 'post_algo', 'numpy') == 'native' and out_local.is_cuda
+    slab_tuning = 8192 if getattr(model, 'slab_prep_split', False) else 0
+
+    def unfold_args(us, first_of):
+        return ([first_of(u) for u in us], [int(plan.folds[u]) for u in us], [(frames[u] - 1) * hop for u in us], overlap, hop, model.n_classes, mu_law, True)
+    first_local, first_all = (lambda u: int(plan.first[u]) - lo), (lambda u: int(plan.first[u]))
+    early = {}
+    if native_post and not return_segments and getattr(model, 'post_tables_early', True):
+        from .post import prepare_unfold
+        for us, first_of in ((local_u, first_local), (rest_u, first_all)):
+            if us and not (shard is not None and first_of is first_all):
+                early[first_of] = prepare_unfold(*unfold_args(us, first_of), device=device)
     with torch.no_grad():
         for utts, clo, chi in (chunk_utterances(plan, lo, hi, max_segments_per_launch) if hi > lo else []):
             noise = [None] * len(mels)
@@ -212,7 +229,8 @@
                             r0 += n_rows[k]
                         else:
                             jobs.append((mels[u], mels_up[a0:a0 + frames[u] * hop], aux[a0 // hop:a0 // hop + frames[u]]))
-                    pre.upsample_many(jobs, rows=rows, streams=int(getattr(model, 'pre_streams', 8)))
+                    pre.upsample_many(jobs, rows=rows, streams=int(getattr(model, 'pre_streams', 8)),
+                                      batched=bool(getattr(model, 'pre_batched', True)))
                     if rows:
                         from .engine import MelRows
                         indent, order = pre.pad * hop, {u: k for k, u in enumerate(utts)}
@@ -279,7 +297,7 @@
                 for t0 in range(0, T, steps):
                     t1 = min(T, t0 + steps)
                     eng.run_segments(mels_up, aux, seg_pos, seg_lim, T, draw(t1 - t0), hop, algo=model.loop_algo, check=check, out=out_view,
-                                     t_range=None if (t0 == 0 and t1 == T) else (t0, t1), sparse_groups=groups, **lib_kw)
+                                     t_range=None if (t0 == 0 and t1 == T) else (t0, t1), sparse_groups=groups, tuning=slab_tuning, **lib_kw)
             except ResidencyError as e:
                 import warnings
                 warnings.warn(f'wavernn_amd: {e}; redoing the chunk unsliced on the next kernel')
@@ -288,7 +306,7 @@
                 for u in gens:
                     gens[u].manual_seed(int(seeds[u]))
                     burn_ctor_draws(model.rnn_dims, model.aux_dims, 'cpu', gens[u])
-                eng.run_segments(mels_up, aux, seg_pos, seg_lim, T, draw(T), hop, algo=model.loop_algo, check=check, out=out_view, sparse_groups=groups, **lib_kw)
+                eng.run_segments(mels_up, aux, seg_pos, seg_lim, T, draw(T), hop, algo=model.loop_algo, check=check, out=out_view, sparse_groups=groups, tuning=slab_tuning, **lib_kw)
             finally:
                 if pool is not None:
                     pool.shutdown()
@@ -319,20 +337,14 @@
         model.train()
     if return_segments:
         return gathered_segments().cpu().numpy().astype(np.float64), plan
-    mine_u = [u for u in range(n_utt) if finish != 'own' or (lo <= plan.first[u] < hi)]
-    local_u = [u for u in mine_u if lo <= plan.first[u] and plan.first[u] + plan.folds[u] <= hi]
-    local_set = set(local_u)
-    rest_u = [u for u in mine_u if u not in local_set]
     outs = [None] * n_utt
-    native_post = loop_fn is None and getattr(model, 'post_algo', 'numpy') == 'native' and out_local.is_cuda
 
     def unfold(segs, first_of, us):
         if not us:
             return
         if native_post:
             from .post import unfold_on_device
-            wav, sl = unfold_on_device(segs, [first_of(u) for u in us], [int(plan.folds[u]) for u in us],
-                                       [(frames[u] - 1) * hop for u in us], overlap, hop, model.n_classes, mu_law, True)
+            wav, sl = unfold_on_device(segs, *unfold_args(us, first_of), tables=early.get(first_of))
             if getattr(model, 'pinned_output', True):
                 host = torch.empty(wav.shape, dtype=wav.dtype, pin_memory=True)
                 host.copy_(wav, non_blocking=True)
@@ -352,13 +364,13 @@
             outs[u] = _fold.finish_waveform(y, (frames[u] - 1) * hop, hop)
 
     t_u = time.perf_counter()
-    unfold(out_local, lambda u: int(plan.first[u]) - lo, local_u)
+    unfold(out_local, first_local, local_u)
     if timings is not None:
         timings['unfold_under_gather_ms'] = timings.get('unfold_under_gather_ms', 0.0) + (time.perf_counter() - t_u) * 1e3
     if shard is not None:
         return outs
     if rest_u:
-        unfold(gathered_segments(), lambda u: int(plan.first[u]), rest_u)
+        unfold(gathered_segments(), first_all, rest_u)
     elif work is not None:
         t_w = time.perf_counter()
         work.wait()
diff --git a/wavernn_amd/csrc/wrnn_abi.hip b/wavernn_amd/csrc/wrnn_abi.hip
--- a/wavernn_amd/csrc/wrnn_abi.hip
+++ b/wavernn_amd/csrc/wrnn_abi.hip
@@ -14,6 +14,7 @@
 hipError_t launch_cond(const CondArgs &a, int n_cus, bool valu, hipStream_t stream);
 hipError_t launch_cond_frames(const CondArgs &a, hipStream_t stream);
 hipError_t launch_cond_frames_slab(const CondArgs &a, hipStream_t stream);
+hipError_t launch_slab_prep(const CondArgs &a, const float *nz_in, float *nz_out, long nz_n, unsigned *xcc, int n_cus, hipStream_t stream);
 hipError_t launch_cond_frag(const CondArgs &a, int n_cus, hipStream_t stream);
 hipError_t launch_noise_mol(const float *in, float *out, long n, int B, int n_cus, hipStream_t stream);
 hipError_t launch_noise_fill(bool mol, int B, int C, int t0, int t1, uint64_t seed, const uint64_t *seg_id, float *out, int n_cus, hipStream_t stream);
@@ -864,9 +865,12 @@
         for (int s0 = pl.t0; s0 < pl.t1; s0 += pl.slab) {
             const int s1 = s0 + pl.slab < pl.t1 ? s0 + pl.slab : pl.t1;
             if (lib_noise) HIPCHK(launch_noise_fill(mol, B, p->tr.C, s0, s1, o->noise_seed, o->noise_seg_id, (float *)(ws + l.nlib), p->tr.n_cus, stream));
+            const bool prep_fused = k.slabbed && !(o->tuning & 8192);
+            const float *mol_rows = nullptr;
             if (mol) {
                 const float *const rows = lib_noise ? (const float *)(ws + l.nlib) : noise + (size_t)(s0 - pl.t0) * 11 * B;
-                HIPCHK(launch_noise_mol(rows, (float *)(ws + l.npre), (long)(s1 - s0) * 11 * B, B, p->tr.n_cus, stream));
+                if (prep_fused) mol_rows = rows;
+                else HIPCHK(launch_noise_mol(rows, (float *)(ws + l.npre), (long)(s1 - s0) * 11 * B, B, p->tr.n_cus, stream));
                 a.noise_pre = (const float *)(ws + l.npre);
                 a.noise_t0 = s0;
             } else if (lib_noise) {
@@ -877,9 +881,11 @@
             }
             if (k.slabbed) {
                 c.t0 = s0; c.B = B; c.FPS = pl.tab_fps;
-                HIPCHK(launch_cond_frames_slab(c, stream));
+                if (prep_fused) HIPCHK(launch_slab_prep(c, mol_rows, (float *)(ws + l.npre), (long)(s1 - s0) * 11 * B, (unsigned *)(ws + l.xcc), p->tr.n_cus, stream));
+                else HIPCHK(launch_cond_frames_slab(c, stream));
                 a.tab_fps = pl.tab_fps; a.tab_t0 = s0;
             }
+            bool xcc_clear = prep_fused;
             for (int r = 0; r < pl.rounds; ++r) {
                 const int rb0 = (int)(((long)r * B) / pl.rounds), rb1 = (int)(((long)(r + 1) * B) / pl.rounds);
                 const int nr = rb1 - rb0;
@@ -888,7 +894,8 @@
                 c.t0 = s0; c.t1 = s1; c.rb0 = rb0; c.B = nr; c.NG = ngr;
                 if (!k.slabbed) HIPCHK(launch_cond_frag(c, p->tr.n_cus, stream));
                 if (!k.slabbed || s0 == 0 || pl.rounds > 1 || (o->tuning & 4)) HIPCHK(hipMemsetAsync(ws + l.xbuf, 0xFF, k.xbuf_fill(pl.G), stream));
-                if (k.slabbed) HIPCHK(hipMemsetAsync(ws + l.xcc, 0, XCC_WORDS * sizeof(unsigned), stream));
+                if (k.slabbed && !xcc_clear) HIPCHK(hipMemsetAsync(ws + l.xcc, 0, XCC_WORDS * sizeof(unsigned), stream));
+                xcc_clear = false;
                 a.state = (float *)(ws + l.state) + (size_t)r * k.state_floats(pl.G);
                 a.t0 = s0; a.t1 = s1; a.cI_t0 = s0; a.rb0 = rb0; a.Btot = nr; a.NG = ngr; a.resume = s0 > 0 ? 1 : 0;
                 a.kind_tag = k.kind_tag;
diff --git a/wavernn_amd/csrc/wrnn_cond.hip b/wavernn_amd/csrc/wrnn_cond.hip
--- a/wavernn_amd/csrc/wrnn_cond.hip
+++ b/wavernn_amd/csrc/wrnn_cond.hip
@@ -227,14 +227,92 @@
     a.c4f[(size_t)row * H + r] = y4 + a.fc2_b[r];
 }
 
-__global__ __launch_bounds__(256) void wrnn_noise_mol_kernel(const float *__restrict__ in, float *__restrict__ out, long n, int B)
-{
-    const long stride = (long)gridDim.x * blockDim.x;
-    for (long i = (long)blockIdx.x * blockDim.x + threadIdx.x; i < n; i += stride) {
+__device__ __forceinline__ void noise_mol_body(const float *__restrict__ in, float *__restrict__ out, long n, int B, long i0, long stride)
+{
+    for (long i = i0; i < n; i += stride) {
         const float u = in[i];
         const int col = (int)(i % (11L * B));
         out[i] = (col < 10 * B) ? logf(-logf(u)) : (logf(u) - logf(1.0f - u));
     }
+}
+__global__ __launch_bounds__(256) void wrnn_noise_mol_kernel(const float *__restrict__ in, float *__restrict__ out, long n, int B)
+{
+    noise_mol_body(in, out, n, B, (long)blockIdx.x * blockDim.x + threadIdx.x, (long)gridDim.x * blockDim.x);
+}
+
+constexpr int SPR = 8;
+struct SlabPrepArgs {
+    CondArgs c;
+    const float *nz_in;
+    float *nz_out;
+    long nz_n;
+    unsigned *xcc;
+    int cond_blocks, nz_blocks;
+};
+__global__ __launch_bounds__(H) void wrnn_slab_prep_kernel(const SlabPrepArgs s)
+{
+    const int r = threadIdx.x;
+    if ((int)blockIdx.x >= s.cond_blocks) {
+        const int nb = (int)blockIdx.x - s.cond_blocks;
+        if (nb == 0)
+            for (int i = r; i < XCC_WORDS; i += H) s.xcc[i] = 0u;
+        noise_mol_body(s.nz_in, s.nz_out, s.nz_n, s.c.B, (long)nb * H + r, (long)s.nz_blocks * H);
+        return;
+    }
+    const CondArgs &a = s.c;
+    __shared__ float ax[SPR][4 * AUX];
+    const int nrows = a.B * a.FPS + 1, row0 = (int)blockIdx.x * SPR;
+    for (int q = r; q < SPR * 4 * AUX; q += H) {
+        const int i = q / (4 * AUX), e = q % (4 * AUX), row = row0 + i;
+        int f = a.NF;
+        if (row < a.B * a.FPS) {
+            const int b = row / a.FPS, j = row % a.FPS;
+            f = (a.seg_pos[b] + a.t0) / a.hop + j;
+        }
+        ax[i][e] = (f < a.NF) ? a.aux[(size_t)f * 4 * AUX + e] : 0.f;
+    }
+    __syncthreads();
+    float g0[SPR], g1[SPR], g2[SPR], y3[SPR], y4[SPR];
+#pragma unroll
+    for (int i = 0; i < SPR; ++i) { g0[i] = 0.f; g1[i] = 0.f; g2[i] = 0.f; y3[i] = 0.f; y4[i] = 0.f; }
+#pragma unroll 4
+    for (int k = 0; k < AUX; ++k) {
+        const float w0 = a.c2_wT[k * 3 * H + r], w1 = a.c2_wT[k * 3 * H + H + r], w2 = a.c2_wT[k * 3 * H + 2 * H + r];
+        const float w3 = a.c3_wT[k * H + r], w4 = a.c4_wT[k * H + r];
+#pragma unroll
+        for (int i = 0; i < SPR; ++i) {
+            g0[i] = fmaf(w0, ax[i][AUX + k], g0[i]);
+            g1[i] = fmaf(w1, ax[i][AUX + k], g1[i]);
+            g2[i] = fmaf(w2, ax[i][AUX + k], g2[i]);
+            y3[i] = fmaf(w3, ax[i][2 * AUX + k], y3[i]);
+            y4[i] = fmaf(w4, ax[i][3 * AUX + k], y4[i]);
+        }
+    }
+    const float b0 = a.b_ih2[r], b1 = a.b_ih2[H + r], b2 = a.b_ih2[2 * H + r], b3 = a.fc1_b[r], b4 = a.fc2_b[r];
+#pragma unroll
+    for (int i = 0; i < SPR; ++i) {
+        const int row = row0 + i;
+        if (row < nrows) {
+            a.c2f[(size_t)row * 3 * H + r] = g0[i] + b0;
+            a.c2f[(size_t)row * 3 * H + H + r] = g1[i] + b1;
+            a.c2f[(size_t)row * 3 * H + 2 * H + r] = g2[i] + b2;
+            a.c3f[(size_t)row * H + r] = y3[i] + b3;
+            a.c4f[(size_t)row * H + r] = y4[i] + b4;
+        }
+    }
+}
+
+hipError_t launch_slab_prep(const CondArgs &a, const float *nz_in, float *nz_out, long nz_n, unsigned *xcc, int n_cus, hipStream_t stream)
+{
+    SlabPrepArgs s;
+    s.c = a; s.nz_in = nz_in; s.nz_out = nz_out; s.nz_n = nz_in ? nz_n : 0; s.xcc = xcc;
+    s.cond_blocks = (a.B * a.FPS + 1 + SPR - 1) / SPR;
+    long nb = (s.nz_n + H - 1) / H;
+    if (nb > (long)n_cus * 4) nb = (long)n_cus * 4;
+    if (nb < 1) nb = 1;
+    s.nz_blocks = (int)nb;
+    hipLaunchKernelGGL(wrnn_slab_prep_kernel, dim3((unsigned)(s.cond_blocks + s.nz_blocks)), dim3(H), 0, stream, s);
+    return hipGetLastError();
 }
 
 hipError_t launch_noise_mol(const float *in, float *out, long n, int B, int n_cus, hipStream_t stream)
diff --git a/wavernn_amd/csrc/wrnn_pre.hip b/wavernn_amd/csrc/wrnn_pre.hip
--- a/wavernn_amd/csrc/wrnn_pre.hip
+++ b/wavernn_amd/csrc/wrnn_pre.hip
@@ -49,13 +49,13 @@
     return total;
 }
 
-__global__ __launch_bounds__(256) void wrnn_resnet_kernel(const PreArgs a)
+__device__ __forceinline__ void resnet_tile(const PreArgs &a, int tile)
 {
     __shared__ __attribute__((aligned(16))) float XIN[PNF * PLDI];
     __shared__ __attribute__((aligned(16))) float XA[PNF * PLDX];
     __shared__ __attribute__((aligned(16))) float XB[PNF * PLDX];
     const int tid = threadIdx.x, lane = tid & 63, w = tid >> 6;
-    const int j0 = blockIdx.x * PNF;
+    const int j0 = tile * PNF;
     const int N = a.N;
     for (int q = tid; q < PNF * PLDI; q += 256) {
         const int j = q / PLDI, k = q % PLDI;
@@ -121,6 +121,39 @@
     }
 }
 
+__global__ __launch_bounds__(256) void wrnn_resnet_kernel(const PreArgs a) { resnet_tile(a, blockIdx.x); }
+
+struct PreUttDev {
+    const float *mel;
+    float *up, *aux;
+    float *s1, *s2;
+    int n;
+    int blk[4];
+    int pad_;
+};
+static_assert(sizeof(PreUttDev) == 64, "table entry");
+struct PreManyArgs {
+    PreArgs w;
+    const PreUttDev *utt;
+    int n_utt;
+};
+__device__ __forceinline__ int pre_find_utt(const PreUttDev *utt, int n_utt, int stage, int block)
+{
+    int lo = 0, hi = n_utt;
+    while (hi - lo > 1) {
+        const int mid = (lo + hi) >> 1;
+        if (utt[mid].blk[stage] <= block) lo = mid; else hi = mid;
+    }
+    return lo;
+}
+__global__ __launch_bounds__(256) void wrnn_resnet_many_kernel(const PreManyArgs m)
+{
+    const int u = pre_find_utt(m.utt, m.n_utt, 0, blockIdx.x);
+    PreArgs a = m.w;
+    a.mel = m.utt[u].mel; a.aux = m.utt[u].aux; a.N = m.utt[u].n;
+    resnet_tile(a, blockIdx.x - m.utt[u].blk[0]);
+}
+
 struct GenPreArgs {
     PreArgs p;
     int feat, C, R, pad, gf;
@@ -173,16 +206,16 @@
     }
 }
 
-template <bool FIRST, bool LAST, int S, int F = PFEAT>
-__global__ __launch_bounds__(256) void wrnn_upstage_kernel(const float *__restrict__ in, float *__restrict__ out,
-                                                           const float *__restrict__ taps, int n_in, int s_rt, int pad, int indent, int feat_rt = PFEAT)
+template <bool FIRST, bool LAST, int S, int F>
+__device__ __forceinline__ void upstage_body(const float *__restrict__ in, float *__restrict__ out, const float *__restrict__ taps, int n_in, int s_rt,
+                                             int pad, int indent, int feat_rt, long blk, long nblk)
 {
     const int s = S > 0 ? S : s_rt;
     const int feat = F > 0 ? F : feat_rt;
     const long n_out = (long)n_in * s;
     const long total = LAST ? (n_out - 2L * indent) * feat : n_out * feat;
     const int ld_in = FIRST ? n_in - 2 * pad : n_in;
-    for (long idx = (long)blockIdx.x * blockDim.x + threadIdx.x; idx < total; idx += (long)gridDim.x * blockDim.x) {
+    for (long idx = blk * blockDim.x + threadIdx.x; idx < total; idx += nblk * blockDim.x) {
         int c;
         long q;
         if (LAST) { c = (int)(idx % feat); q = idx / feat + indent; }
@@ -203,16 +236,32 @@
         else out[(size_t)c * n_out + q] = acc;
     }
 }
+template <bool FIRST, bool LAST, int S, int F = PFEAT>
+__global__ __launch_bounds__(256) void wrnn_upstage_kernel(const float *__restrict__ in, float *__restrict__ out,
+                                                           const float *__restrict__ taps, int n_in, int s_rt, int pad, int indent, int feat_rt = PFEAT)
+{
+    upstage_body<FIRST, LAST, S, F>(in, out, taps, n_in, s_rt, pad, indent, feat_rt, blockIdx.x, gridDim.x);
+}
+template <bool FIRST, bool LAST, int S>
+__global__ __launch_bounds__(256) void wrnn_upstage_many_kernel(const PreUttDev *__restrict__ utt, int n_utt, const float *__restrict__ taps)
+{
+    constexpr int stage = FIRST ? 1 : 2;
+    const int u = pre_find_utt(utt, n_utt, stage, blockIdx.x);
+    const int nf = utt[u].n + 2 * PPAD, n_in = FIRST ? nf : nf * 5;
+    const float *in = FIRST ? utt[u].mel : utt[u].s1;
+    float *out = FIRST ? utt[u].s1 : (LAST ? utt[u].up : utt[u].s2);
+    upstage_body<FIRST, LAST, S, PFEAT>(in, out, taps, n_in, S, PPAD, 0, PFEAT, blockIdx.x - utt[u].blk[stage], utt[u + 1].blk[stage] - utt[u].blk[stage]);
+}
 
 template <int S>
-__global__ __launch_bounds__(256) void wrnn_upstage_last_kernel(const float *__restrict__ in, float *__restrict__ out,
-                                                                const float *__restrict__ taps, int n_in, int s_rt, int indent)
+__device__ __forceinline__ void upstage_last_body(const float *__restrict__ in, float *__restrict__ out, const float *__restrict__ taps, int n_in, int s_rt,
+                                                  int indent, long blk, long nblk)
 {
     constexpr int TQ = 64;
     __shared__ float tile[TQ][PFEAT + 1];
     const int s = S > 0 ? S : s_rt;
     const long n_out = (long)n_in * s, nq = n_out - 2L * indent;
-    for (long q0 = (long)blockIdx.x * TQ; q0 < nq; q0 += (long)gridDim.x * TQ) {
+    for (long q0 = blk * TQ; q0 < nq; q0 += nblk * TQ) {
         for (int e = threadIdx.x; e < TQ * PFEAT; e += 256) {
             const int c = e / TQ, ql = e % TQ;
             const long q = q0 + ql + indent;
@@ -235,6 +284,18 @@
         }
         __syncthreads();
     }
+}
+template <int S>
+__global__ __launch_bounds__(256) void wrnn_upstage_last_kernel(const float *__restrict__ in, float *__restrict__ out,
+                                                                const float *__restrict__ taps, int n_in, int s_rt, int indent)
+{
+    upstage_last_body<S>(in, out, taps, n_in, s_rt, indent, blockIdx.x, gridDim.x);
+}
+template <int S>
+__global__ __launch_bounds__(256) void wrnn_upstage_last_many_kernel(const PreUttDev *__restrict__ utt, int n_utt, const float *__restrict__ taps, int indent)
+{
+    const int u = pre_find_utt(utt, n_utt, 3, blockIdx.x);
+    upstage_last_body<S>(utt[u].s2, utt[u].up, taps, (utt[u].n + 2 * PPAD) * 25, S, indent, blockIdx.x - utt[u].blk[3], utt[u + 1].blk[3] - utt[u].blk[3]);
 }
 
 }
@@ -264,24 +325,53 @@
 
 static size_t generic_lds_bytes(int feat, int C, int pad, int gf) { return ((size_t)feat * (gf + 2 * pad) + 2 * (size_t)gf * C) * sizeof(float); }
 
-extern "C" int wrnn_pre_create(const wrnn_pre_weights *w, int device, wrnn_pre **out)
-{
-    if (!w || !out) PRE_FAIL(WRNN_ERR_ARG, "NULL argument");
+static int pre_check_dims(const wrnn_pre_weights *w, int *gf_out)
+{
     if (w->feat_dims < 1 || w->feat_dims > 4096 || w->compute_dims < 1 || w->compute_dims > 4096 || w->res_out_dims < 1 || w->res_out_dims > 4096 ||
         w->pad < 0 || w->pad > 64 || w->res_blocks < 0 || w->res_blocks > 64)
         PRE_FAIL(WRNN_ERR_ARG, "bad UpsampleNetwork dims: feat_dims %d, compute_dims %d, res_out_dims %d, pad %d, res_blocks %d", w->feat_dims,
                  w->compute_dims, w->res_out_dims, w->pad, w->res_blocks);
     for (int i = 0; i < 3; ++i)
         if (w->upsample_factors[i] < 1 || w->upsample_factors[i] > 64) PRE_FAIL(WRNN_ERR_ARG, "bad upsample factor %d", w->upsample_factors[i]);
-    if (!w->conv_in_w || !w->bn_in || (w->res_blocks && (!w->res_w || !w->res_bn)) || !w->conv_out_w || !w->conv_out_b || !w->up_w)
-        PRE_FAIL(WRNN_ERR_ARG, "NULL weight pointer");
-    const int FE = w->feat_dims, C = w->compute_dims, R = w->res_out_dims, PD = w->pad, KT = 2 * PD + 1;
+    const int FE = w->feat_dims, C = w->compute_dims, R = w->res_out_dims, PD = w->pad;
     const bool shipped_dims = FE == PFEAT && C == PC && R == PC && PD == PPAD;
     int gf = 0;
     if (!shipped_dims) {
         for (gf = 16; gf >= 1 && generic_lds_bytes(FE, C, PD, gf) > 65536; gf >>= 1) {}
         if (gf < 1) PRE_FAIL(WRNN_ERR_ARG, "UpsampleNetwork too wide for the pre-loop kernel (feat_dims %d, compute_dims %d, pad %d)", FE, C, PD);
     }
+    *gf_out = gf;
+    return WRNN_OK;
+}
+
+static void pre_set_dims(wrnn_pre *p, const wrnn_pre_weights *w, int device, int gf)
+{
+    p->device = device; p->blocks = w->res_blocks; p->total_scale = 1;
+    p->feat = w->feat_dims; p->C = w->compute_dims; p->R = w->res_out_dims; p->pad = w->pad; p->gf = gf;
+    for (int i = 0; i < 3; ++i) { p->scales[i] = w->upsample_factors[i]; p->total_scale *= w->upsample_factors[i]; }
+}
+
+extern "C" int wrnn_pre_debug_host_handle(const wrnn_pre_weights *w, wrnn_pre **out)
+{
+    if (!w || !out) PRE_FAIL(WRNN_ERR_ARG, "NULL argument");
+    int gf = 0;
+    const int rc = pre_check_dims(w, &gf);
+    if (rc != WRNN_OK) return rc;
+    wrnn_pre *p = new wrnn_pre();
+    pre_set_dims(p, w, -1, gf);
+    *out = p;
+    return WRNN_OK;
+}
+
+extern "C" int wrnn_pre_create(const wrnn_pre_weights *w, int device, wrnn_pre **out)
+{
+    if (!w || !out) PRE_FAIL(WRNN_ERR_ARG, "NULL argument");
+    int gf = 0;
+    const int rc_dims = pre_check_dims(w, &gf);
+    if (rc_dims != WRNN_OK) return rc_dims;
+    if (!w->conv_in_w || !w->bn_in || (w->res_blocks && (!w->res_w || !w->res_bn)) || !w->conv_out_w || !w->conv_out_b || !w->up_w)
+        PRE_FAIL(WRNN_ERR_ARG, "NULL weight pointer");
+    const int FE = w->feat_dims, C = w->compute_dims, R = w->res_out_dims, PD = w->pad, KT = 2 * PD + 1;
     int n = 0;
     if (hipGetDeviceCount(&n) != hipSuccess || n <= 0 || device >= n) PRE_FAIL(WRNN_ERR_NO_DEVICE, "no HIP device %d (count %d)", device, n);
     DeviceGuard dg(device);
@@ -308,9 +398,7 @@
     for (int i = 0; i < 3; ++i) { o_t[i] = put(w->up_w + toff, 2 * w->upsample_factors[i] + 1); toff += 2 * w->upsample_factors[i] + 1; }
     put(nullptr, 64);
     wrnn_pre *p = new wrnn_pre();
-    p->device = device; p->blocks = B; p->total_scale = 1;
-    p->feat = FE; p->C = C; p->R = R; p->pad = PD; p->gf = gf;
-    for (int i = 0; i < 3; ++i) { p->scales[i] = w->upsample_factors[i]; p->total_scale *= w->upsample_factors[i]; }
+    pre_set_dims(p, w, device, gf);
     hipError_t e = hipMalloc((void **)&p->dev, h.size() * 4);
     if (e != hipSuccess) { delete p; PRE_FAIL(WRNN_ERR_HIP, "hipMalloc failed: %s", hipGetErrorString(e)); }
     e = hipMemcpy(p->dev, h.data(), h.size() * 4, hipMemcpyHostToDevice);
@@ -325,7 +413,7 @@
 extern "C" void wrnn_pre_destroy(wrnn_pre *p)
 {
     if (!p) return;
-    (void)hipFree(p->dev);
+    if (p->dev) (void)hipFree(p->dev);
     delete p;
 }
 
@@ -345,6 +433,7 @@
     if (n_frames < 1 || (double)n_frames * p->total_scale > 2.0e9) PRE_FAIL(WRNN_ERR_ARG, "bad n_frames %d", n_frames);
     if (workspace_bytes < wrnn_pre_workspace_bytes(p, n_frames)) PRE_FAIL(WRNN_ERR_WORKSPACE, "workspace too small");
     if (((uintptr_t)workspace & 255) != 0) PRE_FAIL(WRNN_ERR_ARG, "workspace must be 256-byte aligned");
+    if (p->device < 0) PRE_FAIL(WRNN_ERR_NO_DEVICE, "a dims-only handle (wrnn_pre_debug_host_handle) launches nothing");
     hipStream_t stream = (hipStream_t)stream_;
     DeviceGuard dg(p->device);
     PRE_HIP(dg.err);
@@ -400,3 +489,96 @@
 {
     return pre_run(p, mel, n_frames, mel_rows, aux, workspace, workspace_bytes, stream, true);
 }
+
+static size_t al256(size_t x) { return (x + 255) & ~(size_t)255; }
+static bool pre_many_batched(const wrnn_pre *p) { return p->gf == 0 && p->scales[0] == 5 && p->scales[1] == 5 && p->scales[2] == 11; }
+static size_t pre_many_slice(const wrnn_pre *p, int32_t n_frames, bool rows_only, size_t *s2_off)
+{
+    if (!pre_many_batched(p)) return al256(wrnn_pre_workspace_bytes(p, n_frames));
+    const size_t nf = (size_t)n_frames + 2 * p->pad, s1 = al256(nf * p->scales[0] * p->feat * sizeof(float));
+    if (s2_off) *s2_off = s1;
+    return s1 + (rows_only ? 0 : al256(nf * p->scales[0] * p->scales[1] * p->feat * sizeof(float)));
+}
+
+extern "C" size_t wrnn_pre_workspace_bytes_many(const wrnn_pre *p, const wrnn_pre_utt *utts, int32_t n_utt, int32_t rows_only)
+{
+    if (!p || !utts || n_utt < 1) return 0;
+    size_t total = al256((size_t)(n_utt + 1) * sizeof(PreUttDev));
+    for (int u = 0; u < n_utt; ++u) {
+        if (utts[u].n_frames < 1) return 0;
+        total += pre_many_slice(p, utts[u].n_frames, rows_only != 0, nullptr);
+    }
+    return total;
+}
+
+extern "C" int wrnn_pre_upsample_many(const wrnn_pre *p, const wrnn_pre_utt *utts, int32_t n_utt, int32_t rows_only, float *mels_up, float *aux,
+                                      void *workspace, size_t workspace_bytes, void *stream_)
+{
+    if (!p || !mels_up || !aux || !workspace) PRE_FAIL(WRNN_ERR_ARG, "NULL argument");
+    if (!utts) PRE_FAIL(WRNN_ERR_ARG, "NULL utterance table");
+    if (n_utt < 1 || n_utt > 65536) PRE_FAIL(WRNN_ERR_ARG, "bad utterance count %d (1 .. 65536 per call)", n_utt);
+    for (int u = 0; u < n_utt; ++u) {
+        if (utts[u].n_frames < 1 || (double)utts[u].n_frames * p->total_scale > 2.0e9) PRE_FAIL(WRNN_ERR_ARG, "utterance %d: bad n_frames %d", u, utts[u].n_frames);
+        if (!utts[u].mel || utts[u].up_row < 0 || utts[u].aux_row < 0) PRE_FAIL(WRNN_ERR_ARG, "utterance %d: NULL mel or negative output offset", u);
+    }
+    const size_t need = wrnn_pre_workspace_bytes_many(p, utts, n_utt, rows_only);
+    if (workspace_bytes < need) PRE_FAIL(WRNN_ERR_ARG, "workspace too small: %zu bytes, wrnn_pre_workspace_bytes_many says %zu", workspace_bytes, need);
+    if (((uintptr_t)workspace & 255) != 0) PRE_FAIL(WRNN_ERR_ARG, "workspace must be 256-byte aligned");
+    if (p->device < 0) PRE_FAIL(WRNN_ERR_NO_DEVICE, "a dims-only handle (wrnn_pre_debug_host_handle) launches nothing");
+    const bool rows = rows_only != 0;
+    char *ws = (char *)workspace;
+    size_t off = al256((size_t)(n_utt + 1) * sizeof(PreUttDev));
+    if (!pre_many_batched(p)) {
+        for (int u = 0; u < n_utt; ++u) {
+            const size_t slice = pre_many_slice(p, utts[u].n_frames, rows, nullptr);
+            const int rc = pre_run(p, utts[u].mel, utts[u].n_frames, mels_up + (size_t)utts[u].up_row * p->feat, aux + (size_t)utts[u].aux_row * p->R,
+                                   ws + off, slice, stream_, rows);
+            if (rc != WRNN_OK) return rc;
+            off += slice;
+        }
+        return WRNN_OK;
+    }
+    hipStream_t stream = (hipStream_t)stream_;
+    DeviceGuard dg(p->device);
+    PRE_HIP(dg.err);
+    auto grid = [](long total) { long b = (total + 255) / 256; return (long)(b > 65535 ? 65535 : (b < 1 ? 1 : b)); };
+    std::vector<PreUttDev> tab((size_t)n_utt + 1);
+    long blk[4] = {0, 0, 0, 0};
+    for (int u = 0; u < n_utt; ++u) {
+        const int n = utts[u].n_frames;
+        const long nf = (long)n + 2 * PPAD;
+        size_t s2_off = 0;
+        const size_t slice = pre_many_slice(p, n, rows, &s2_off);
+        PreUttDev &d = tab[u];
+        d.mel = utts[u].mel; d.up = mels_up + (size_t)utts[u].up_row * PFEAT; d.aux = aux + (size_t)utts[u].aux_row * PC;
+        d.s1 = (float *)(ws + off); d.s2 = rows ? nullptr : (float *)(ws + off + s2_off);
+        d.n = n; d.pad_ = 0;
+        for (int s = 0; s < 4; ++s) d.blk[s] = (int)blk[s];
+        blk[0] += (n + PNF - 1) / PNF;
+        blk[1] += grid(nf * 5 * PFEAT);
+        blk[2] += grid(nf * 25 * PFEAT);
+        blk[3] += rows ? 0 : grid((long)n * p->total_scale * 4);
+        for (int s = 0; s < 4; ++s)
+            if (blk[s] > 0x7fffffffL) PRE_FAIL(WRNN_ERR_ARG, "too many frames for one call (stage grid of %ld workgroups); split the table", blk[s]);
+        off += slice;
+    }
+    memset(&tab[n_utt], 0, sizeof(PreUttDev));
+    for (int s = 0; s < 4; ++s) tab[n_utt].blk[s] = (int)blk[s];
+    PreUttDev *d_tab = (PreUttDev *)ws;
+    PRE_HIP(hipMemcpyAsync(d_tab, tab.data(), tab.size() * sizeof(PreUttDev), hipMemcpyHostToDevice, stream));
+    PreManyArgs m;
+    memset(&m, 0, sizeof m);
+    m.w.conv_in_w = p->conv_in_w; m.w.bn_in = p->bn_in; m.w.res_w = p->res_w; m.w.res_bn = p->res_bn;
+    m.w.conv_out_w = p->conv_out_w; m.w.conv_out_b = p->conv_out_b; m.w.blocks = p->blocks;
+    m.utt = d_tab; m.n_utt = n_utt;
+    hipLaunchKernelGGL(wrnn_resnet_many_kernel, dim3((unsigned)blk[0]), dim3(256), 0, stream, m);
+    hipLaunchKernelGGL((wrnn_upstage_many_kernel<true, false, 5>), dim3((unsigned)blk[1]), dim3(256), 0, stream, d_tab, n_utt, p->taps[0]);
+    if (rows) {
+        hipLaunchKernelGGL((wrnn_upstage_many_kernel<false, true, 5>), dim3((unsigned)blk[2]), dim3(256), 0, stream, d_tab, n_utt, p->taps[1]);
+    } else {
+        hipLaunchKernelGGL((wrnn_upstage_many_kernel<false, false, 5>), dim3((unsigned)blk[2]), dim3(256), 0, stream, d_tab, n_utt, p->taps[1]);
+        hipLaunchKernelGGL((wrnn_upstage_last_many_kernel<11>), dim3((unsigned)blk[3]), dim3(256), 0, stream, d_tab, n_utt, p->taps[2], PPAD * p->total_scale);
+    }
+    PRE_HIP(hipGetLastError());
+    return WRNN_OK;
+}
diff --git a/wavernn_amd/model.py b/wavernn_amd/model.py
--- a/wavernn_amd/model.py
+++ b/wavernn_amd/model.py
@@ -117,8 +117,11 @@
         self.loop_algo = 'auto'
         self.sparse_groups = None
         self.pre_algo = 'native'
+        self.pre_batched = True
         self.pre_streams = 8
         self.pinned_output = True
+        self.post_tables_early = True
+        self.slab_prep_split = False
         self.mel_in_loop = None
         self.post_algo = 'native'
         self.noise_chunk_bytes = 2 << 30
diff --git a/wavernn_amd/post.py b/wavernn_amd/post.py
--- a/wavernn_amd/post.py
+++ b/wavernn_amd/post.py
@@ -30,24 +30,46 @@
     return _tables[key]
 
 
-def unfold_on_device(segments, first, folds, wave_lens, overlap, hop, n_classes, mu_law, batched=True):
+class UnfoldTables:
+
+    def __init__(self, first, folds, wave_lens, overlap, hop, n_classes, mu_law, batched, dev):
+        self.tail_len = 20 * hop
+        if min(wave_lens) < self.tail_len:
+            raise ValueError(f'operands could not be broadcast together with shapes ({min(wave_lens)},) ({self.tail_len},)')
+        n = self.n_utt = len(wave_lens)
+        self.off = np.concatenate([[0], np.cumsum(wave_lens)]).astype(np.int64)
+        stage = torch.empty(8 * (n + 1) + 8 * n, dtype=torch.uint8, pin_memory=True)
+        h = stage.numpy()
+        h[:8 * (n + 1)] = self.off.view(np.uint8)
+        h[8 * (n + 1):] = np.concatenate([np.asarray(first, np.int32), np.asarray(folds, np.int32)]).view(np.uint8)
+        self.tabs = stage.to(dev, non_blocking=True)
+        self.overlap, self.batched, self.n_classes = (overlap if batched else 0), bool(batched), n_classes
+        self.fade_in, self.fade_out, self.tail = _fade_tables(self.overlap, hop, dev)
+        self.lut = _mu_law_lut(n_classes, dev) if mu_law else None
+        self.out = torch.empty(int(self.off[-1]), dtype=torch.float64, device=dev)
+        self.key = (tuple(int(x) for x in first), tuple(int(x) for x in folds), tuple(int(x) for x in wave_lens))
+
+
+def prepare_unfold(first, folds, wave_lens, overlap, hop, n_classes, mu_law, batched=True, device='cuda'):
+    return UnfoldTables(first, folds, wave_lens, overlap, hop, n_classes, mu_law, batched, torch.device(device))
+
+
+def unfold_on_device(segments, first, folds, wave_lens, overlap, hop, n_classes, mu_law, batched=True, tables=None):
     dev = segments.device
-    tail_len = 20 * hop
-    if min(wave_lens) < tail_len:
-        raise ValueError(f'operands could not be broadcast together with shapes ({min(wave_lens)},) ({tail_len},)')
+    t = tables
+    if t is None:
+        t = UnfoldTables(first, folds, wave_lens, overlap, hop, n_classes, mu_law, batched, dev)
+    elif t.key != (tuple(int(x) for x in first), tuple(int(x) for x in folds), tuple(int(x) for x in wave_lens)) or t.lut is None and mu_law:
+        raise ValueError('unfold tables prepared for other utterances')
     L = _lib.lib()
-    n_utt, T = len(wave_lens), int(segments.shape[1])
-    off = np.concatenate([[0], np.cumsum(wave_lens)]).astype(np.int64)
-    tabs = torch.from_numpy(np.concatenate([np.asarray(first, np.int32), np.asarray(folds, np.int32)])).to(dev)
-    d_off = torch.from_numpy(off).to(dev)
-    fade_in, fade_out, tail = _fade_tables(overlap if batched else 0, hop, dev)
-    lut = _mu_law_lut(n_classes, dev) if mu_law else None
-    out = torch.empty(int(off[-1]), dtype=torch.float64, device=dev)
+    n_utt, T, off = t.n_utt, int(segments.shape[1]), t.off
     segments = segments.contiguous()
     stream = torch.cuda.current_stream(dev).cuda_stream
-    rc = L.wrnn_post_unfold(segments.data_ptr(), T, n_utt, tabs.data_ptr(), tabs.data_ptr() + 4 * n_utt, d_off.data_ptr(),
-                            lut.data_ptr() if lut is not None else None, n_classes, fade_in.data_ptr(), fade_out.data_ptr(),
-                            overlap if batched else 0, tail.data_ptr(), tail_len, 1 if batched else 0, out.data_ptr(), stream)
+    p_off = t.tabs.data_ptr()
+    p_first = p_off + 8 * (n_utt + 1)
+    rc = L.wrnn_post_unfold(segments.data_ptr(), T, n_utt, p_first, p_first + 4 * n_utt, p_off,
+                            t.lut.data_ptr() if t.lut is not None else None, n_classes, t.fade_in.data_ptr(), t.fade_out.data_ptr(),
+                            t.overlap, t.tail.data_ptr(), t.tail_len, 1 if t.batched else 0, t.out.data_ptr(), stream)
     if rc != 0:
         raise _lib.WrnnError(f'wrnn_post_unfold failed (rc={rc}): {L.wrnn_post_last_error().decode()}')
-    return out, [(int(off[u]), int(off[u + 1])) for u in range(n_utt)]
+    return t.out, [(int(off[u]), int(off[u + 1])) for u in range(n_utt)]
diff --git a/wavernn_amd/pre.py b/wavernn_amd/pre.py
--- a/wavernn_amd/pre.py
+++ b/wavernn_amd/pre.py
@@ -92,7 +92,32 @@
             raise _lib.WrnnError(f'wrnn_pre_upsample failed (rc={rc}): {self.lib.wrnn_pre_last_error().decode()}')
         return mels_up, aux
 
-    def upsample_many(self, jobs, rows=False, streams=8):
+    def upsample_batched(self, jobs, rows=False):
+        mels = [mel[0] if mel.dim() == 3 else mel for mel, _, _ in jobs]
+        mels = [m.to(self.device, torch.float32).contiguous() for m in mels]
+        tab = (_lib.PreUtt * len(jobs))()
+        up_base, aux_base = min(up.data_ptr() for _, up, _ in jobs), min(ax.data_ptr() for _, _, ax in jobs)
+        up_b, aux_b = 4 * self.feat_dims, 4 * self.res_out_dims
+        for k, (m, (_, up, ax)) in enumerate(zip(mels, jobs)):
+            n = int(m.shape[1])
+            if m.shape[0] != self.feat_dims:
+                raise ValueError(f'Expected a mel shaped ({self.feat_dims}, n_hops), but got {tuple(m.shape)}!')
+            assert up.is_contiguous() and ax.is_contiguous() and up.shape == ((self.rows_of(n) if rows else n * self.hop), self.feat_dims)
+            assert ax.shape == (n, self.res_out_dims) and (up.data_ptr() - up_base) % up_b == 0 and (ax.data_ptr() - aux_base) % aux_b == 0
+            tab[k].mel, tab[k].n_frames = m.data_ptr(), n
+            tab[k].up_row, tab[k].aux_row = (up.data_ptr() - up_base) // up_b, (ax.data_ptr() - aux_base) // aux_b
+        nbytes = int(self.lib.wrnn_pre_workspace_bytes_many(self._pre, tab, len(jobs), int(rows)))
+        ws = getattr(self, '_ws_many', None)
+        if ws is None or ws.numel() < nbytes:
+            ws = self._ws_many = torch.empty(nbytes, dtype=torch.uint8, device=self.device)
+        stream = torch.cuda.current_stream(self.device).cuda_stream
+        rc = self.lib.wrnn_pre_upsample_many(self._pre, tab, len(jobs), int(rows), up_base, aux_base, ws.data_ptr(), ws.numel(), stream)
+        if rc != 0:
+            raise _lib.WrnnError(f'wrnn_pre_upsample_many failed (rc={rc}): {self.lib.wrnn_pre_last_error().decode()}')
+
+    def upsample_many(self, jobs, rows=False, streams=8, batched=True):
+        if batched and jobs:
+            return self.upsample_batched(jobs, rows=rows)
         if streams <= 1 or len(jobs) <= 1:
             for mel, up, aux in jobs:
                 self.upsample(mel, mels_up=up, aux=aux, _rows=rows)
```

Result: faster. 11.26 million (median of 6 runs) (+1.1%).
